# INDA25PlusPlus/rsoderh-raytracing

Hardware: AMD Instinct MI355X
Metric: Mrays/s, house.toml 1920x1080 256spp 8-bounce (higher is better)
Workload: dtype f32; 1 GPU; house.toml 1920x1080 256 spp 8 bounces, synthetic 2048x1024 HDRI env; parallelism=single GPU

## Files before the change

include/rsrt.h:

```cpp
#ifndef RSRT_H
#define RSRT_H

#include <stddef.h>
#include <stdint.h>

#include "rsrt_types.h"

#ifdef __cplusplus
extern "C" {
#endif

typedef enum rsrt_status {
    RSRT_OK = 0,
    RSRT_ERR_INVALID_ARGUMENT = 1,
    RSRT_ERR_NO_DEVICE = 2,
    RSRT_ERR_HIP = 3,
    RSRT_ERR_NOT_READY = 4,
    RSRT_ERR_OUT_OF_MEMORY = 5,
    RSRT_ERR_COMM = 6
} rsrt_status;

typedef struct rsrt_context rsrt_context;

enum {
// ... 92 lines not shown
rsrt_status rsrt_resolve_mean_f16(rsrt_context *ctx, uint32_t sample_total, uint16_t *host_rgba16f, size_t n_halfs);

rsrt_status rsrt_debug_view_f16(rsrt_context *ctx, uint32_t dev_index, uint32_t environment_index, uint32_t sample_count,
                                uint16_t *host_rgba16f_inout, size_t n_halfs);

rsrt_status rsrt_display_srgb8(rsrt_context *ctx, uint32_t sample_total, uint8_t *host_rgba8, size_t n_bytes);

rsrt_status rsrt_render(rsrt_context *ctx, const rsrt_camera *camera, uint32_t width, uint32_t height,
                        uint32_t sample_begin, uint32_t sample_count, uint32_t max_bounces,
                        uint32_t environment_index, uint32_t flags, void *hip_stream);
rsrt_status rsrt_synchronize(rsrt_context *ctx);
rsrt_status rsrt_get_stats(rsrt_context *ctx, rsrt_stats *out);

rsrt_status rsrt_aov_render(rsrt_context *ctx, const rsrt_camera *camera, uint32_t width, uint32_t height, uint32_t sample_begin,
                            uint32_t sample_count, uint32_t flags, void *hip_stream);
rsrt_status rsrt_aov_bind(rsrt_context *ctx, void *device_f32x8, uint32_t width, uint32_t height);
rsrt_status rsrt_aov_clear(rsrt_context *ctx);
rsrt_status rsrt_aov_download(rsrt_context *ctx, float *host_f32x8, size_t n_floats);

enum { RSRT_DENOISE_DEMODULATE = 1u };
typedef struct rsrt_denoise_params {
    uint32_t iterations;
    uint32_t flags;
    float sigma_color;
    float sigma_normal;
    float sigma_depth;
} rsrt_denoise_params;
rsrt_status rsrt_denoise(rsrt_context *ctx, uint32_t sample_total, uint32_t aov_sample_total, const rsrt_denoise_params *params,
                         void *device_out_rgba32f, void *hip_stream);
rsrt_status rsrt_denoised_download(rsrt_context *ctx, float *host_rgba, size_t n_floats);
rsrt_status rsrt_denoised_display_srgb8(rsrt_context *ctx, uint8_t *host_rgba8, size_t n_bytes);

typedef struct rsrt_temporal_params {
    uint32_t max_history;
    float depth_tolerance;
    float normal_tolerance;
} rsrt_temporal_params;
rsrt_status rsrt_temporal_accumulate(rsrt_context *ctx, const rsrt_camera *camera, uint32_t sample_total, uint32_t aov_sample_total,
                                     const rsrt_temporal_params *params, void *hip_stream);
rsrt_status rsrt_temporal_reset(rsrt_context *ctx);
rsrt_status rsrt_temporal_download(rsrt_context *ctx, float *host_rgba, size_t n_floats);
enum { RSRT_DENOISE_TEMPORAL = 2u };

enum { RSRT_TEMPORAL_MOMENTS = 1u };
rsrt_status rsrt_temporal_accumulate_ex(rsrt_context *ctx, const rsrt_camera *camera, uint32_t sample_total, uint32_t aov_sample_total,
                                        const rsrt_temporal_params *params, uint32_t flags, void *hip_stream);
rsrt_status rsrt_temporal_moments_download(rsrt_context *ctx, float *host_f32x4, size_t n_floats);
enum { RSRT_DENOISE_VARIANCE = 4u, RSRT_DENOISE_CLAMP = 8u };

rsrt_status rsrt_guide_render(rsrt_context *ctx, const rsrt_camera *camera, uint32_t width, uint32_t height, uint32_t sample_begin,
                              uint32_t sample_count, uint32_t flags, void *hip_stream);
rsrt_status rsrt_guide_bind(rsrt_context *ctx, void *device_f32x8, uint32_t width, uint32_t height);
rsrt_status rsrt_guide_clear(rsrt_context *ctx);
rsrt_status rsrt_guide_download(rsrt_context *ctx, float *host_f32x8, size_t n_floats);

enum { RSRT_UPSAMPLE_DEMODULATE = 1u, RSRT_UPSAMPLE_DENOISED = 2u, RSRT_UPSAMPLE_TEMPORAL = 4u };
typedef struct rsrt_upsample_params {
    uint32_t flags;
    float sigma_normal;
    float sigma_depth;
} rsrt_upsample_params;
rsrt_status rsrt_upsample(rsrt_context *ctx, uint32_t sample_total, uint32_t aov_sample_total, uint32_t guide_sample_total,
                          const rsrt_upsample_params *params, void *device_out_rgba32f, void *hip_stream);
rsrt_status rsrt_upsampled_download(rsrt_context *ctx, float *host_rgba, size_t n_floats);
rsrt_status rsrt_upsampled_display_srgb8(rsrt_context *ctx, uint8_t *host_rgba8, size_t n_bytes);

typedef struct rsrt_hit {
    uint32_t did_hit;
    float distance;
    float hit_point[3];
    float normal[3];
    uint32_t material_id;
} rsrt_hit;
rsrt_status rsrt_cast_rays(rsrt_context *ctx, uint32_t n_rays, const float *origins_xyz, const float *directions_xyz,
                           uint32_t mode, uint32_t flags, rsrt_hit *out);

rsrt_status rsrt_wide_tree_build(const rsrt_primitive_info *primitives, uint32_t n_primitives, const rsrt_bvh_node *bvh_nodes, uint32_t n_bvh_nodes,
                                 float *wnodes_out, uint32_t *n_wnodes, uint32_t *old_of_new);

rsrt_status rsrt_get_debug_counters(rsrt_context *ctx, uint64_t out[32]);
rsrt_status rsrt_get_region_counters(rsrt_context *ctx, uint64_t out[32]);
rsrt_status rsrt_get_walk_counters(rsrt_context *ctx, uint64_t *out, uint32_t n);

rsrt_status rsrt_selftest_numerics(rsrt_context *ctx, uint64_t out[4]);

const char *rsrt_describe(rsrt_context *ctx);
const char *rsrt_build_id(void);

#ifdef __cplusplus
}
#endif
#endif
```

rsoderh-raytracing_amd/csrc/hip/rsrt_api.hip:

```cpp
#include <hip/hip_fp16.h>
#include <hip/hip_runtime.h>

#include <algorithm>
#include <cstdarg>
#include <cstdio>
#include <cstdlib>
#include <cstring>
#include <string>
#include <vector>

#include "../../../include/rsrt.h"
#include "../../../include/rsrt_tonemap.h"
#include "rt_device.h"

#define RT_BLOCK 256
#define RT_STATS_WORDS 48
#define RT_WAVE 64
#ifndef RT_WALK_POOL
#define RT_WALK_POOL 192u
#endif
#ifndef RT_BIG_POOL
#define RT_BIG_POOL 192u
#endif

// ... 395 lines not shown
    case 2: return reinterpret_cast<const void *>(&rt_cast_rays_kernel<SV, (SV == 2 ? 1 : 2)>);
    case 3: return reinterpret_cast<const void *>(&rt_cast_rays_kernel<SV, 3>);
    case 5: return reinterpret_cast<const void *>(&rt_cast_rays_kernel<SV, 5>);
    case 6: return reinterpret_cast<const void *>(&rt_cast_rays_coop_kernel<SV>);
    default: return reinterpret_cast<const void *>(&rt_cast_rays_kernel<SV, 4>);
    }
}
static const void *probe_function(int sv, int trav)
{
    return sv == 0 ? probe_function_sv<0>(trav) : (sv == 1 ? probe_function_sv<1>(trav) : probe_function_sv<2>(trav));
}

static constexpr uint32_t kLanes = 4;
static constexpr uint64_t kSmallPaths = 4ull << 20;
static constexpr int kPipeBlocks = 1;
static constexpr uint32_t kChunksPerWave = 32;
static constexpr uint32_t kDescendQuorum = 30;
static constexpr uint32_t kStopQuorum = 40;

struct rsrt_context {
    int device = 0;
    hipStream_t stream = nullptr;
    hipEvent_t ev[3] = {nullptr, nullptr, nullptr};
    std::string error;
    std::string description;
    int cus = 0;
    float4 *scene_blob = nullptr;
    DevScene scene{};
    bool scene_ready = false;
    uint32_t hybrid_head_f4 = 0, hybrid_pnode_f4 = 0;
    uint32_t wimg_nodes = 0;
    std::vector<Env> envs;
    uint32_t rank = 0, world = 1, tile_w = 16, tile_h = 16;
    float4 *accum = nullptr;
    float4 *accum_owned = nullptr;
    uint32_t acc_w = 0, acc_h = 0;
    struct Lane {
        hipStream_t stream = nullptr;
        unsigned int *work_counter = nullptr;
        float *sample_buf = nullptr;
        size_t sample_buf_bytes = 0;
        uint32_t *cold_state = nullptr;
        size_t cold_bytes = 0;
        hipEvent_t resolved = nullptr;
        bool resolved_valid = false;
        hipEvent_t traced = nullptr;
        bool traced_valid = false;
        hipEvent_t caller_at = nullptr;
    };
    Lane lanes[kLanes];
    uint32_t next_small_lane = 1;
    unsigned long long *dev_stats = nullptr;
    rsrt_stats stats{};
    struct PassEvents { hipEvent_t begin, traced, end; };
    std::vector<PassEvents> pending_events;
    double cum_trace_ms = 0, cum_resolve_ms = 0, base_trace_ms = 0, base_resolve_ms = 0;
    unsigned long long base_counts[4] = {0, 0, 0, 0};
    uint32_t cum_launches = 0, base_launches = 0;
    std::vector<hipEvent_t> event_pool;
    hipEvent_t last_event = nullptr;
    hipStream_t last_stream = nullptr;
    bool last_valid = false;
    void *comm = nullptr;
    bool comm_owned = false;
    bool comm_dense_mode = false;
    uint32_t comm_rank = 0, comm_world = 1;
    struct ReduceEvents { hipEvent_t begin, end; };
    std::vector<ReduceEvents> pending_reduce;
    double cum_reduce_ms = 0, base_reduce_ms = 0;
    uint32_t cum_reduces = 0;
    void *comm_buf = nullptr;
    size_t comm_buf_bytes = 0;
    void *scratch = nullptr;
    size_t scratch_bytes = 0;
    int blocks_per_cu[21] = {};
    bool small_form = false;
    int max_traversal = 6;
    uint32_t coop_lds_cap = RT_COOP_NCAP, coop_lifo_at = RT_COOP_LIFO_AT, coop_narrow_at = RT_COOP_NARROW_AT;
    uint32_t coop_gcap = RT_COOP_GCAP;
    bool allow_flat = true;
    bool flat_oriented = true;
    bool allow_hybrid = true;
    uint32_t trace_budget = 0;
    uint32_t flat_quorum = 20;
    size_t sample_buffer_budget = 16ull << 30;
    uint32_t probe_repeat = 1;
    int hw_queues = 4;
    bool hw_queue_warned = false;
    unsigned long long debug_words[32] = {0};
    float4 *aov = nullptr;
    float4 *aov_owned = nullptr;
    uint32_t aov_w = 0, aov_h = 0;
    void *dn_scratch = nullptr;
    uint32_t dn_w = 0, dn_h = 0;
    float4 *dn_last = nullptr;
    float4 *tp_buf = nullptr;
    uint32_t tp_w = 0, tp_h = 0, tp_cur = 0, tp_frames = 0;
    float tp_cam[13] = {0};
    float4 *tp_mom = nullptr;
    uint32_t tp_moments = 0;
    float4 *guide = nullptr;
    float4 *guide_owned = nullptr;
    uint32_t guide_w = 0, guide_h = 0;
    void *up_scratch = nullptr;
    uint32_t up_w = 0, up_h = 0;
    float4 *up_out = nullptr;
    uint32_t up_out_w = 0, up_out_h = 0;
    float4 *up_last = nullptr;
    uint32_t up_last_w = 0, up_last_h = 0;
};

namespace {

rsrt_status fail(rsrt_context *ctx, rsrt_status st, const char *fmt, ...)
{
    char buf[1024];
    va_list ap;
    va_start(ap, fmt);
    vsnprintf(buf, sizeof buf, fmt, ap);
    va_end(ap);
    if (ctx) ctx->error = buf;
    else g_create_error = buf;
    return st;
}

#define HIP_TRY(ctx, expr)                                                                                   \
    do {                                                                                                     \
        hipError_t e_ = (expr);                                                                              \
        if (e_ != hipSuccess)                                                                                \
            return fail(ctx, e_ == hipErrorOutOfMemory ? RSRT_ERR_OUT_OF_MEMORY : RSRT_ERR_HIP, "%s failed: %s", #expr, \
                        hipGetErrorString(e_));                                                              \
    } while (0)

struct DeviceGuard {
    explicit DeviceGuard(int dev) { (void)hipSetDevice(dev); }
};

inline float fmaxh(float a, float b) { return a < b ? b : a; }
inline float fminh(float a, float b) { return b < a ? b : a; }
inline float saturateh(float x) { return fminh(fmaxh(x, 0.0f), 1.0f); }
inline float4 f4(float x, float y, float z, float w) { return make_float4(x, y, z, w); }
inline float u2f(uint32_t u) { float f; memcpy(&f, &u, 4); return f; }

void make_sphere_record(const rsrt_sphere &s, float4 *r)
{
    r[0] = f4(s.pos[0], s.pos[1], s.pos[2], u2f(PRIM_SPHERE | (s.material_id << 2)));
    r[1] = f4(s.radius, s.radius * s.radius, 0, 0);
    r[2] = r[3] = f4(0, 0, 0, 0);
}
void make_plane_record(const rsrt_plane &p, float4 *r)
{
    r[0] = f4(p.pos[0], p.pos[1], p.pos[2], u2f(PRIM_PLANE | (p.material_id << 2)));
    r[1] = f4(p.normal[0], p.normal[1], p.normal[2], 0);
    r[2] = f4(p.base_change_matrix[0][0], p.base_change_matrix[1][0], p.base_change_matrix[2][0], 0);
    r[3] = f4(p.base_change_matrix[0][2], p.base_change_matrix[1][2], p.base_change_matrix[2][2], 0);
}
void make_triangle_record(const rsrt_triangle &t, uint32_t index, const rsrt_vec3 *v, float4 *r)
{
    const float *a = v[t.vertex_0].v, *b = v[t.vertex_1].v, *c = v[t.vertex_2].v;
    r[0] = f4(a[0], a[1], a[2], u2f(PRIM_TRIANGLE | (t.material_id << 2)));
    r[1] = f4(b[0] - a[0], b[1] - a[1], b[2] - a[2], u2f(index));
    r[2] = f4(c[0] - a[0], c[1] - a[1], c[2] - a[2], 0);
    r[3] = f4(0, 0, 0, 0);
}
bool same_test(const float4 *a, const float4 *b)
{
    uint32_t ta, tb;
    memcpy(&ta, &a[0].w, 4); memcpy(&tb, &b[0].w, 4);
    if ((ta & 3u) != (tb & 3u) || memcmp(&a[0], &b[0], 12) != 0) return false;
    if ((ta & 3u) == PRIM_TRIANGLE) return memcmp(&a[1], &b[1], 12) == 0 && memcmp(&a[2], &b[2], 12) == 0;
    return memcmp(a + 1, b + 1, 3 * sizeof(float4)) == 0;
}
void make_material_record(const rsrt_material &m, float4 *r)
{
    const float t = saturateh(m.metallic);
    float f0[3], kd[3];
    for (int k = 0; k < 3; k++) f0[k] = (1.0f - t) * 0.04f + t * m.color[k];
    const float maxf0 = fmaxh(f0[0], fmaxh(f0[1], f0[2]));
    for (int k = 0; k < 3; k++) kd[k] = (m.color[k] * (1.0f - t)) * (1.0f - maxf0);
    const float alpha = fmaxh(0.001f, m.roughness * m.roughness);
    const float ps = saturateh(0.2126f * f0[0] + 0.7152f * f0[1] + 0.0722f * f0[2]);
    r[0] = f4(m.color[0], m.color[1], m.color[2], m.metallic);
    r[1] = f4(f0[0], f0[1], f0[2], alpha);
    r[2] = f4(m.emission[0], m.emission[1], m.emission[2], ps);
    r[3] = f4(kd[0], kd[1], kd[2], 1.0f - ps);
}

struct WideNode { uint32_t ch[4]; uint32_t n_ch, n_int, first_child; };
bool build_wide_tree(const rsrt_bvh_node *nodes, uint32_t n_nodes, const rsrt_primitive_info *prims, uint32_t n_prims, std::vector<WideNode> &wide,
                     std::vector<rsrt_primitive_info> &prims_out, std::vector<rsrt_bvh_node> &nodes_out, std::vector<uint32_t> *old_of_new, uint32_t *wide_depth = nullptr)
{
    wide.clear();
    bool ok = n_nodes >= 3 && nodes[0].primitives_len == 0;
    {
        std::vector<uint8_t> covered(n_prims, 0);
        for (uint32_t i = 0; i < n_nodes && ok; i++) {
            const rsrt_bvh_node &nd = nodes[i];
            if (nd.primitives_len > 8) ok = false;
            for (uint32_t k = 0; k < nd.primitives_len && ok; k++) {
                uint8_t &c = covered[nd.primitives_or_second_child_index + k];
                ok = c == 0;
                c = 1;
            }
            if (nd.primitives_len == 0)
                for (uint32_t c : {i + 1u, nd.primitives_or_second_child_index})
                    for (int k = 0; k < 3; k++)
                        ok = ok && nodes[c].bounds_min[k] >= nd.bounds_min[k] && nodes[c].bounds_max[k] <= nd.bounds_max[k];
        }
        for (uint32_t p = 0; p < n_prims; p++) ok = ok && covered[p];
    }
    if (!ok) return false;
    auto area = [&](uint32_t i) {
        const double dx = (double)nodes[i].bounds_max[0] - nodes[i].bounds_min[0], dy = (double)nodes[i].bounds_max[1] - nodes[i].bounds_min[1],
                     dz = (double)nodes[i].bounds_max[2] - nodes[i].bounds_min[2];
        const double a = dx * dy + dy * dz + dz * dx;
        return a == a ? a : 0.0;
    };
    std::vector<uint32_t> queue{0u}, level{0u};
    uint32_t wdepth = 1;
    const bool by_area = true;
    std::vector<std::pair<double, uint32_t>> heap{{area(0), 0u}};
    size_t bfs_next = 0;
    while (by_area ? !heap.empty() : bfs_next < queue.size()) {
        size_t qi;
        if (by_area) {
            std::pop_heap(heap.begin(), heap.end(), [](const std::pair<double, uint32_t> &a, const std::pair<double, uint32_t> &b) { return a.first < b.first || (a.first == b.first && a.second > b.second); });
            qi = heap.back().second;
            heap.pop_back();
        } else {
            qi = bfs_next++;
        }
        const uint32_t r = queue[qi];
        std::vector<uint32_t> ch{r + 1u, nodes[r].primitives_or_second_child_index};
        while (ch.size() < 4) {
            int best = -1;
            for (size_t k = 0; k < ch.size(); k++)
                if (nodes[ch[k]].primitives_len == 0 && (best < 0 || area(ch[k]) > area(ch[best]))) best = (int)k;
            if (best < 0) break;
            const uint32_t c = ch[best];
            ch[best] = c + 1u;
            ch.insert(ch.begin() + best + 1, nodes[c].primitives_or_second_child_index);
        }
        WideNode w{};
        for (uint32_t c : ch) if (nodes[c].primitives_len == 0) w.ch[w.n_ch++] = c;
        w.n_int = w.n_ch;
        for (uint32_t c : ch) if (nodes[c].primitives_len != 0) w.ch[w.n_ch++] = c;
        w.first_child = (uint32_t)queue.size();
        for (uint32_t k = 0; k < w.n_int; k++) {
            const uint32_t idx = (uint32_t)queue.size();
            queue.push_back(w.ch[k]);
            level.push_back(level[qi] + 1u);
            wdepth = std::max(wdepth, level[qi] + 2u);
            if (by_area) {
                heap.push_back({area(w.ch[k]), idx});
// ... 269 lines not shown

rsrt_status pack_environment(rsrt_context *ctx, Env &e)
{
    const size_t n = (size_t)e.width * e.height;
    rsrt_status st = begin_work(ctx, ctx->stream);
    if (st) return st;
    const unsigned nb = (unsigned)((n + 255) / 256);
    hipLaunchKernelGGL(rt_env_pack_texels_kernel, dim3(nb), dim3(256), 0, ctx->stream, e.rgba, e.alias, n);
    hipLaunchKernelGGL(rt_env_pack_alias_kernel, dim3(nb), dim3(256), 0, ctx->stream, e.alias, n);
    HIP_TRY(ctx, hipGetLastError());
    if ((st = end_work(ctx, ctx->stream))) return st;
    HIP_TRY(ctx, hipStreamSynchronize(ctx->stream));
    return RSRT_OK;
}

rsrt_status display_from_n(rsrt_context *ctx, const float4 *sum, size_t n, uint32_t sample_total, uint8_t *host_rgba8, size_t n_bytes)
{
    DeviceGuard g(ctx->device);
    if (!host_rgba8 || n_bytes != n * 4 || sample_total == 0) return fail(ctx, RSRT_ERR_INVALID_ARGUMENT, "display_srgb8: expected %zu bytes and sample_total > 0", n * 4);
    rsrt_status st = ensure_scratch(ctx, n * sizeof(uchar4));
    if (st || (st = begin_work(ctx, ctx->stream))) return st;
    uchar4 *tmp = static_cast<uchar4 *>(ctx->scratch);
    hipLaunchKernelGGL(rt_display_kernel, dim3((unsigned)((n + 255) / 256)), dim3(256), 0, ctx->stream, sum, n, sample_total, tmp);
    HIP_TRY(ctx, hipGetLastError());
    HIP_TRY(ctx, hipMemcpyAsync(host_rgba8, tmp, n * sizeof(uchar4), hipMemcpyDeviceToHost, ctx->stream));
    if ((st = end_work(ctx, ctx->stream))) return st;
    HIP_TRY(ctx, hipStreamSynchronize(ctx->stream));
    return RSRT_OK;
}

rsrt_status display_from(rsrt_context *ctx, const float4 *sum, uint32_t sample_total, uint8_t *host_rgba8, size_t n_bytes)
{
    return display_from_n(ctx, sum, (size_t)ctx->acc_w * ctx->acc_h, sample_total, host_rgba8, n_bytes);
}

}

extern "C" {

rsrt_status rsrt_context_create(int device_index, rsrt_context **out)
{
    if (!out) return fail(nullptr, RSRT_ERR_INVALID_ARGUMENT, "out is NULL");
    *out = nullptr;
    int n = 0;
    hipError_t e = hipGetDeviceCount(&n);
    if (e != hipSuccess || n == 0)
        return fail(nullptr, RSRT_ERR_NO_DEVICE, "no HIP device available (%s); librsrt has no CPU path", hipGetErrorString(e));
    if (device_index < 0 || device_index >= n) return fail(nullptr, RSRT_ERR_INVALID_ARGUMENT, "device_index %d out of range [0,%d)", device_index, n);
    hipDeviceProp_t prop;
    if ((e = hipGetDeviceProperties(&prop, device_index)) != hipSuccess) return fail(nullptr, RSRT_ERR_HIP, "hipGetDeviceProperties: %s", hipGetErrorString(e));
    if (strncmp(prop.gcnArchName, "gfx950", 6) != 0)
        return fail(nullptr, RSRT_ERR_NO_DEVICE, "device %d is %s; librsrt is built for gfx950 (MI355X) only", device_index, prop.gcnArchName);
    rsrt_context *ctx = new rsrt_context();
    ctx->device = device_index;
    ctx->cus = prop.multiProcessorCount;
    DeviceGuard g(device_index);
    if ((e = hipStreamCreateWithFlags(&ctx->stream, hipStreamNonBlocking)) != hipSuccess ||
        (e = hipEventCreateWithFlags(&ctx->last_event, hipEventDisableTiming)) != hipSuccess ||
        (e = [&] { hipError_t r = hipSuccess;
                   for (auto &L : ctx->lanes) {
                       if (r == hipSuccess) r = hipMalloc(&L.work_counter, sizeof(unsigned int));
                       if (r == hipSuccess) r = hipStreamCreateWithFlags(&L.stream, hipStreamNonBlocking);
                       if (r == hipSuccess) r = hipEventCreateWithFlags(&L.resolved, hipEventDisableTiming);
                       if (r == hipSuccess) r = hipEventCreateWithFlags(&L.traced, hipEventDisableTiming);
                       if (r == hipSuccess) r = hipEventCreateWithFlags(&L.caller_at, hipEventDisableTiming);
                   }
                   return r; }()) != hipSuccess ||
        (e = hipMalloc(&ctx->dev_stats, RT_STATS_WORDS * sizeof(unsigned long long))) != hipSuccess ||
        (e = hipMemsetAsync(ctx->dev_stats, 0, RT_STATS_WORDS * sizeof(unsigned long long), ctx->stream)) != hipSuccess ||
        (e = hipStreamSynchronize(ctx->stream)) != hipSuccess) {
        fail(nullptr, RSRT_ERR_HIP, "context setup failed: %s", hipGetErrorString(e));
        delete ctx;
        return RSRT_ERR_HIP;
    }
    for (bool small : {false, true})
        for (int m = 0; m < 21; m++) (void)hipFuncSetAttribute(variant_function(small, m / 7, m % 7), hipFuncAttributeMaxDynamicSharedMemorySize, 160 * 1024);
    if (const char *kv = getenv("RSRT_KERNEL")) ctx->small_form = atoi(kv) == 2;
    if (const char *hy = getenv("RSRT_HYBRID")) ctx->allow_hybrid = atoi(hy) != 0;
    if (const char *ty = getenv("RSRT_TRAVERSAL")) ctx->max_traversal = atoi(ty);
    if (const char *fl = getenv("RSRT_FLAT")) ctx->allow_flat = atoi(fl) != 0;
    if (const char *fo = getenv("RSRT_FLAT_ORIENTED")) ctx->flat_oriented = atoi(fo) != 0;
    if (const char *tb = getenv("RSRT_TRACE_BUDGET")) { int v = atoi(tb); if (v > 0) ctx->trace_budget = (uint32_t)v; }
    if (const char *fq = getenv("RSRT_FLAT_QUORUM")) { int v = atoi(fq); if (v >= 0 && v <= 100) ctx->flat_quorum = (uint32_t)v; }
    if (const char *e2 = getenv("RSRT_SAMPLE_BUFFER_MB")) { long v = atol(e2); if (v > 0) ctx->sample_buffer_budget = (size_t)v << 20; }
    if (const char *pr = getenv("RSRT_PROBE_REPEAT")) { int v = atoi(pr); if (v > 1 && v <= 4096) ctx->probe_repeat = (uint32_t)v; }
    if (const char *cl = getenv("RSRT_COOP_LDS_CAP")) { int v = atoi(cl); if (v >= (int)RT_COOP_MIN_LDS_CAP && v <= (int)RT_COOP_NCAP) ctx->coop_lds_cap = (uint32_t)v; }
    if (const char *cf = getenv("RSRT_COOP_LIFO_AT")) { int v = atoi(cf); if (v >= 0 && v <= (int)RT_COOP_NARROW_AT) ctx->coop_lifo_at = (uint32_t)v; }
    if (const char *cn = getenv("RSRT_COOP_NARROW_AT")) { int v = atoi(cn); if (v >= 0 && v <= (int)RT_COOP_NARROW_AT) ctx->coop_narrow_at = (uint32_t)v; }
    if (const char *cg = getenv("RSRT_COOP_GCAP")) { int v = atoi(cg); if (v >= 64 && v <= (int)RT_COOP_GCAP && v % 64 == 0) ctx->coop_gcap = (uint32_t)v; }
    if (const char *cm = getenv("RSRT_COMM_MODE")) ctx->comm_dense_mode = strcmp(cm, "reduce") == 0;
    if (const char *hq = getenv("GPU_MAX_HW_QUEUES")) { int v = atoi(hq); if (v > 0) ctx->hw_queues = v; }
    for (int m = 0; m < 21; m++) (void)hipFuncSetAttribute(probe_function(m / 7, m % 7), hipFuncAttributeMaxDynamicSharedMemorySize, 160 * 1024);
    char buf[256];
    snprintf(buf, sizeof buf, "librsrt 0.1; %s (%s); %d CUs", prop.name, prop.gcnArchName, ctx->cus);
    ctx->description = buf;
    *out = ctx;
    return RSRT_OK;
}

void rsrt_context_destroy(rsrt_context *ctx)
{
    if (!ctx) return;
    DeviceGuard g(ctx->device);
    (void)sync_all(ctx);
    (void)rsrt_comm_destroy(ctx);
    for (auto &re : ctx->pending_reduce) { (void)hipEventDestroy(re.begin); (void)hipEventDestroy(re.end); }
    if (ctx->last_event) (void)hipEventDestroy(ctx->last_event);
    (void)hipFree(ctx->scratch);
    (void)hipFree(ctx->comm_buf);
    for (auto &pe : ctx->pending_events) { (void)hipEventDestroy(pe.begin); (void)hipEventDestroy(pe.traced); (void)hipEventDestroy(pe.end); }
    for (auto e : ctx->event_pool) (void)hipEventDestroy(e);
    (void)hipFree(ctx->scene_blob);
    for (auto &e : ctx->envs) { (void)hipFree(e.rgba); (void)hipFree(e.alias); }
    (void)hipFree(ctx->accum_owned);
    (void)hipFree(ctx->aov_owned);
    (void)hipFree(ctx->dn_scratch);
    (void)hipFree(ctx->tp_buf);
    (void)hipFree(ctx->tp_mom);
    (void)hipFree(ctx->guide_owned);
    (void)hipFree(ctx->up_scratch);
    (void)hipFree(ctx->up_out);
    for (auto &L : ctx->lanes) {
        (void)hipFree(L.sample_buf);
        (void)hipFree(L.cold_state);
        (void)hipFree(L.work_counter);
        if (L.resolved) (void)hipEventDestroy(L.resolved);
        if (L.traced) (void)hipEventDestroy(L.traced);
        if (L.caller_at) (void)hipEventDestroy(L.caller_at);
        if (L.stream) (void)hipStreamDestroy(L.stream);
    }
    (void)hipFree(ctx->dev_stats);
    (void)hipStreamDestroy(ctx->stream);
    delete ctx;
}

const char *rsrt_last_error(const rsrt_context *ctx) { return ctx ? ctx->error.c_str() : g_create_error.c_str(); }

#ifndef RSRT_BUILD_ID
#define RSRT_BUILD_ID "unknown"
#endif
const char *rsrt_build_id(void) { return RSRT_BUILD_ID; }

const char *rsrt_describe(rsrt_context *ctx) { return ctx ? ctx->description.c_str() : "librsrt 0.1"; }

rsrt_status rsrt_upload_scene(rsrt_context *ctx, const rsrt_material *materials, uint32_t n_materials, const rsrt_sphere *spheres,
                              uint32_t n_spheres, const rsrt_plane *planes, uint32_t n_planes, const rsrt_vec3 *vertices,
                              uint32_t n_vertices, const rsrt_vec3 *normals, uint32_t n_normals, const rsrt_triangle *triangles,
                              uint32_t n_triangles, const rsrt_primitive_info *primitives_in, uint32_t n_primitives,
                              const rsrt_bvh_node *nodes_in, uint32_t n_nodes)
{
    if (!ctx) return RSRT_ERR_INVALID_ARGUMENT;
    DeviceGuard g(ctx->device);
    ctx->tp_frames = 0;
    const rsrt_primitive_info *primitives = primitives_in;
    const rsrt_bvh_node *nodes = nodes_in;
    if (n_nodes == 0 || !nodes) return fail(ctx, RSRT_ERR_INVALID_ARGUMENT, "bvh_nodes is empty");
    if (n_nodes >= RT_END) return fail(ctx, RSRT_ERR_INVALID_ARGUMENT, "bvh_nodes: %u nodes exceed the 25-bit traversal cursor", n_nodes);
    if ((n_materials && !materials) || (n_spheres && !spheres) || (n_planes && !planes) || (n_vertices && !vertices) ||
        (n_normals && !normals) || (n_triangles && !triangles) || (n_primitives && !primitives))
        return fail(ctx, RSRT_ERR_INVALID_ARGUMENT, "a non-empty array has a NULL pointer");
    if (n_materials >= (1u << 30)) return fail(ctx, RSRT_ERR_INVALID_ARGUMENT, "too many materials");
    for (uint32_t i = 0; i < n_spheres; i++)
        if (spheres[i].material_id >= n_materials) return fail(ctx, RSRT_ERR_INVALID_ARGUMENT, "sphere %u: material_id %u out of range", i, spheres[i].material_id);
    for (uint32_t i = 0; i < n_planes; i++)
        if (planes[i].material_id >= n_materials) return fail(ctx, RSRT_ERR_INVALID_ARGUMENT, "plane %u: material_id %u out of range", i, planes[i].material_id);
    for (uint32_t i = 0; i < n_triangles; i++) {
        const rsrt_triangle &t = triangles[i];
        if (t.material_id >= n_materials) return fail(ctx, RSRT_ERR_INVALID_ARGUMENT, "triangle %u: material_id %u out of range", i, t.material_id);
        if (t.vertex_0 >= n_vertices || t.vertex_1 >= n_vertices || t.vertex_2 >= n_vertices)
            return fail(ctx, RSRT_ERR_INVALID_ARGUMENT, "triangle %u: vertex index out of range", i);
        if (t.normal_0 >= n_normals || t.normal_1 >= n_normals || t.normal_2 >= n_normals)
            return fail(ctx, RSRT_ERR_INVALID_ARGUMENT, "triangle %u: normal index out of range", i);
    }
    for (uint32_t i = 0; i < n_primitives; i++) {
        const rsrt_primitive_info &p = primitives[i];
        uint32_t lim = p.primitive_type == 0 ? n_spheres : (p.primitive_type == 1 ? n_planes : (p.primitive_type == 2 ? n_triangles : 0));
        if (p.index >= lim) return fail(ctx, RSRT_ERR_INVALID_ARGUMENT, "primitive %u: type %u index %u out of range", i, p.primitive_type, p.index);
    }
    uint32_t depth = 0;
    {
        std::vector<std::pair<uint32_t, uint32_t>> st;
        std::vector<uint8_t> seen(n_nodes, 0);
        st.push_back({0u, 0u});
        while (!st.empty()) {
            auto [i, d] = st.back();
            st.pop_back();
            if (seen[i]) return fail(ctx, RSRT_ERR_INVALID_ARGUMENT, "bvh node %u reachable twice", i);
            seen[i] = 1;
            depth = std::max(depth, d);
            const rsrt_bvh_node &nd = nodes[i];
            if (nd.primitives_len > 0) {
                if (nd.primitives_len > 0xffffu || (uint64_t)nd.primitives_or_second_child_index + nd.primitives_len > n_primitives)
                    return fail(ctx, RSRT_ERR_INVALID_ARGUMENT, "bvh leaf %u: primitive range out of bounds", i);
            } else {
                uint32_t second = nd.primitives_or_second_child_index;
                if (nd.split_axis > 2 || i + 1 >= n_nodes || second <= i + 1 || second >= n_nodes)
                    return fail(ctx, RSRT_ERR_INVALID_ARGUMENT, "bvh interior node %u: bad child index / axis", i);
                st.push_back({second, d + 1});
                st.push_back({i + 1, d + 1});
            }
        }
        for (uint32_t i = 0; i < n_nodes; i++)
            if (!seen[i]) return fail(ctx, RSRT_ERR_INVALID_ARGUMENT, "bvh node %u is not reachable from the root", i);
    }
    std::vector<WideNode> wide;
    std::vector<rsrt_primitive_info> prims_perm;
    std::vector<rsrt_bvh_node> nodes_perm;
    uint32_t wide_depth = 0;
    const bool wide_ok = build_wide_tree(nodes, n_nodes, primitives, n_primitives, wide, prims_perm, nodes_perm, nullptr, &wide_depth);
    if (wide_ok) {
        primitives = prims_perm.data();
        nodes = nodes_perm.data();
    }
    std::vector<uint32_t> escape(8ull * n_nodes, RT_END);
    for (uint32_t q = 0; q < 8; q++) {
        std::vector<std::pair<uint32_t, uint32_t>> st;
        st.push_back({0u, RT_END});
        while (!st.empty()) {
            auto [i, esc] = st.back();
            st.pop_back();
            escape[(size_t)q * n_nodes + i] = esc;
            const rsrt_bvh_node &nd = nodes[i];
            if (nd.primitives_len == 0) {
                const bool far_first = (q >> nd.split_axis) & 1u;
                const uint32_t first = i + 1, second = nd.primitives_or_second_child_index;
                const uint32_t near_c = far_first ? second : first, far_c = far_first ? first : second;
                st.push_back({near_c, far_c});
                st.push_back({far_c, esc});
            }
        }
    }
    const size_t esc_f4 = (8ull * n_nodes + 3) / 4;
    std::vector<uint32_t> leaf_nodes;
    bool flat_ok = n_primitives <= 64 && n_spheres <= 64 && n_planes <= 64;
    {
        std::vector<uint8_t> covered(n_primitives, 0);
        for (uint32_t i = 0; i < n_nodes && flat_ok; i++)
            for (uint32_t k = 0; k < nodes[i].primitives_len && flat_ok; k++) {
                uint8_t &c = covered[nodes[i].primitives_or_second_child_index + k];
                flat_ok = c == 0;
                c = 1;
            }
    }
    for (uint32_t i = 0; i < n_nodes; i++) {
        const rsrt_bvh_node &nd = nodes[i];
        if (nd.primitives_len != 0) { leaf_nodes.push_back(i); continue; }
        for (uint32_t c : {i + 1u, nd.primitives_or_second_child_index})
            for (int k = 0; k < 3; k++)
                flat_ok = flat_ok && nodes[c].bounds_min[k] >= nd.bounds_min[k] && nodes[c].bounds_max[k] <= nd.bounds_max[k];
    }
    flat_ok = flat_ok && leaf_nodes.size() <= 32;
    std::vector<uint32_t> flat_rank(8 * 16, 0u);
    uint64_t tri_mask = 0, plane_mask = 0;
    if (flat_ok) {
        for (uint32_t p = 0; p < n_primitives; p++) {
            if (primitives[p].primitive_type >= 2) tri_mask |= 1ull << p;
            else if (primitives[p].primitive_type == 1) plane_mask |= 1ull << p;
        }
        for (uint32_t q = 0; q < 8; q++) {
            std::vector<uint32_t> st{0u};
            uint32_t pos = 0;
            while (!st.empty()) {
                const uint32_t i = st.back();
                st.pop_back();
                const rsrt_bvh_node &nd = nodes[i];
                if (nd.primitives_len != 0) {
                    for (uint32_t k = 0; k < nd.primitives_len; k++, pos++) {
                        const uint32_t rec = nd.primitives_or_second_child_index + k;
                        flat_rank[q * 16 + (rec >> 2)] |= pos << (8 * (rec & 3));
                    }
                } else {
                    const bool far_first = (q >> nd.split_axis) & 1u;
                    const uint32_t first = i + 1, second = nd.primitives_or_second_child_index;
                    st.push_back(far_first ? first : second);
                    st.push_back(far_first ? second : first);
                }
            }
        }
    }
    const size_t flat_f4 = flat_ok ? 2 * leaf_nodes.size() : 0, rank_f4 = flat_ok ? 32 : 0;
    const size_t ostride_f4 = 2 * (leaf_nodes.size() | 1);
    const size_t oflat_f4 = flat_ok && ctx->flat_oriented ? 8 * ostride_f4 : 0;
    const size_t base_f4 = 2ull * n_nodes + 4ull * n_primitives + 3ull * n_triangles + 4ull * n_materials + 4ull * n_spheres + 4ull * n_planes + esc_f4 + flat_f4;
    const bool flat_oriented = oflat_f4 != 0 && (base_f4 + oflat_f4) * sizeof(float4) <= kSmallImageBytes;
    std::vector<uint32_t> prim_rank(8ull * n_primitives, 0xffffffffu);
    for (uint32_t q = 0; q < 8; q++) {
        std::vector<uint32_t> st{0u};
        uint32_t pos = 0;
        while (!st.empty()) {
            const uint32_t i = st.back();
            st.pop_back();
            const rsrt_bvh_node &nd = nodes[i];
            if (nd.primitives_len != 0) {
                for (uint32_t k = 0; k < nd.primitives_len; k++, pos++) {
                    uint32_t &rk = prim_rank[(size_t)q * n_primitives + nd.primitives_or_second_child_index + k];
                    rk = std::min(rk, pos);
                }
            } else {
                const bool far_first = (q >> nd.split_axis) & 1u;
                const uint32_t first = i + 1, second = nd.primitives_or_second_child_index;
                st.push_back(far_first ? first : second);
                st.push_back(far_first ? second : first);
            }
        }
    }
    struct PNode { uint32_t old; uint32_t jump_to; };
    std::vector<uint32_t> succ(n_nodes, n_nodes);
    {
        std::vector<std::pair<uint32_t, uint32_t>> st;
        st.push_back({0u, n_nodes});
        while (!st.empty()) {
            auto [i, after] = st.back();
            st.pop_back();
            succ[i] = after;
            const rsrt_bvh_node &nd = nodes[i];
            if (nd.primitives_len == 0) {
                st.push_back({i + 1, nd.primitives_or_second_child_index});
                st.push_back({nd.primitives_or_second_child_index, after});
            }
        }
    }
    const uint32_t kTopMax = kHybridRoomF4 / 2u;
    std::vector<PNode> plist;
    uint32_t top_elems = 0;
    for (uint32_t want = std::min<uint32_t>(n_nodes, kTopMax);; want = want * 7 / 8) {
        std::vector<uint8_t> in_top(n_nodes, 0);
        {
            auto area = [&](uint32_t i) {
                const double dx = (double)nodes[i].bounds_max[0] - nodes[i].bounds_min[0], dy = (double)nodes[i].bounds_max[1] - nodes[i].bounds_min[1],
                             dz = (double)nodes[i].bounds_max[2] - nodes[i].bounds_min[2];
                const double a = dx * dy + dy * dz + dz * dx;
                return a == a ? a : 0.0;
            };
            std::vector<std::pair<double, uint32_t>> heap;
            heap.push_back({area(0), 0u});
            uint32_t taken = 0;
            while (!heap.empty() && taken < want) {
                std::pop_heap(heap.begin(), heap.end());
                const uint32_t i = heap.back().second;
                heap.pop_back();
                in_top[i] = 1;
                taken++;
                if (nodes[i].primitives_len == 0)
                    for (uint32_t c : {i + 1u, nodes[i].primitives_or_second_child_index}) {
                        heap.push_back({area(c), c});
                        std::push_heap(heap.begin(), heap.end());
                    }
            }
        }
        plist.clear();
        for (int pass = 0; pass < 2; pass++) {
            std::vector<uint32_t> order;
            for (uint32_t i = 0; i < n_nodes; i++)
                if ((in_top[i] != 0) == (pass == 0)) order.push_back(i);
            for (size_t k = 0; k < order.size(); k++) {
                const uint32_t i = order[k];
                plist.push_back({i, 0u});
                const uint32_t follows = k + 1 < order.size() ? order[k + 1] : 0xffffffffu;
                if (nodes[i].primitives_len != 0 && succ[i] != follows) plist.push_back({0xffffffffu, succ[i]});
            }
            if (pass == 0) top_elems = (uint32_t)plist.size();
        }
        if (top_elems <= kTopMax || want <= 1) break;
    }
    const uint32_t n_pnodes = (uint32_t)plist.size();
    if (n_pnodes >= RT_END) return fail(ctx, RSRT_ERR_INVALID_ARGUMENT, "bvh_nodes: %u traversal elements exceed the 25-bit cursor", n_pnodes);
    std::vector<uint32_t> new_id(n_nodes + 1, n_pnodes);
    for (uint32_t e = 0; e < n_pnodes; e++)
        if (plist[e].old != 0xffffffffu) new_id[plist[e].old] = e;
    const size_t pnode_f4 = 2ull * n_pnodes, prank_f4 = (8ull * n_primitives + 3) / 4, wnode_f4 = 8ull * wide.size();
    const uint32_t wimg_nodes = wide_ok ? (uint32_t)wide.size() : 0u;
    const size_t n_f4 = base_f4 + (flat_oriented ? oflat_f4 : 0);
    std::vector<float4> img(n_f4 + rank_f4 + pnode_f4 + prank_f4 + wnode_f4);
    float4 *p = img.data();
    float4 *p_nodes = p;
    bool typed_leaves = true;
    for (uint32_t i = 0; i < n_nodes; i++) typed_leaves = typed_leaves && nodes[i].primitives_len <= 8;
    for (uint32_t i = 0; i < n_nodes; i++, p += 2) {
        const rsrt_bvh_node &nd = nodes[i];
        p[0] = f4(nd.bounds_min[0], nd.bounds_min[1], nd.bounds_min[2], u2f(nd.primitives_or_second_child_index));
        uint32_t hi = nd.split_axis;
        if (nd.primitives_len != 0) {
            hi = 0;
            if (typed_leaves)
                for (uint32_t k = 0; k < nd.primitives_len; k++) {
                    const uint32_t ty = primitives[nd.primitives_or_second_child_index + k].primitive_type;
                    if (ty >= 2) hi |= 1u << k;
                    else if (ty == 1) hi |= 1u << (8 + k);
                }
        }
        p[1] = f4(nd.bounds_max[0], nd.bounds_max[1], nd.bounds_max[2], u2f(nd.primitives_len | (hi << 16)));
    }
    float4 *p_esc = p;
    memcpy(p_esc, escape.data(), escape.size() * sizeof(uint32_t));
    p += esc_f4;
    const size_t traversal_head_f4 = (size_t)(p - img.data());
    float4 *p_prims = p;
    for (uint32_t i = 0; i < n_primitives; i++, p += 4) {
        const rsrt_primitive_info &pi = primitives[i];
        if (pi.primitive_type == 0) make_sphere_record(spheres[pi.index], p);
        else if (pi.primitive_type == 1) make_plane_record(planes[pi.index], p);
        else make_triangle_record(triangles[pi.index], pi.index, vertices, p);
    }
    float4 *p_trin = p;
    for (uint32_t i = 0; i < n_triangles; i++, p += 3) {
        const float *a = normals[triangles[i].normal_0].v, *b = normals[triangles[i].normal_1].v, *c = normals[triangles[i].normal_2].v;
        p[0] = f4(a[0], a[1], a[2], b[0]);
        p[1] = f4(b[1], b[2], c[0], c[1]);
        p[2] = f4(c[2], 0, 0, 0);
    }
    float4 *p_mats = p;
    for (uint32_t i = 0; i < n_materials; i++, p += 4) make_material_record(materials[i], p);
    float4 *p_fbs = p;
    for (uint32_t i = 0; i < n_spheres; i++, p += 4) make_sphere_record(spheres[i], p);
    float4 *p_fbp = p;
    for (uint32_t i = 0; i < n_planes; i++, p += 4) make_plane_record(planes[i], p);
    float4 *p_flat = p;
    if (flat_ok) {
        for (uint32_t i : leaf_nodes) {
            const rsrt_bvh_node &nd = nodes[i];
            uint64_t lm = (nd.primitives_len >= 64 ? ~0ull : ((1ull << nd.primitives_len) - 1ull)) << nd.primitives_or_second_child_index;
            for (uint32_t b = 1; b < nd.primitives_len; b++)
                for (uint32_t a = 0; a < b; a++)
                    if (same_test(p_prims + 4 * (nd.primitives_or_second_child_index + a), p_prims + 4 * (nd.primitives_or_second_child_index + b))) {
                        lm &= ~(1ull << (nd.primitives_or_second_child_index + b));
                        break;
                    }
            p[0] = f4(nd.bounds_min[0], nd.bounds_min[1], nd.bounds_min[2], u2f((uint32_t)lm));
            p[1] = f4(nd.bounds_max[0], nd.bounds_max[1], nd.bounds_max[2], u2f((uint32_t)(lm >> 32)));
            p += 2;
        }
        if (flat_oriented) {
            for (uint32_t q = 0; q < 8; q++)
                for (size_t k = 0; k < leaf_nodes.size(); k++) {
                    const float4 lo = p_flat[2 * k], hi = p_flat[2 * k + 1];
                    float4 *c = p + q * ostride_f4 + 2 * k;
                    c[0] = f4(q & 1u ? hi.x : lo.x, q & 2u ? hi.y : lo.y, q & 4u ? hi.z : lo.z, lo.w);
                    c[1] = f4(q & 1u ? lo.x : hi.x, q & 2u ? lo.y : hi.y, q & 4u ? lo.z : hi.z, hi.w);
                }
            p += oflat_f4;
        }
        memcpy(p, flat_rank.data(), flat_rank.size() * sizeof(uint32_t));
    }
    {
        std::vector<uint32_t> twins;
        for (uint32_t i = 0; i < n_nodes; i++) {
            const rsrt_bvh_node &nd = nodes[i];
            for (uint32_t b = 1; b < nd.primitives_len; b++)
                for (uint32_t a = 0; a < b; a++)
                    if (same_test(p_prims + 4 * (nd.primitives_or_second_child_index + a), p_prims + 4 * (nd.primitives_or_second_child_index + b))) {
                        twins.push_back(nd.primitives_or_second_child_index + b);
                        break;
                    }
        }
        for (uint32_t r : twins) p_prims[4 * r + 2].w = u2f(1u);
    }
    float4 *p_pnodes = img.data() + n_f4 + rank_f4;
    for (uint32_t e = 0; e < n_pnodes; e++) {
        if (plist[e].old == 0xffffffffu) {
            const uint32_t to = new_id[plist[e].jump_to];
            p_pnodes[2 * e] = f4(0, 0, 0, u2f(to));
            p_pnodes[2 * e + 1] = f4(0, 0, 0, u2f(to));
            continue;
        }
        const uint32_t i = plist[e].old;
        p_pnodes[2 * e] = p_nodes[2 * i];
        p_pnodes[2 * e + 1] = p_nodes[2 * i + 1];
        if (nodes[i].primitives_len == 0) {
            p_pnodes[2 * e].w = u2f(new_id[i + 1]);
            p_pnodes[2 * e + 1].w = u2f(new_id[succ[i]]);
        } else {
            p_pnodes[2 * e].w = u2f(nodes[i].primitives_or_second_child_index | 0x80000000u);
        }
    }
    if (n_primitives) memcpy(p_pnodes + pnode_f4, prim_rank.data(), prim_rank.size() * sizeof(uint32_t));
    fill_wide_nodes(wide, nodes, primitives, p_pnodes + pnode_f4 + prank_f4);

    { rsrt_status st0 = sync_all(ctx); if (st0) return st0; }
    if (ctx->scene_blob) { (void)hipFree(ctx->scene_blob); ctx->scene_blob = nullptr; }
    ctx->scene_ready = false;
    HIP_TRY(ctx, hipMalloc(&ctx->scene_blob, img.size() * sizeof(float4)));
    HIP_TRY(ctx, hipMemcpy(ctx->scene_blob, img.data(), img.size() * sizeof(float4), hipMemcpyHostToDevice));
    DevScene &sc = ctx->scene;
    sc.nodes = ctx->scene_blob + (p_nodes - img.data());
    sc.prims = ctx->scene_blob + (p_prims - img.data());
    sc.tri_normals = ctx->scene_blob + (p_trin - img.data());
    sc.materials = ctx->scene_blob + (p_mats - img.data());
    sc.fb_spheres = ctx->scene_blob + (p_fbs - img.data());
    sc.fb_planes = ctx->scene_blob + (p_fbp - img.data());
    sc.escape = ctx->scene_blob + (p_esc - img.data());
    sc.flat_leaves = ctx->scene_blob + (p_flat - img.data());
    sc.flat_ostride = flat_oriented ? (uint32_t)ostride_f4 : 0u;
    sc.flat_rank = reinterpret_cast<const uint32_t *>(ctx->scene_blob + n_f4);
    sc.pnodes = ctx->scene_blob + n_f4 + rank_f4;
    sc.n_pnodes = n_pnodes;
    sc.prim_rank = reinterpret_cast<const uint32_t *>(ctx->scene_blob + n_f4 + rank_f4 + pnode_f4);
    sc.wnodes = ctx->scene_blob + n_f4 + rank_f4 + pnode_f4 + prank_f4;
    sc.n_wnodes = (uint32_t)wide.size();
    sc.wide_ok = wide_ok ? 1u : 0u;
    sc.wide_deep = (wide_ok && wide_depth > RT_WSTACK + 1u) ? 1u : 0u;
    sc.coop_ok = (wide_ok && n_primitives < RT_COOP_MAX_RECORDS && wide.size() < RT_COOP_MAX_NODES) ? 1u : 0u;
    sc.lds_wnodes = 0u;
    ctx->wimg_nodes = wimg_nodes;
    sc.flat_ok = flat_ok ? 1u : 0u;
    sc.n_cull = 0; sc.cull_always = 0xffffffffu;
    if (flat_ok) {
        std::vector<uint32_t> leaf_index(n_nodes, 0u);
        for (size_t k = 0; k < leaf_nodes.size(); k++) leaf_index[leaf_nodes[k]] = (uint32_t)k;
        std::vector<std::pair<uint32_t, uint32_t>> st{{0u, 0u}};
        uint32_t always = 0u;
        const uint32_t cull_depth = 2u;
        while (!st.empty()) {
            auto [i, d] = st.back();
            st.pop_back();
            const rsrt_bvh_node &nd = nodes[i];
            if (nd.primitives_len != 0) { always |= 1u << leaf_index[i]; continue; }
            if (d == cull_depth && sc.n_cull < 8) {
                uint32_t m = 0;
                std::vector<uint32_t> sub{i};
                while (!sub.empty()) {
                    const uint32_t j = sub.back();
                    sub.pop_back();
                    if (nodes[j].primitives_len != 0) m |= 1u << leaf_index[j];
                    else { sub.push_back(j + 1); sub.push_back(nodes[j].primitives_or_second_child_index); }
                }
                for (int k = 0; k < 3; k++) { sc.cull_min[sc.n_cull][k] = nd.bounds_min[k]; sc.cull_max[sc.n_cull][k] = nd.bounds_max[k]; }
                sc.cull_mask[sc.n_cull++] = m;
                continue;
            }
            st.push_back({i + 1, d + 1});
            st.push_back({nd.primitives_or_second_child_index, d + 1});
        }
        sc.cull_always = always;
    }
    sc.n_leaves = (uint32_t)leaf_nodes.size();
    sc.tri_mask_lo = (uint32_t)tri_mask; sc.tri_mask_hi = (uint32_t)(tri_mask >> 32);
    sc.plane_mask_lo = (uint32_t)plane_mask; sc.plane_mask_hi = (uint32_t)(plane_mask >> 32);
    sc.n_nodes = n_nodes; sc.n_prims = n_primitives; sc.n_tris = n_triangles; sc.n_materials = n_materials;
    sc.n_spheres = n_spheres; sc.n_planes = n_planes;
    sc.stack_entries = depth + 1;
    sc.typed_leaves = typed_leaves ? 1u : 0u;
    const size_t stack_bytes = (size_t)sc.stack_entries * RT_BLOCK * sizeof(uint32_t);
    if (stack_bytes > 128 * 1024) return fail(ctx, RSRT_ERR_INVALID_ARGUMENT, "bvh depth %u exceeds the supported traversal stack", depth);
    sc.lds_float4s = (n_f4 * sizeof(float4) <= kSmallImageBytes) ? (uint32_t)n_f4 : 0u;
    sc.lds_hybrid = 0;
    sc.lds_src = sc.nodes;
    ctx->hybrid_head_f4 = ctx->hybrid_pnode_f4 = 0;
    if (sc.lds_float4s == 0) {
        if (traversal_head_f4 * sizeof(float4) <= 40 * 1024) ctx->hybrid_head_f4 = (uint32_t)traversal_head_f4;
        ctx->hybrid_pnode_f4 = 2u * top_elems;
    } else {
        ctx->wimg_nodes = 0;
    }
    memset(ctx->blocks_per_cu, 0, sizeof ctx->blocks_per_cu);
    ctx->scene_ready = true;
    return RSRT_OK;
}

rsrt_status rsrt_build_bvh_device(rsrt_context *ctx, const rsrt_sphere *spheres, uint32_t n_spheres, const rsrt_plane_desc *planes, uint32_t n_planes,
                                  const rsrt_vec3 *vertices, uint32_t n_vertices, const rsrt_triangle *triangles, uint32_t n_triangles,
                                  rsrt_primitive_info *primitives_out, rsrt_bvh_node *nodes_out, uint32_t *n_nodes_out, uint32_t *depth_out, double *build_ms_out)
{
    if (!ctx) return RSRT_ERR_INVALID_ARGUMENT;
    DeviceGuard g(ctx->device);
    const uint64_t n64 = (uint64_t)n_spheres + n_planes + n_triangles;
    if (n64 == 0) return fail(ctx, RSRT_ERR_INVALID_ARGUMENT, "build_bvh: empty scene");
    if (n64 > 0x3fffffffull) return fail(ctx, RSRT_ERR_INVALID_ARGUMENT, "build_bvh: too many primitives");
    if (!primitives_out || !nodes_out || (n_spheres && !spheres) || (n_planes && !planes) || (n_triangles && (!triangles || !vertices)))
        return fail(ctx, RSRT_ERR_INVALID_ARGUMENT, "build_bvh: NULL array");
    for (uint32_t i = 0; i < n_triangles; i++)
        if (triangles[i].vertex_0 >= n_vertices || triangles[i].vertex_1 >= n_vertices || triangles[i].vertex_2 >= n_vertices)
            return fail(ctx, RSRT_ERR_INVALID_ARGUMENT, "build_bvh: triangle %u: vertex index out of range", i);
    const uint32_t n = (uint32_t)n64;
    { rsrt_status st0 = sync_all(ctx); if (st0) return st0; }
    size_t off = 0;
    auto take = [&](size_t bytes) { const size_t o = off; off += (bytes + 255) & ~(size_t)255; return o; };
    const size_t o_sph = take((size_t)n_spheres * sizeof(rsrt_sphere)), o_pl = take((size_t)n_planes * sizeof(rsrt_plane_desc)),
                 o_v = take((size_t)n_vertices * sizeof(rsrt_vec3)), o_tri = take((size_t)n_triangles * sizeof(rsrt_triangle));
    size_t o_items[6];
    for (auto &o : o_items) o = take((size_t)n * sizeof(float4));
    const size_t o_nodes = take((size_t)2 * n * sizeof(BvhNodeB)), o_t0 = take((size_t)n * sizeof(BvhTask)), o_t1 = take((size_t)n * sizeof(BvhTask));
    const size_t o_pre = take((size_t)n * 4), o_holes = take((size_t)n * 4), o_backs = take((size_t)n * 4), o_cnt = take(16);
    const size_t o_outn = take((size_t)2 * n * sizeof(rsrt_bvh_node)), o_outp = take((size_t)n * sizeof(rsrt_primitive_info));
    char *blob = nullptr;
    HIP_TRY(ctx, hipMalloc(&blob, off));
    struct Free { char *p; ~Free() { (void)hipFree(p); } } free_blob{blob};
    hipStream_t q = ctx->stream;
    if (n_spheres) HIP_TRY(ctx, hipMemcpyAsync(blob + o_sph, spheres, (size_t)n_spheres * sizeof(rsrt_sphere), hipMemcpyHostToDevice, q));
    if (n_planes) HIP_TRY(ctx, hipMemcpyAsync(blob + o_pl, planes, (size_t)n_planes * sizeof(rsrt_plane_desc), hipMemcpyHostToDevice, q));
    if (n_vertices) HIP_TRY(ctx, hipMemcpyAsync(blob + o_v, vertices, (size_t)n_vertices * sizeof(rsrt_vec3), hipMemcpyHostToDevice, q));
    if (n_triangles) HIP_TRY(ctx, hipMemcpyAsync(blob + o_tri, triangles, (size_t)n_triangles * sizeof(rsrt_triangle), hipMemcpyHostToDevice, q));
    BvhItems A{reinterpret_cast<float4 *>(blob + o_items[0]), reinterpret_cast<float4 *>(blob + o_items[1]), reinterpret_cast<float4 *>(blob + o_items[2])};
    BvhItems B{reinterpret_cast<float4 *>(blob + o_items[3]), reinterpret_cast<float4 *>(blob + o_items[4]), reinterpret_cast<float4 *>(blob + o_items[5])};
    BvhNodeB *bnodes = reinterpret_cast<BvhNodeB *>(blob + o_nodes);
    BvhTask *tasks[2] = {reinterpret_cast<BvhTask *>(blob + o_t0), reinterpret_cast<BvhTask *>(blob + o_t1)};
    uint32_t *counters = reinterpret_cast<uint32_t *>(blob + o_cnt);
    hipEvent_t e0 = get_event(ctx), e1 = get_event(ctx);
    struct Back { rsrt_context *c; hipEvent_t a, b; ~Back() { c->event_pool.push_back(a); c->event_pool.push_back(b); } } back{ctx, e0, e1};
    HIP_TRY(ctx, hipEventRecord(e0, q));
    hipLaunchKernelGGL(rt_bvh_items_kernel, dim3((n + 255) / 256), dim3(256), 0, q, reinterpret_cast<const rsrt_sphere *>(blob + o_sph), n_spheres,
                       reinterpret_cast<const rsrt_plane_desc *>(blob + o_pl), n_planes, reinterpret_cast<const rsrt_vec3 *>(blob + o_v),
                       reinterpret_cast<const rsrt_triangle *>(blob + o_tri), n_triangles, A);
    HIP_TRY(ctx, hipMemcpyAsync(B.bmin, A.bmin, (size_t)n * sizeof(float4), hipMemcpyDeviceToDevice, q));
    HIP_TRY(ctx, hipMemcpyAsync(B.bmax, A.bmax, (size_t)n * sizeof(float4), hipMemcpyDeviceToDevice, q));
    HIP_TRY(ctx, hipMemcpyAsync(B.cen, A.cen, (size_t)n * sizeof(float4), hipMemcpyDeviceToDevice, q));
    const BvhTask root{0u, n, 0u};
    uint32_t cnt[4] = {1u, 0u, 0u, 0u};
    HIP_TRY(ctx, hipMemcpyAsync(tasks[0], &root, sizeof root, hipMemcpyHostToDevice, q));
    HIP_TRY(ctx, hipMemcpyAsync(counters, cnt, sizeof cnt, hipMemcpyHostToDevice, q));
    std::vector<std::pair<uint32_t, uint32_t>> levels;
    uint32_t n_tasks = 1, first = 0, n_build = 1;
    BvhItems *src = &A, *dst = &B;
    for (int lvl = 0; n_tasks > 0; lvl++) {
        if (lvl > 4096) return fail(ctx, RSRT_ERR_INVALID_ARGUMENT, "build_bvh: tree deeper than 4096 levels");
        levels.push_back({first, n_tasks});
        hipLaunchKernelGGL(rt_bvh_level_kernel, dim3(n_tasks), dim3(RT_BVH_BLOCK), 0, q, tasks[lvl & 1], n_tasks, *src, *dst, bnodes, tasks[(lvl + 1) & 1], counters,
                           reinterpret_cast<uint32_t *>(blob + o_pre), reinterpret_cast<uint32_t *>(blob + o_holes), reinterpret_cast<uint32_t *>(blob + o_backs));
        hipLaunchKernelGGL(rt_bvh_copy_leaves_kernel, dim3(n_tasks), dim3(64), 0, q, tasks[lvl & 1], n_tasks, bnodes, *src, *dst);
        HIP_TRY(ctx, hipGetLastError());
        HIP_TRY(ctx, hipMemcpyAsync(cnt, counters, sizeof cnt, hipMemcpyDeviceToHost, q));
        HIP_TRY(ctx, hipStreamSynchronize(q));
        if (cnt[2]) return fail(ctx, RSRT_ERR_INVALID_ARGUMENT, "build_bvh: a split left one side empty (the reference's median fallback, src/bvh.rs:317-326, is not built on the device): use rsrt_build_bvh");
        first = n_build;
        n_tasks = cnt[1];
        n_build = cnt[0];
        cnt[1] = 0;
        HIP_TRY(ctx, hipMemcpyAsync(counters + 1, &cnt[1], 4, hipMemcpyHostToDevice, q));
        std::swap(src, dst);
    }
    for (size_t d = levels.size(); d-- > 0;)
        hipLaunchKernelGGL(rt_bvh_sizes_kernel, dim3((levels[d].second + 255) / 256), dim3(256), 0, q, bnodes, levels[d].first, levels[d].second);
    for (size_t d = 0; d < levels.size(); d++)
        hipLaunchKernelGGL(rt_bvh_positions_kernel, dim3((levels[d].second + 255) / 256), dim3(256), 0, q, bnodes, levels[d].first, levels[d].second);
    hipLaunchKernelGGL(rt_bvh_emit_kernel, dim3((n_build + 255) / 256), dim3(256), 0, q, bnodes, n_build, reinterpret_cast<rsrt_bvh_node *>(blob + o_outn));
    hipLaunchKernelGGL(rt_bvh_prims_kernel, dim3((n + 255) / 256), dim3(256), 0, q, *src, n, reinterpret_cast<rsrt_primitive_info *>(blob + o_outp));
    HIP_TRY(ctx, hipGetLastError());
    HIP_TRY(ctx, hipEventRecord(e1, q));
    HIP_TRY(ctx, hipMemcpyAsync(nodes_out, blob + o_outn, (size_t)n_build * sizeof(rsrt_bvh_node), hipMemcpyDeviceToHost, q));
    HIP_TRY(ctx, hipMemcpyAsync(primitives_out, blob + o_outp, (size_t)n * sizeof(rsrt_primitive_info), hipMemcpyDeviceToHost, q));
    HIP_TRY(ctx, hipStreamSynchronize(q));
    float ms = 0;
    HIP_TRY(ctx, hipEventElapsedTime(&ms, e0, e1));
    if (n_nodes_out) *n_nodes_out = n_build;
    if (depth_out) *depth_out = (uint32_t)levels.size() - 1u;
    if (build_ms_out) *build_ms_out = ms;
    return RSRT_OK;
}

rsrt_status rsrt_wide_tree_build(const rsrt_primitive_info *primitives, uint32_t n_primitives, const rsrt_bvh_node *nodes, uint32_t n_nodes,
                                 float *wnodes_out, uint32_t *n_wnodes, uint32_t *old_of_new)
{
    if (!primitives || !nodes || !n_wnodes || n_nodes == 0) return RSRT_ERR_INVALID_ARGUMENT;
    for (uint32_t i = 0; i < n_nodes; i++) {
        const rsrt_bvh_node &nd = nodes[i];
        if (nd.primitives_len > 0) { if ((uint64_t)nd.primitives_or_second_child_index + nd.primitives_len > n_primitives) return RSRT_ERR_INVALID_ARGUMENT; }
        else if (i + 1 >= n_nodes || nd.primitives_or_second_child_index <= i + 1 || nd.primitives_or_second_child_index >= n_nodes) return RSRT_ERR_INVALID_ARGUMENT;
    }
    std::vector<WideNode> wide;
    std::vector<rsrt_primitive_info> pp;
    std::vector<rsrt_bvh_node> np;
    std::vector<uint32_t> oon;
    if (!build_wide_tree(nodes, n_nodes, primitives, n_primitives, wide, pp, np, &oon)) return RSRT_ERR_INVALID_ARGUMENT;
    const uint32_t cap = *n_wnodes;
    *n_wnodes = (uint32_t)wide.size();
    if (wnodes_out) {
        if (cap < wide.size()) return RSRT_ERR_INVALID_ARGUMENT;
        fill_wide_nodes(wide, np.data(), pp.data(), reinterpret_cast<float4 *>(wnodes_out));
    }
    if (old_of_new) memcpy(old_of_new, oon.data(), oon.size() * sizeof(uint32_t));
    return RSRT_OK;
}

rsrt_status rsrt_upload_environment(rsrt_context *ctx, uint32_t slot, uint32_t width, uint32_t height, const float *rgba,
                                    const rsrt_alias_entry *alias)
{
    if (!ctx) return RSRT_ERR_INVALID_ARGUMENT;
    DeviceGuard g(ctx->device);
    ctx->tp_frames = 0;
    if (!rgba || width == 0 || height == 0) return fail(ctx, RSRT_ERR_INVALID_ARGUMENT, "environment: NULL data or zero size");
    if ((uint64_t)width * height > 0x7fffffffull) return fail(ctx, RSRT_ERR_INVALID_ARGUMENT, "environment too large");
    if (slot > 63) return fail(ctx, RSRT_ERR_INVALID_ARGUMENT, "environment slot %u > 63", slot);
    const size_t n = (size_t)width * height;
    if (alias)
        for (size_t i = 0; i < n; i++)
            if (alias[i].alias_index >= n) return fail(ctx, RSRT_ERR_INVALID_ARGUMENT, "alias entry %zu: alias_index %u out of range", i, alias[i].alias_index);
    if (ctx->envs.size() <= slot) ctx->envs.resize(slot + 1);
    Env &e = ctx->envs[slot];
    { rsrt_status st0 = sync_all(ctx); if (st0) return st0; }
    if (e.rgba) { (void)hipFree(e.rgba); e.rgba = nullptr; }
    if (e.alias) { (void)hipFree(e.alias); e.alias = nullptr; }
    e.width = e.height = 0;
    HIP_TRY(ctx, hipMalloc(&e.rgba, n * sizeof(float4)));
    HIP_TRY(ctx, hipMalloc(&e.alias, n * sizeof(uint4)));
    HIP_TRY(ctx, hipMemcpy(e.rgba, rgba, n * sizeof(float4), hipMemcpyHostToDevice));
    if (alias) {
        HIP_TRY(ctx, hipMemcpy(e.alias, alias, n * sizeof(uint4), hipMemcpyHostToDevice));
        e.width = width;
        e.height = height;
        return pack_environment(ctx, e);
    }
    e.width = width;
    e.height = height;
    const rsrt_status st = rsrt_environment_build_alias(ctx, slot, nullptr, 0, nullptr);
    if (st) { e.width = e.height = 0; }
    return st;
}

rsrt_status rsrt_environment_build_alias(rsrt_context *ctx, uint32_t slot, rsrt_alias_entry *host_out, size_t n_entries, uint32_t *leftover_out)
{
    if (!ctx) return RSRT_ERR_INVALID_ARGUMENT;
    DeviceGuard g(ctx->device);
    if (slot >= ctx->envs.size() || !ctx->envs[slot].rgba || !ctx->envs[slot].alias || ctx->envs[slot].width == 0)
        return fail(ctx, RSRT_ERR_NOT_READY, "environment %u not uploaded", slot);
    Env &e = ctx->envs[slot];
    const size_t n = (size_t)e.width * e.height;
    if (host_out && n_entries != n) return fail(ctx, RSRT_ERR_INVALID_ARGUMENT, "build_alias: expected %zu entries", n);
    const uint32_t nb = (uint32_t)((n + 255) / 256);
    const size_t bytes = n * 4 * 3 + (size_t)nb * 4 + 16;
    rsrt_status st = ensure_scratch(ctx, bytes);
    if (st || (st = begin_work(ctx, ctx->stream))) return st;
    float *p = static_cast<float *>(ctx->scratch);
    uint32_t *small = reinterpret_cast<uint32_t *>(p + n), *large = small + n, *blocks = large + n, *scalars = blocks + nb;
    hipStream_t q = ctx->stream;
    hipLaunchKernelGGL(rt_alias_weights_kernel, dim3(nb), dim3(256), 0, q, e.rgba, e.width, e.height, p);
    hipLaunchKernelGGL(rt_alias_sum_kernel, dim3(1), dim3(64), 0, q, p, n, reinterpret_cast<float *>(scalars));
    hipLaunchKernelGGL(rt_alias_normalise_kernel, dim3(nb), dim3(256), 0, q, p, n, reinterpret_cast<const float *>(scalars), e.alias, blocks);
    hipLaunchKernelGGL(rt_alias_scan_kernel, dim3(1), dim3(1024), 0, q, blocks, nb, scalars + 1);
    hipLaunchKernelGGL(rt_alias_scatter_kernel, dim3(nb), dim3(256), 0, q, p, n, blocks, small, large);
    hipLaunchKernelGGL(rt_alias_vose_kernel, dim3(1), dim3(64), 0, q, p, n, small, scalars + 1, large, e.alias, scalars + 2);
    hipLaunchKernelGGL(rt_alias_pmf_kernel, dim3(nb), dim3(256), 0, q, p, n, e.alias);
    HIP_TRY(ctx, hipGetLastError());
// ... 249 lines not shown
}

rsrt_status rsrt_synchronize(rsrt_context *ctx)
{
    if (!ctx) return RSRT_ERR_INVALID_ARGUMENT;
    DeviceGuard g(ctx->device);
    return sync_all(ctx);
}

rsrt_status rsrt_get_stats(rsrt_context *ctx, rsrt_stats *out)
{
    if (!ctx || !out) return RSRT_ERR_INVALID_ARGUMENT;
    DeviceGuard g(ctx->device);
    rsrt_status st = collect_stats(ctx);
    if (st) return st;
    *out = ctx->stats;
    return RSRT_OK;
}

__global__ void rt_selftest_rcp_kernel(unsigned long long *out)
{
    unsigned long long bad = 0, raw_differs = 0, fast_path = 0;
    const uint64_t stride = (uint64_t)gridDim.x * blockDim.x;
    for (uint64_t i = (uint64_t)blockIdx.x * blockDim.x + threadIdx.x; i < (1ull << 32); i += stride) {
        const float x = as_f((uint32_t)i);
        const float ref = 1.0f / x;
        if (as_u(rt_rcp(x)) != as_u(ref)) {
            bad++;
            atomicMin(&out[3], (unsigned long long)i);
        }
        const uint32_t ex = ((uint32_t)i >> 23) & 0xffu;
        if (ex - 2u < 251u) {
            fast_path++;
            if (as_u(__builtin_amdgcn_rcpf(x)) != as_u(ref)) raw_differs++;
        }
    }
    atomicAdd(&out[0], bad);
    atomicAdd(&out[1], fast_path);
    atomicAdd(&out[2], raw_differs);
}

rsrt_status rsrt_selftest_numerics(rsrt_context *ctx, uint64_t out[4])
{
    if (!ctx || !out) return RSRT_ERR_INVALID_ARGUMENT;
    DeviceGuard g(ctx->device);
    unsigned long long *d = nullptr, h[4] = {0, 0, 0, ~0ull};
    { rsrt_status st0 = sync_all(ctx); if (st0) return st0; }
    HIP_TRY(ctx, hipMalloc(&d, sizeof h));
    hipError_t e = hipMemcpy(d, h, sizeof h, hipMemcpyHostToDevice);
    if (e == hipSuccess) {
        hipLaunchKernelGGL(rt_selftest_rcp_kernel, dim3(ctx->cus * 8), dim3(256), 0, ctx->stream, d);
        e = hipGetLastError();
    }
    if (e == hipSuccess) e = hipStreamSynchronize(ctx->stream);
    if (e == hipSuccess) e = hipMemcpy(h, d, sizeof h, hipMemcpyDeviceToHost);
    (void)hipFree(d);
    if (e != hipSuccess) return fail(ctx, RSRT_ERR_HIP, "selftest: %s", hipGetErrorString(e));
    for (int i = 0; i < 4; i++) out[i] = h[i];
    return RSRT_OK;
}

rsrt_status rsrt_get_debug_counters(rsrt_context *ctx, uint64_t out[32])
{
    if (!ctx || !out) return RSRT_ERR_INVALID_ARGUMENT;
    DeviceGuard g(ctx->device);
    rsrt_status st = collect_stats(ctx);
    if (st) return st;
    for (int i = 0; i < 32; i++) out[i] = ctx->debug_words[i];
    return RSRT_OK;
}

rsrt_status rsrt_get_walk_counters(rsrt_context *ctx, uint64_t *out, uint32_t n)
{
    if (!ctx || (!out && n != 0)) return RSRT_ERR_INVALID_ARGUMENT;
    DeviceGuard g(ctx->device);
    { rsrt_status st0 = sync_all(ctx); if (st0) return st0; }
    unsigned long long c[RT_COOP_NSTATS];
    HIP_TRY(ctx, hipMemcpy(c, ctx->dev_stats + RT_COOP_STATS, sizeof c, hipMemcpyDeviceToHost));
    for (uint32_t i = 0; i < n && i < RT_COOP_NSTATS; i++) out[i] = c[i];
    for (uint32_t i = RT_COOP_NSTATS; i < n; i++) out[i] = 0;
    return RSRT_OK;
}

rsrt_status rsrt_get_region_counters(rsrt_context *ctx, uint64_t out[32])
{
    if (!ctx || !out) return RSRT_ERR_INVALID_ARGUMENT;
    DeviceGuard g(ctx->device);
    for (int i = 0; i < 32; i++) out[i] = 0;
#ifdef RT_INSTRUMENT
    { rsrt_status st0 = sync_all(ctx); if (st0) return st0; }
    unsigned long long h[32], z[32] = {0};
    HIP_TRY(ctx, hipMemcpyFromSymbol(h, HIP_SYMBOL(rt_region_lanes), sizeof h));
    HIP_TRY(ctx, hipMemcpyToSymbol(HIP_SYMBOL(rt_region_lanes), z, sizeof z));
    for (int i = 0; i < 32; i++) out[i] = h[i];
#endif
    return RSRT_OK;
}

rsrt_status rsrt_cast_rays(rsrt_context *ctx, uint32_t n, const float *origins, const float *dirs, uint32_t mode, uint32_t flags,
                           rsrt_hit *out)
{
    if (!ctx) return RSRT_ERR_INVALID_ARGUMENT;
    DeviceGuard g(ctx->device);
    if (!ctx->scene_ready) return fail(ctx, RSRT_ERR_NOT_READY, "no scene uploaded");
    if (n == 0) return RSRT_OK;
    if (!origins || !dirs || !out || mode > 31 || ((mode >> 1) & 7u) > 6u) return fail(ctx, RSRT_ERR_INVALID_ARGUMENT, "cast_rays: bad arguments");
    DevScene sc = ctx->scene;
    const uint32_t sel = (mode >> 1) & 7u;
    const int trav = sel == 0 ? 0 : (sel == 1 ? 4 : (sel == 2 ? 1 : (sel == 3 ? 2 : (sel == 4 ? 3 : (sel == 5 ? 5 : 6)))));
    const size_t coop_lds = trav == 6 ? (size_t)(RT_BLOCK / RT_WAVE) * 4u * pool_wave_lds_dwords(6, 64u) : 0u;
    int sv = 0;
    if (mode & 16u) {
        if (sc.lds_float4s != 0) {
            sv = 1;
        } else {
            const uint32_t all_f4 = 160u * 1024u / (uint32_t)sizeof(float4);
            const uint32_t stack_f4 = trav == 4 ? (uint32_t)(((size_t)sc.stack_entries * RT_BLOCK * sizeof(uint32_t) + 15u) / 16u) : 0u;
            const uint32_t coop_f4 = (uint32_t)((coop_lds + 15u) / 16u);
            if (!hybrid_stage(ctx, sc, trav == 5 ? 4 : (trav == 4 ? 0 : trav), all_f4 > stack_f4 + coop_f4 ? all_f4 - stack_f4 - coop_f4 : 0u))
                return fail(ctx, RSRT_ERR_INVALID_ARGUMENT, "cast_rays: this scene is not staged in LDS by the production kernel");
            sv = 2;
        }
    } else {
        sc.lds_float4s = 0;
    }
    if (trav == 6 && !(sc.wide_ok && sc.coop_ok)) return fail(ctx, RSRT_ERR_INVALID_ARGUMENT, "cast_rays: the cooperative walk needs what the wide walk needs, fewer than 2^21 records and 2^24 wide nodes");
    if (trav == 5 && !sc.wide_ok) return fail(ctx, RSRT_ERR_INVALID_ARGUMENT, "cast_rays: the wide walk needs nested boxes, leaves of at most 8 primitives that share no record, and a wide tree of at most 25 levels");
    if ((trav == 1 || trav == 3) && !sc.typed_leaves) return fail(ctx, RSRT_ERR_INVALID_ARGUMENT, "cast_rays: typed leaf loops need leaves of at most 8 primitives");
    if (trav == 2 && (!sc.flat_ok || sv == 2)) return fail(ctx, RSRT_ERR_INVALID_ARGUMENT, "cast_rays: the flat traversal needs a scene of at most 64 records with nested boxes");
    { rsrt_status st0 = sync_all(ctx); if (st0) return st0; }
    float *d_o = nullptr, *d_d = nullptr;
    rsrt_hit *d_h = nullptr;
    uint32_t *d_g = nullptr;
    const uint32_t n_blocks = (n + RT_BLOCK - 1) / RT_BLOCK;
    hipError_t e = hipMalloc(&d_o, (size_t)n * 12);
    if (e == hipSuccess && trav == 6) e = hipMalloc(&d_g, (size_t)n_blocks * (RT_BLOCK / RT_WAVE) * RT_COOP_GCAP * sizeof(uint32_t));
    if (e == hipSuccess) e = hipMalloc(&d_d, (size_t)n * 12);
    if (e == hipSuccess) e = hipMalloc(&d_h, (size_t)n * sizeof(rsrt_hit));
    if (e == hipSuccess) e = hipMemcpy(d_o, origins, (size_t)n * 12, hipMemcpyHostToDevice);
    if (e == hipSuccess) e = hipMemcpy(d_d, dirs, (size_t)n * 12, hipMemcpyHostToDevice);
    if (e == hipSuccess) {
        const size_t smem = (size_t)sc.lds_float4s * sizeof(float4) + (trav == 4 ? (size_t)sc.stack_entries * RT_BLOCK * sizeof(uint32_t) : 0u) + coop_lds;
        if (smem > 160 * 1024) { (void)hipFree(d_o); (void)hipFree(d_d); (void)hipFree(d_h); (void)hipFree(d_g); return fail(ctx, RSRT_ERR_INVALID_ARGUMENT, "cast_rays: needs %zu bytes of LDS", smem); }
        uint32_t repeat = ctx->probe_repeat;
        void *kargs[] = {&sc, &n, &d_o, &d_d, &mode, &flags, &repeat, &d_h, &d_g, &ctx->coop_lds_cap, &ctx->coop_lifo_at, &ctx->coop_narrow_at, &ctx->coop_gcap,
                         &ctx->dev_stats};
        e = hipLaunchKernel(probe_function(sv, trav), dim3(n_blocks), dim3(RT_BLOCK), kargs, smem, ctx->stream);
    }
    if (e == hipSuccess) e = hipStreamSynchronize(ctx->stream);
    if (e == hipSuccess) e = hipMemcpy(out, d_h, (size_t)n * sizeof(rsrt_hit), hipMemcpyDeviceToHost);
    (void)hipFree(d_o); (void)hipFree(d_d); (void)hipFree(d_h); (void)hipFree(d_g);
    if (e != hipSuccess) return fail(ctx, RSRT_ERR_HIP, "cast_rays: %s", hipGetErrorString(e));
    return RSRT_OK;
}

}

#include "rsrt_comm.h"
#include "rt_denoise.h"
#include "rt_temporal.h"
#include "rt_variance.h"
#include "rt_upsample.h"
```

rsoderh-raytracing_amd/csrc/hip/rt_device.h:

```cpp
#pragma once
#include "rt_math.h"

#ifdef RT_INSTRUMENT
#define RT_DBG_N 32
struct DbgCounters { unsigned long long c[RT_DBG_N]; };
#define DBG_DECL DbgCounters &dbg,
#define DBG_ARG dbg,
#ifdef RT_SHADE_PROFILE
#define DBG_ADD(i, v) do { if ((i) < 10 || (i) > 15) dbg.c[i] += (v); } while (0)
#define DBG_WAVE_TICK(i) do { } while (0)
#else
#define DBG_ADD(i, v) dbg.c[i] += (v)
#define DBG_WAVE_TICK(i) do { if ((threadIdx.x & 63u) == (uint32_t)__builtin_ctzll(__ballot(true))) dbg.c[i] += 1; } while (0)
#endif
#else
#define DBG_DECL
#define DBG_ARG
#define DBG_ADD(i, v) do { } while (0)
#define DBG_WAVE_TICK(i) do { } while (0)
#endif

#define RT_INFINITY 1.70141183460469231732e+38f
#define RT_PI ((float)3.14159)
#define RT_INV_PI ((float)(1.0 / 3.14159))
#define RT_TWO_PI ((float)(2.0 * 3.14159))

enum { PRIM_SPHERE = 0, PRIM_PLANE = 1, PRIM_TRIANGLE = 2 };
enum { SRC_BVH = 0, SRC_FB_SPHERE = 1, SRC_FB_PLANE = 2 };

struct DevScene {
    const float4 *nodes;
    const float4 *prims;
    const float4 *tri_normals;
    const float4 *materials;
    const float4 *fb_spheres;
    const float4 *fb_planes;
    const float4 *escape;
    const float4 *flat_leaves;
    uint32_t n_nodes, n_prims, n_tris, n_materials, n_spheres, n_planes;
    uint32_t stack_entries;
    uint32_t lds_float4s;
    uint32_t lds_hybrid;
    uint32_t typed_leaves;
    uint32_t flat_ok, n_leaves;
    uint32_t tri_mask_lo, tri_mask_hi, plane_mask_lo, plane_mask_hi;
    const uint32_t *flat_rank;
    float cull_min[8][3], cull_max[8][3];
    uint32_t cull_mask[8], cull_always, n_cull;
    const float4 *pnodes;
    uint32_t n_pnodes;
    const uint32_t *prim_rank;
    const float4 *wnodes;
    uint32_t n_wnodes, wide_ok;
    uint32_t wide_deep;
    uint32_t coop_ok;
    uint32_t lds_wnodes;
    uint32_t flat_ostride;
    const float4 *lds_src;
};

struct DevEnv {
    const float4 *rgba;
    const uint4 *alias;
    uint32_t width, height;
    float wf, hf;
    float dphi_dtheta;
    uint32_t width_shift;
};

template <bool LDS>
struct SceneView;

extern __shared__ float4 rt_smem[];

template <>
struct SceneView<true> {
    uint32_t o_nodes, o_prims, o_esc, o_trin, o_mats, o_fbs, o_fbp, o_flat;
    const float4 *pnodes;
    const float4 *wnodes;
    RT_DEV void pnode_pair(uint32_t e, float4 &n0, float4 &n1) const { n0 = pnodes[2u * e]; n1 = pnodes[2u * e + 1u]; }
    RT_DEV void wnode(uint32_t i, float4 (&n)[8]) const
    {
#pragma unroll
        for (int k = 0; k < 8; k++) n[k] = wnodes[8u * i + k];
    }
    RT_DEV float4 node(uint32_t i) const { return rt_smem[o_nodes + i]; }
    RT_DEV float4 flat(uint32_t i) const { return rt_smem[o_flat + i]; }
    RT_DEV float4 prim(uint32_t i) const { return rt_smem[o_prims + i]; }
    template <int N>
    RT_DEV void prim_rec(uint32_t rec, float4 (&r)[N]) const
    {
#pragma unroll
        for (int k = 0; k < N; k++) r[k] = rt_smem[o_prims + 4u * rec + (uint32_t)k];
    }
    RT_DEV float4 trin(uint32_t i) const { return rt_smem[o_trin + i]; }
    RT_DEV float4 mat(uint32_t i) const { return rt_smem[o_mats + i]; }
    RT_DEV float4 rec(uint32_t src, uint32_t i) const
    {
        return rt_smem[o_prims + (src == SRC_FB_SPHERE ? o_fbs - o_prims : 0u) + (src == SRC_FB_PLANE ? o_fbp - o_prims : 0u) + i];
    }
    RT_DEV uint32_t esc(uint32_t i) const { return reinterpret_cast<const uint32_t *>(rt_smem + o_esc)[i]; }
};
template <>
struct SceneView<false> {
    const float4 *nodes, *prims, *tri_normals, *materials, *fb_spheres, *fb_planes, *escape, *flat_leaves, *pnodes, *wnodes;
    RT_DEV void pnode_pair(uint32_t e, float4 &n0, float4 &n1) const { n0 = pnodes[2u * e]; n1 = pnodes[2u * e + 1u]; }
    RT_DEV void wnode(uint32_t i, float4 (&n)[8]) const
    {
#pragma unroll
        for (int k = 0; k < 8; k++) n[k] = wnodes[8u * i + k];
    }
    RT_DEV float4 node(uint32_t i) const { return nodes[i]; }
    RT_DEV float4 flat(uint32_t i) const { return flat_leaves[i]; }
    RT_DEV float4 prim(uint32_t i) const { return prims[i]; }
    template <int N>
    RT_DEV void prim_rec(uint32_t rec, float4 (&r)[N]) const
    {
#pragma unroll
        for (int k = 0; k < N; k++) r[k] = prims[4u * rec + (uint32_t)k];
    }
    RT_DEV float4 trin(uint32_t i) const { return tri_normals[i]; }
    RT_DEV float4 mat(uint32_t i) const { return materials[i]; }
    RT_DEV float4 rec(uint32_t src, uint32_t i) const
    {
        const ptrdiff_t ds = fb_spheres - prims, dp = fb_planes - prims;
        return prims[(src == SRC_FB_SPHERE ? ds : 0) + (src == SRC_FB_PLANE ? dp : 0) + (ptrdiff_t)i];
    }
    RT_DEV uint32_t esc(uint32_t i) const { return reinterpret_cast<const uint32_t *>(escape)[i]; }
};

struct SceneViewHybrid {
    uint32_t o_nodes, o_esc;
    const float4 *prims, *tri_normals, *materials, *fb_spheres, *fb_planes;
// ... 797 lines not shown
            const float4 n0 = S.node(2u * cur), n1 = S.node(2u * cur + 1u);
            const uint32_t esc = S.esc(ebase + cur);
            float t_0;
            bool inside = slab_test(n0, n1, o, inv, t_0);
            inside = inside & !(prune & (t_0 > h.t));
            const uint32_t idx = as_u(n0.w), la = as_u(n1.w);
            const uint32_t len = la & 0xffffu, hi = la >> 16;
            const bool descend = inside & (len == 0u);
            const uint32_t near_child = ((octant >> (hi & 3u)) & 1u) ? idx : cur + 1u;
            if (inside & (len != 0u)) {
#pragma unroll
                for (int j = 0; j < RT_LEAFQ; j++) qi[j] = (nq == (uint32_t)j) ? idx : qi[j];
                const uint32_t sh = 8u * nq;
                all_m |= ((1u << len) - 1u) << sh;
                tri_m |= (hi & 0xffu) << sh;
                pl_m |= (hi >> 8) << sh;
                steps += len;
                nq++;
            }
            cur = descend ? near_child : esc;
        }
        uint32_t sp_m = all_m & ~(tri_m | pl_m);
        uint32_t best_p = 0xffffffffu;
        while (tri_m != 0u) {
            DBG_WAVE_TICK(12);
            DBG_ADD(13, 1);
            const uint32_t p = take_lowest(tri_m);
            uint32_t base = qi[0];
#pragma unroll
            for (int j = 1; j < RT_LEAFQ; j++) base = ((p >> 3) == (uint32_t)j) ? qi[j] : base;
            const uint32_t rec = base + (p & 7u);
            const float4 r0 = S.prim(4u * rec), r1 = S.prim(4u * rec + 1u), r2 = S.prim(4u * rec + 2u);
            float u, v;
            const float t = triangle_t(o, d, v3(r0.x, r0.y, r0.z), v3(r1.x, r1.y, r1.z), v3(r2.x, r2.y, r2.z), u, v);
            const bool better = (t >= 0.0f) & (t < h.t);
            h.t = better ? t : h.t;
            h.ref = better ? rec : h.ref;
            best_p = better ? p : best_p;
            if (better & anyhit) { cur = RT_END; tri_m = pl_m = sp_m = 0u; }
        }
        while (pl_m != 0u) {
            DBG_WAVE_TICK(15);
            DBG_ADD(13, 1);
            const uint32_t p = take_lowest(pl_m);
            uint32_t base = qi[0];
#pragma unroll
            for (int j = 1; j < RT_LEAFQ; j++) base = ((p >> 3) == (uint32_t)j) ? qi[j] : base;
            const uint32_t rec = base + (p & 7u);
            const float4 r0 = S.prim(4u * rec), r1 = S.prim(4u * rec + 1u), r2 = S.prim(4u * rec + 2u), r3 = S.prim(4u * rec + 3u);
            const float t = plane_t(o, d, v3(r0.x, r0.y, r0.z), v3(r1.x, r1.y, r1.z), v3(r2.x, r2.y, r2.z), v3(r3.x, r3.y, r3.z));
            const bool better = (t >= 0.0f) & ((t < h.t) | ((t == h.t) & (p < best_p) & (best_p != 0xffffffffu)));
            h.t = better ? t : h.t;
            h.ref = better ? rec : h.ref;
            best_p = better ? p : best_p;
            if (better & anyhit) { cur = RT_END; pl_m = sp_m = 0u; }
        }
        while (sp_m != 0u) {
            DBG_WAVE_TICK(28);
            DBG_ADD(13, 1);
            const uint32_t p = take_lowest(sp_m);
            uint32_t base = qi[0];
#pragma unroll
            for (int j = 1; j < RT_LEAFQ; j++) base = ((p >> 3) == (uint32_t)j) ? qi[j] : base;
            const uint32_t rec = base + (p & 7u);
            const float4 r0 = S.prim(4u * rec), r1 = S.prim(4u * rec + 1u);
            const float t = sphere_t(o, d, v3(r0.x, r0.y, r0.z), r1.y);
            const bool better = (t >= 0.0f) & ((t < h.t) | ((t == h.t) & (p < best_p) & (best_p != 0xffffffffu)));
            h.t = better ? t : h.t;
            h.ref = better ? rec : h.ref;
            best_p = better ? p : best_p;
            if (better & anyhit) { cur = RT_END; sp_m = 0u; }
        }
    }
    work += steps;
}

RT_DEV uint32_t flat_rank_of(const DevScene &sc, uint32_t octant, uint32_t rec)
{
    return (sc.flat_rank[octant * 16u + (rec >> 2)] >> (8u * (rec & 3u))) & 0xffu;
}

template <class View>
RT_DEV void trace_flat(DBG_DECL const View &S, const DevScene &sc, V3 o, V3 d, V3 inv, bool anyhit, uint32_t quorum, uint32_t &cur, unsigned long long &rem, Hit &h,
                       bool coherent = false)
{
    RT_MARK(4);
    const bool resumed = cur != 0u;
    uint32_t all_lo = 0u, all_hi = 0u;
    const uint32_t n_leaves = __ballot(!resumed) != 0ull ? sc.n_leaves : 0u;
    uint32_t active = 0xffffffffu;
    if (coherent && n_leaves != 0u) {
        active = sc.cull_always;
        for (uint32_t g = 0; g < sc.n_cull; g++) {
            const float ax = (sc.cull_min[g][0] - o.x) * inv.x, bx = (sc.cull_max[g][0] - o.x) * inv.x;
            const float ay = (sc.cull_min[g][1] - o.y) * inv.y, by = (sc.cull_max[g][1] - o.y) * inv.y;
            const float az = (sc.cull_min[g][2] - o.z) * inv.z, bz = (sc.cull_max[g][2] - o.z) * inv.z;
            const float t_0 = __builtin_fmaxf(__builtin_fmaxf(__builtin_fmaxf(__builtin_fminf(ax, bx), __builtin_fminf(ay, by)), __builtin_fminf(az, bz)), 0.0f);
            const float t_1 = __builtin_fminf(__builtin_fminf(__builtin_fminf(__builtin_fmaxf(ax, bx), __builtin_fmaxf(ay, by)), __builtin_fmaxf(az, bz)), RT_INFINITY);
            if (__ballot(!resumed & !(t_0 > t_1)) != 0ull) active |= sc.cull_mask[g];
        }
    }
    if (sc.flat_ostride != 0u) {
        const uint32_t octant = (inv.x < 0.0f ? 1u : 0u) | (inv.y < 0.0f ? 2u : 0u) | (inv.z < 0.0f ? 4u : 0u);
        const uint32_t table = 2u * sc.n_leaves + octant * sc.flat_ostride;
#pragma unroll 4
        for (uint32_t L = 0; L < n_leaves; L++) {
            if (!((active >> L) & 1u)) continue;
            RT_MARK(5);
            DBG_WAVE_TICK(10);
            DBG_ADD(11, 1);
            const float4 n0 = S.flat(table + 2u * L), n1 = S.flat(table + 2u * L + 1u);
            const float ax = (n0.x - o.x) * inv.x, bx = (n1.x - o.x) * inv.x;
            const float ay = (n0.y - o.y) * inv.y, by = (n1.y - o.y) * inv.y;
            const float az = (n0.z - o.z) * inv.z, bz = (n1.z - o.z) * inv.z;
            const float t_0 = __builtin_fmaxf(__builtin_fmaxf(__builtin_fmaxf(ax, ay), az), 0.0f);
            const float t_1 = __builtin_fminf(__builtin_fminf(__builtin_fminf(bx, by), bz), RT_INFINITY);
            const uint32_t keep = t_0 > t_1 ? 0u : 0xffffffffu;
            all_lo |= as_u(n0.w) & keep;
            all_hi |= as_u(n1.w) & keep;
        }
    } else {
#pragma unroll 4
        for (uint32_t L = 0; L < n_leaves; L++) {
            if (!((active >> L) & 1u)) continue;
            RT_MARK(5);
            DBG_WAVE_TICK(10);
            DBG_ADD(11, 1);
            const float4 n0 = S.flat(2u * L), n1 = S.flat(2u * L + 1u);
            const float ax = (n0.x - o.x) * inv.x, bx = (n1.x - o.x) * inv.x;
            const float ay = (n0.y - o.y) * inv.y, by = (n1.y - o.y) * inv.y;
            const float az = (n0.z - o.z) * inv.z, bz = (n1.z - o.z) * inv.z;
            const float t_0 = __builtin_fmaxf(__builtin_fmaxf(__builtin_fmaxf(__builtin_fminf(ax, bx), __builtin_fminf(ay, by)), __builtin_fminf(az, bz)), 0.0f);
            const float t_1 = __builtin_fminf(__builtin_fminf(__builtin_fminf(__builtin_fmaxf(ax, bx), __builtin_fmaxf(ay, by)), __builtin_fmaxf(az, bz)), RT_INFINITY);
            const bool miss = t_0 > t_1;
            all_lo |= miss ? 0u : as_u(n0.w);
            all_hi |= miss ? 0u : as_u(n1.w);
        }
    }
    RT_MARK(6);
    const unsigned long long all_m = resumed ? rem : (((unsigned long long)all_hi << 32) | all_lo);
    const unsigned long long tri_all = ((unsigned long long)sc.tri_mask_hi << 32) | sc.tri_mask_lo;
    const unsigned long long pl_all = ((unsigned long long)sc.plane_mask_hi << 32) | sc.plane_mask_lo;
    unsigned long long tri_m = all_m & tri_all, pl_m = all_m & pl_all, sp_m = all_m & ~(tri_all | pl_all);
    const uint32_t octant = (inv.x < 0.0f ? 1u : 0u) | (inv.y < 0.0f ? 2u : 0u) | (inv.z < 0.0f ? 4u : 0u);
#define RT_FLAT_ACCEPT(t, rec)                                                                                         \
    bool better = ((t) >= 0.0f) & ((t) < h.t);                                                                         \
    if (((t) == h.t) & (h.t < RT_INFINITY)) better = flat_rank_of(sc, octant, (rec)) < flat_rank_of(sc, octant, h.ref); \
    h.t = better ? (t) : h.t;                                                                                          \
    h.ref = better ? (rec) : h.ref;
    const uint32_t tri_started = (uint32_t)__popcll(__ballot(tri_m != 0ull));
    while (tri_m != 0ull) {
        RT_MARK(7);
        DBG_WAVE_TICK(12);
        DBG_ADD(13, 1); DBG_ADD(25, 1);
        const uint32_t rec_a = (uint32_t)__builtin_ctzll(tri_m);
        tri_m &= tri_m - 1ull;
        const bool two = tri_m != 0ull;
        const uint32_t rec_b = two ? (uint32_t)__builtin_ctzll(tri_m) : rec_a;
        tri_m &= tri_m - 1ull;
        const float4 a0 = S.prim(4u * rec_a), a1 = S.prim(4u * rec_a + 1u), a2 = S.prim(4u * rec_a + 2u);
        const float4 b0 = S.prim(4u * rec_b), b1 = S.prim(4u * rec_b + 1u), b2 = S.prim(4u * rec_b + 2u);
        float u, v;
        const float ta = triangle_t(o, d, v3(a0.x, a0.y, a0.z), v3(a1.x, a1.y, a1.z), v3(a2.x, a2.y, a2.z), u, v);
        const float tb = triangle_t(o, d, v3(b0.x, b0.y, b0.z), v3(b1.x, b1.y, b1.z), v3(b2.x, b2.y, b2.z), u, v);
        bool stop;
        {
            const float t = ta;
            RT_FLAT_ACCEPT(t, rec_a)
            stop = better & anyhit;
        }
        if (two & !stop) {
            DBG_ADD(13, 1);
            const float t = tb;
            RT_FLAT_ACCEPT(t, rec_b)
            stop = better & anyhit;
        }
        if (stop) tri_m = pl_m = sp_m = 0ull;
        if ((uint32_t)__popcll(__ballot(tri_m != 0ull)) * 100u < tri_started * quorum) break;
    }
    RT_MARK(8);
    const unsigned long long tri_left = tri_m;
    while (pl_m != 0ull) {
        RT_MARK(9);
        DBG_WAVE_TICK(15);
        DBG_ADD(13, 1); DBG_ADD(29, 1);
        const uint32_t rec = (uint32_t)__builtin_ctzll(pl_m);
        pl_m &= pl_m - 1ull;
        const float4 r0 = S.prim(4u * rec), r1 = S.prim(4u * rec + 1u), r2 = S.prim(4u * rec + 2u), r3 = S.prim(4u * rec + 3u);
        const float t = plane_t(o, d, v3(r0.x, r0.y, r0.z), v3(r1.x, r1.y, r1.z), v3(r2.x, r2.y, r2.z), v3(r3.x, r3.y, r3.z));
        RT_FLAT_ACCEPT(t, rec)
        if (better & anyhit) pl_m = sp_m = 0ull;
    }
    RT_MARK(8);
    while (sp_m != 0ull) {
        RT_MARK(10);
        DBG_WAVE_TICK(28);
        DBG_ADD(13, 1); DBG_ADD(30, 1);
        const uint32_t rec = (uint32_t)__builtin_ctzll(sp_m);
        sp_m &= sp_m - 1ull;
        const float4 r0 = S.prim(4u * rec), r1 = S.prim(4u * rec + 1u);
        const float t = sphere_t(o, d, v3(r0.x, r0.y, r0.z), r1.y);
        RT_FLAT_ACCEPT(t, rec)
        if (better & anyhit) sp_m = 0ull;
    }
#undef RT_FLAT_ACCEPT
    RT_MARK(13);
    rem = (anyhit & (h.t < RT_INFINITY)) ? 0ull : tri_left;
    cur = rem != 0ull ? 1u : RT_END;
}

#define RT_REF_UNKNOWN 0xffffffffu
RT_DEV uint32_t prim_rank_of(const DevScene &sc, uint32_t octant, uint32_t rec) { return sc.prim_rank[(size_t)octant * sc.n_prims + rec]; }

template <class View>
RT_DEV void trace_preorder(DBG_DECL const View &S, const DevScene &sc, V3 o, V3 d, bool prune, bool anyhit, uint32_t budget, uint32_t quorum, uint32_t &cur,
                           Hit &h, const uint32_t *ref_mem, uint32_t &work)
{
    static_assert(RT_LEAFQ >= 2 && RT_LEAFQ <= 4, "one byte of each 32-bit mask per held leaf; the leaf-loop vote rewinds to a second or later leaf");
    const V3 inv = rt_rcp3(d);
    const uint32_t octant = (inv.x < 0.0f ? 1u : 0u) | (inv.y < 0.0f ? 2u : 0u) | (inv.z < 0.0f ? 4u : 0u);
    const uint32_t n_elems = sc.n_pnodes;
    uint32_t steps = 0;
    while (cur != RT_END && steps < budget) {
        DBG_WAVE_TICK(14);
        uint32_t qi[RT_LEAFQ], qe[RT_LEAFQ];
        uint32_t nq = 0, all_m = 0, tri_m = 0, pl_m = 0;
#pragma unroll
        for (int j = 0; j < RT_LEAFQ; j++) qi[j] = qe[j] = 0u;
        const uint32_t started = (uint32_t)__popcll(__ballot(true));
        while (cur != RT_END && nq < RT_LEAFQ) {
            DBG_WAVE_TICK(10);
            DBG_ADD(11, 1);
            steps++;
            float4 n0, n1;
            S.pnode_pair(cur, n0, n1);
            float t_0;
            bool inside = slab_test(n0, n1, o, inv, t_0);
            inside = inside & !(prune & (t_0 > h.t));
            const uint32_t w0 = as_u(n0.w), w1 = as_u(n1.w);
            const bool leaf = (w0 >> 31) != 0u;
            if (inside & leaf) {
                const uint32_t idx = w0 & 0x7fffffffu, len = w1 & 0xffffu, hi = w1 >> 16;
#pragma unroll
                for (int j = 0; j < RT_LEAFQ; j++) {
                    qi[j] = (nq == (uint32_t)j) ? idx : qi[j];
                    qe[j] = (nq == (uint32_t)j) ? cur : qe[j];
                }
                const uint32_t sh = 8u * nq;
                all_m |= ((1u << len) - 1u) << sh;
                tri_m |= (hi & 0xffu) << sh;
                pl_m |= (hi >> 8) << sh;
                steps += len;
                nq++;
            }
            const uint32_t next = leaf ? cur + 1u : (inside ? w0 : w1);
            cur = next >= n_elems ? RT_END : next;
            if ((uint32_t)__popcll(__ballot((cur != RT_END) & (nq < RT_LEAFQ))) * 100u < started * quorum) break;
        }
        uint32_t sp_m = all_m & ~(tri_m | pl_m);
#define RT_PRE_ACCEPT(t, rec)                                                                                   \
        bool better = ((t) >= 0.0f) & ((t) < h.t);                                                                  \
        if (((t) == h.t) & (h.t < RT_INFINITY)) {                                                                   \
            if (h.ref == RT_REF_UNKNOWN) h.ref = *ref_mem;                                                          \
            better = prim_rank_of(sc, octant, (rec)) < prim_rank_of(sc, octant, h.ref);                            \
        }                                                                                                           \
        h.t = better ? (t) : h.t;                                                                                   \
        h.ref = better ? (rec) : h.ref;
        const uint32_t tri_started = (uint32_t)__popcll(__ballot(tri_m != 0u));
        while (tri_m != 0u) {
            DBG_WAVE_TICK(12);
            DBG_ADD(13, 1);
            const uint32_t pa = take_lowest(tri_m);
            const bool two = tri_m != 0u;
            const uint32_t pb = two ? take_lowest(tri_m) : pa;
            uint32_t base_a = qi[0], base_b = qi[0];
#pragma unroll
            for (int j = 1; j < RT_LEAFQ; j++) {
                base_a = ((pa >> 3) == (uint32_t)j) ? qi[j] : base_a;
                base_b = ((pb >> 3) == (uint32_t)j) ? qi[j] : base_b;
            }
            const uint32_t rec_a = base_a + (pa & 7u), rec_b = base_b + (pb & 7u);
            const float4 a0 = S.prim(4u * rec_a), a1 = S.prim(4u * rec_a + 1u), a2 = S.prim(4u * rec_a + 2u);
            const float4 b0 = S.prim(4u * rec_b), b1 = S.prim(4u * rec_b + 1u), b2 = S.prim(4u * rec_b + 2u);
            float u, v;
            bool stop = false;
            {
                const float t = triangle_t(o, d, v3(a0.x, a0.y, a0.z), v3(a1.x, a1.y, a1.z), v3(a2.x, a2.y, a2.z), u, v);
                RT_PRE_ACCEPT(t, rec_a)
// ... 198 lines not shown
        if (im != 0u) {
            if ((w.grp & 15u) != 0u) wstack_push<DEEP>(w, w.grp, r.wmem, r.wstride);
            w.grp = ((wa & 0x3ffffffu) << 4) | im;
        } else if ((w.grp & 15u) == 0u) {
            w.grp = wstack_pop<DEEP>(w, r.wmem, r.wstride);
        }
        if ((w.grp & 15u) != 0u) {
            w.cur = (w.grp >> 4) + (uint32_t)__builtin_ctz(w.grp);
            w.grp &= w.grp - 1u;
        } else {
            w.cur = RT_END;
        }
        if (stop) { w.cur = RT_END; r.tri_m = 0ull; r.ovf_tri = 0u; }
        if ((uint32_t)__popcll(__ballot(r.looking())) * 100u < n_started * quorum) break;
    }
}

template <class View>
RT_DEV void wide_tris(DBG_DECL const View &S, const DevScene &sc, WideRay &r, Hit &h, uint32_t quorum, bool all)
{
    const V3 o = r.o, d = r.d;
    const uint32_t tri_started = (uint32_t)__popcll(__ballot(r.tri_m != 0ull));
    while (r.tri_m != 0ull) {
        DBG_WAVE_TICK(12);
        DBG_ADD(13, 1);
        const uint32_t rec_a = r.win_base + (uint32_t)__builtin_ctzll(r.tri_m);
        r.tri_m &= r.tri_m - 1ull;
        const bool two = r.tri_m != 0ull;
        const uint32_t rec_b = two ? r.win_base + (uint32_t)__builtin_ctzll(r.tri_m) : rec_a;
        r.tri_m &= r.tri_m - 1ull;
        float4 ra[3], rb[3];
        S.template prim_rec<3>(rec_a, ra);
        S.template prim_rec<3>(rec_b, rb);
        float u, v;
        bool stop = false;
        {
            const float t = triangle_t(o, d, v3(ra[0].x, ra[0].y, ra[0].z), v3(ra[1].x, ra[1].y, ra[1].z), v3(ra[2].x, ra[2].y, ra[2].z), u, v);
            RT_WIDE_ACCEPT(t, rec_a)
            stop = better & r.anyhit;
        }
        if (two & !stop) {
            DBG_ADD(13, 1);
            const float t = triangle_t(o, d, v3(rb[0].x, rb[0].y, rb[0].z), v3(rb[1].x, rb[1].y, rb[1].z), v3(rb[2].x, rb[2].y, rb[2].z), u, v);
            RT_WIDE_ACCEPT(t, rec_b)
            stop = better & r.anyhit;
        }
        if (stop) { r.w.cur = RT_END; r.tri_m = 0ull; r.ovf_tri = 0u; }
        if (!all && (uint32_t)__popcll(__ballot(r.tri_m != 0ull)) * 100u < tri_started * quorum) break;
    }
    if (r.ovf_tri != 0u && r.tri_m == 0ull) { r.win_base = r.ovf_base; r.tri_m = r.ovf_tri; r.ovf_tri = 0u; }
}
#undef RT_WIDE_TEST_OTHER
#undef RT_WIDE_ACCEPT

template <bool DEEP, class View>
RT_DEV void trace_wide(DBG_DECL const View &S, const DevScene &sc, V3 o, V3 d, V3 inv, bool anyhit, uint32_t budget, uint32_t quorum, uint32_t stop_quorum,
                       WalkState &w, Hit &h, const uint32_t *ref_mem, uint32_t *wmem, uint32_t wstride, uint32_t &work)
{
    WideRay r;
    r.start(o, d, inv, anyhit, ref_mem, wmem, wstride);
    r.w = w;
    uint32_t steps = 0, rounds = 0;
    const uint32_t started = (uint32_t)__popcll(__ballot(r.w.cur != RT_END));
    bool stopping = false;
    for (;;) {
        DBG_WAVE_TICK(14);
        if (!stopping) wide_nodes<DEEP>(DBG_ARG S, sc, r, h, quorum, (uint32_t)__popcll(__ballot(true)), steps);
        wide_tris(DBG_ARG S, sc, r, h, quorum, stopping);
        if (stopping) {
            if (r.tri_m == 0ull) break;
            continue;
        }
        rounds++;
        stopping = rounds >= budget || (uint32_t)__popcll(__ballot((r.w.cur != RT_END) | (r.tri_m != 0ull))) * 100u < started * stop_quorum;
        if (r.tri_m == 0ull && (stopping || r.w.cur == RT_END)) break;
    }
    w = r.w;
    work += steps;
}

template <int TRAV, class View>
RT_DEV void trace_dispatch(DBG_DECL const View &S, const DevScene &sc, V3 o, V3 d, bool prune, bool anyhit, uint32_t budget, uint32_t quorum, uint32_t &cur,
                           Hit &h, const uint32_t *ref_mem, uint32_t &work, unsigned long long &flat_rem, uint32_t *wmem = nullptr, uint32_t wstride = 0,
                           uint32_t stop_quorum = 0, bool coherent = false)
{
    if (TRAV == 4 || TRAV == 5) {
        constexpr bool DEEP = TRAV == 5;
        const V3 inv = rt_rcp3(d);
        const float finite = ((inv.x + inv.y) + inv.z) * 0.0f + ((o.x + o.y) + o.z) * 0.0f;
        if (finite == 0.0f) {
            WalkState w;
            w.fresh();
            if (cur != 0u) wstate_load<DEEP>(w, wmem, wstride);
            trace_wide<DEEP>(DBG_ARG S, sc, o, d, inv, anyhit, budget, quorum, stop_quorum, w, h, ref_mem, wmem, wstride, work);
            if (w.cur == RT_END) {
                cur = RT_END;
            } else {
                wstate_store<DEEP>(w, wmem, wstride);
                cur = 1u;
            }
        } else {
            trace_preorder(DBG_ARG S, sc, o, d, prune, anyhit, 0xffffffffu, 0u, cur, h, ref_mem, work);
        }
    } else if (TRAV == 2) {
        const V3 inv = rt_rcp3(d);
        const float finite = ((inv.x + inv.y) + inv.z) * 0.0f + ((o.x + o.y) + o.z) * 0.0f;
        if (finite == 0.0f) {
            trace_flat(DBG_ARG S, sc, o, d, inv, anyhit, quorum, cur, flat_rem, h, coherent);
        } else {
            RT_MARK_COLD();
            trace_threaded(DBG_ARG S, sc.n_nodes, o, d, prune, anyhit, 0xffffffffu, cur, h, work);
        }
    } else if (TRAV == 3) {
        trace_preorder(DBG_ARG S, sc, o, d, prune, anyhit, budget, quorum, cur, h, ref_mem, work);
    } else if (TRAV == 1) {
        trace_threaded_typed(DBG_ARG S, sc.n_nodes, o, d, prune, anyhit, budget, cur, h, work);
    } else {
        trace_threaded(DBG_ARG S, sc.n_nodes, o, d, prune, anyhit, budget, cur, h, work);
    }
}
```

rsoderh-raytracing_amd/csrc/hip/rt_wavepool.h:

```cpp
#pragma once
#include "rt_device.h"
#include "rt_coop.h"

enum HotField { H_OX, H_OY, H_OZ, H_EX, H_EY, H_EZ, H_SX, H_SY, H_SZ, H_T, H_CT, H_COUNT };
enum CtBits : uint32_t {
    F_SHADOW = 8u,
    F_EXT = 16u,
    F_NEE = 32u,
    F_OCCLUDED = 64u,
    CT_FLAGS = 120u,
    CT_SHIFT = 7u
};
enum ColdField {
    C_TX, C_TY, C_TZ, C_LX, C_LY, C_LZ, C_NEEX, C_NEEY, C_NEEZ, C_LASTPDF, C_OUT,
    C_RNG,
    C_BOUNCE,
    C_REF,
    C_COUNT,
    C_REM_LO = C_RNG, C_REM_HI = C_BOUNCE,
    C_COUNT_FLAT = C_REF
};
#define RT_FLAT_BOUNCE_SHIFT 8u
#define RT_FLAT_BOUNCE_BITS 0xffff00u
#define RT_FLAT_RESUMED (1u << 24)
#define RT_FLAT_MAX_BOUNCES 0xffffu
#define C_WIDE_STATE ((uint32_t)C_COUNT)
#define C_COUNT_WIDE ((uint32_t)C_COUNT + 2u + RT_WSTACK)
#define C_COUNT_WIDE_DEEP ((uint32_t)C_COUNT + RT_WSTATE_WORDS)
__host__ __device__ constexpr uint32_t pool_cold_columns(int trav)
{
    return trav == 2 ? (uint32_t)C_COUNT_FLAT : (trav == 4 ? C_COUNT_WIDE : (trav == 5 ? C_COUNT_WIDE_DEEP : (trav == 6 ? (uint32_t)C_REF : (uint32_t)C_COUNT)));
}
enum PoolTag { TAG_FREE = 0, TAG_TRACE = 1, TAG_MISS = 2, TAG_SHADE = 3, TAG_FINISH = 4, TAG_IDLE = 6 };
enum PoolStage { ST_GEN = 0, ST_TRACE = 1, ST_MISS = 2, ST_SHADE = 3, ST_FINISH = 4, ST_COUNT = 5 };

__host__ __device__ constexpr uint32_t pool_hot_columns(int trav) { return trav == 6 ? 12u : (uint32_t)H_COUNT; }
__host__ __device__ constexpr uint32_t pool_list_dwords(int trav) { return trav == 6 ? RT_COOP_LCAP : 64u; }
__host__ __device__ constexpr uint32_t pool_wave_lds_dwords(int trav, uint32_t pool) { return pool_hot_columns(trav) * pool + pool_list_dwords(trav) + (trav == 6 ? RT_COOP_NCAP + RT_COOP_MAP : 0u); }
__host__ __device__ constexpr uint32_t pool_wave_cold_dwords(int trav, uint32_t pool) { return pool_cold_columns(trav) * pool + (trav == 6 ? RT_COOP_GCAP : 0u); }
template <uint32_t POOL, int TRAV>
struct PoolLayout {
    static constexpr uint32_t kSlotsPerLane = (POOL + 63u) / 64u;
    static constexpr uint32_t kHotDwords = pool_hot_columns(TRAV) * POOL;
    static constexpr uint32_t kListDwords = pool_list_dwords(TRAV);
    static constexpr uint32_t kWaveLdsDwords = pool_wave_lds_dwords(TRAV, POOL);
    static constexpr uint32_t kColdColumns = pool_cold_columns(TRAV);
    static constexpr uint32_t kWaveColdDwords = pool_wave_cold_dwords(TRAV, POOL);
    static constexpr uint32_t kCtColumn = pool_hot_columns(TRAV) - 1u;
};

RT_DEV uint32_t stage_of_tag(uint32_t tag) { return tag; }

#define RT_WAVE_HANDOVER()                                        \
    do {                                                          \
        __builtin_amdgcn_fence(__ATOMIC_RELEASE, "wavefront");    \
        __builtin_amdgcn_wave_barrier();                          \
        __builtin_amdgcn_fence(__ATOMIC_ACQUIRE, "wavefront");    \
    } while (0)

typedef float rt_f3v __attribute__((ext_vector_type(3)));
typedef rt_f3v rt_f3v_a4 __attribute__((aligned(4)));
RT_DEV void store_sample(float *dst, V3 L) { __builtin_nontemporal_store(rt_f3v{L.x, L.y, L.z}, reinterpret_cast<rt_f3v_a4 *>(dst)); }

#ifndef RT_POOL_WAVES_PER_SIMD
#define RT_POOL_WAVES_PER_SIMD 4
#endif
template <int SV> struct PoolView;
template <> struct PoolView<0> { typedef SceneView<false> type; static __device__ __forceinline__ type make(const DevScene &sc) { return make_view<false>(sc); } };
template <> struct PoolView<1> { typedef SceneView<true> type; static __device__ __forceinline__ type make(const DevScene &sc) { return make_view<true>(sc); } };
template <> struct PoolView<2> { typedef SceneViewHybrid type; static __device__ __forceinline__ type make(const DevScene &sc) { return make_view_hybrid(sc); } };

template <int SV, uint32_t BLOCK, uint32_t POOL, int TRAV>
__global__ __launch_bounds__(BLOCK, RT_POOL_WAVES_PER_SIMD) void rt_render_pool_kernel(RenderParams P)
{
    typedef PoolLayout<POOL, TRAV> L;
    constexpr bool kCoop = TRAV == 6;
    constexpr bool kBounceInCt = TRAV == 2;
    constexpr bool kRngHot = TRAV == 2;
    constexpr uint32_t kTCell = kRngHot ? (uint32_t)H_SX : (uint32_t)H_T;
    constexpr bool kFlatVote = kRngHot && kBounceInCt;
    constexpr bool kPackedMiss = TRAV == 2 || TRAV == 6;
    constexpr bool kGenTrace = TRAV >= 2 && !kCoop;
    const DevScene &sc = P.scene;
    if (SV != 0) stage_scene_lds(sc);
    const typename PoolView<SV>::type S = PoolView<SV>::make(sc);
    const uint32_t lane0 = threadIdx.x & (RT_WAVE - 1);
    constexpr bool kScalarWave = SV == 2 || TRAV == 6;
    const uint32_t wave = kScalarWave ? (uint32_t)__builtin_amdgcn_readfirstlane((int)(threadIdx.x / RT_WAVE)) : threadIdx.x / RT_WAVE;
    uint32_t *const lds32 = reinterpret_cast<uint32_t *>(rt_smem + sc.lds_float4s);
    uint32_t *const W = lds32 + wave * L::kWaveLdsDwords;
    uint32_t *const WCT = W + L::kCtColumn * POOL;
    uint32_t *const list = W + L::kHotDwords;
    uint32_t *const G = P.cold_state + (size_t)(blockIdx.x * (BLOCK / RT_WAVE) + wave) * L::kWaveColdDwords;
    const bool prune = (P.flags & RSRT_FLAG_PRUNE) != 0;
    const bool anyhit_shadow = !(P.flags & RSRT_FLAG_REFERENCE_TRAVERSAL);
    const uint32_t tile_px = P.tile_w * P.tile_h;

#define HOT(f, slot) W[(f) * POOL + (slot)]
#define HOTF(f, slot) as_f(HOT(f, slot))
#define SETHU(f, slot, val) W[(f) * POOL + (slot)] = (val)
#define SETH(f, slot, val) SETHU(f, slot, as_u(val))
#define CT_OF(slot) WCT[(slot)]
#define TAG_OF(slot) (WCT[(slot)] & 7u)
#define SET_TAG(slot, tag) WCT[(slot)] = (uint32_t)(tag)
#define SET_CT(slot, payload, flags, tag) WCT[(slot)] = ((payload) << CT_SHIFT) | (flags) | (uint32_t)(tag)
#define BEST_REF(slot) W[9u * POOL + 2u * (slot)]
#define BEST_T(slot) W[9u * POOL + 2u * (slot) + 1u]
#define COLD(f, slot) G[(f) * POOL + (slot)]
#define COLDF(f, slot) as_f(G[(f) * POOL + (slot)])
#define SETC(f, slot, val) G[(f) * POOL + (slot)] = as_u(val)

    for (uint32_t k = 0; k < L::kSlotsPerLane; k++)
        if (lane0 + 64u * k < POOL) SET_TAG(lane0 + 64u * k, TAG_FREE);
    RT_WAVE_HANDOVER();

    uint32_t chunk_next = 0, chunk_left = 0, chunk_tile_slot0 = 0, chunk_tx0 = 0, chunk_ty0 = 0, chunk_s0 = 0, chunk_p0 = 0;
    bool exhausted = false;
    unsigned long long n_paths = 0, n_ext = 0, n_shadow = 0;
    uint32_t n_work = 0;
#ifdef RT_INSTRUMENT
    DbgCounters dbg;
    for (int i = 0; i < RT_DBG_N; i++) dbg.c[i] = 0;
#endif

#ifdef RT_INSTRUMENT
    unsigned long long t_prev = __builtin_amdgcn_s_memtime();
#define DBG_STAMP(i) do { unsigned long long t_now = __builtin_amdgcn_s_memtime(); if (lane0 == 0) dbg.c[i] += t_now - t_prev; t_prev = t_now; } while (0)
#else
#define DBG_STAMP(i) do { } while (0)
#endif
#if defined(RT_INSTRUMENT) && defined(RT_SHADE_PROFILE)
#define SHADE_STAMP(i) DBG_STAMP(i)
#else
#define SHADE_STAMP(i) do { } while (0)
#endif
    auto ray_end = [&](const uint32_t slot, const uint32_t ct, const Hit &h, const uint32_t cur, const float t_in, const unsigned long long flat_rem) __attribute__((always_inline)) {
        const bool shadow = (ct & F_SHADOW) != 0u;
        const uint32_t bounce_bits = kBounceInCt ? ((ct >> CT_SHIFT) & RT_FLAT_BOUNCE_BITS) : 0u;
        const bool found = TRAV >= 3 ? (h.ref != RT_REF_UNKNOWN) : (h.t < t_in);
        const bool done = cur == RT_END || (kFlatVote && shadow && h.t < RT_INFINITY);
        if (!done && kFlatVote) {
            COLD(C_REM_LO, slot) = (uint32_t)flat_rem;
            COLD(C_REM_HI, slot) = (uint32_t)(flat_rem >> 32);
            if (!shadow) SETH(kTCell, slot, h.t);
            SET_CT(slot, RT_FLAT_RESUMED | bounce_bits | (shadow ? 0u : h.ref), ct & CT_FLAGS, TAG_TRACE);
        } else if (!done) {
            if (!kRngHot) SETH(H_T, slot, h.t);
            if (TRAV != 2 && !shadow && found) COLD(C_REF, slot) = h.ref;
            SET_CT(slot, cur, ct & CT_FLAGS, TAG_TRACE);
        } else if (shadow) {
            n_shadow++;
            if (!kRngHot) SETH(H_T, slot, RT_INFINITY);
            const uint32_t fl = (ct & (F_EXT | F_NEE)) | (h.t < RT_INFINITY ? (uint32_t)F_OCCLUDED : 0u);
            SET_CT(slot, bounce_bits, fl, (ct & F_EXT) ? TAG_TRACE : TAG_FINISH);
        } else {
            n_ext++;
            SETH(kTCell, slot, h.t);
            if (TRAV != 2 && found) COLD(C_REF, slot) = h.ref;
            SET_CT(slot, (TRAV == 2 ? h.ref : 0u) | bounce_bits, ct & (F_NEE | F_OCCLUDED), h.did_hit() ? TAG_SHADE : TAG_MISS);
        }
    };
    auto trace_slot = [&](const uint32_t slot, const uint32_t ct, const V3 o, const V3 d, const bool coherent) __attribute__((always_inline)) {
        const bool shadow = (ct & F_SHADOW) != 0u;
        Hit h;
        uint32_t cur = kBounceInCt ? (kFlatVote ? (ct >> (CT_SHIFT + 24u)) : 0u) : (ct >> CT_SHIFT);
        h.src = SRC_BVH;
        h.t = kRngHot ? RT_INFINITY : HOTF(H_T, slot); h.u = h.v = 0.0f;
        unsigned long long flat_rem = 0ull;
        if (kFlatVote && cur != 0u) {
            flat_rem = ((unsigned long long)COLD(C_REM_HI, slot) << 32) | COLD(C_REM_LO, slot);
            if (!shadow) h.t = HOTF(kTCell, slot);
        }
        h.ref = (TRAV >= 3 && !shadow) ? RT_REF_UNKNOWN : ((kFlatVote && cur != 0u) ? ((ct >> CT_SHIFT) & 63u) : 0u);
        const float t_in = h.t;
        trace_dispatch<TRAV>(DBG_ARG S, sc, o, d, prune, shadow && anyhit_shadow, P.trace_budget, TRAV == 2 ? (kFlatVote ? P.flat_quorum : 0u) : P.descend_quorum,
                             cur, h, &COLD(C_REF, slot), n_work, flat_rem, TRAV >= 4 ? &G[C_WIDE_STATE * POOL + slot] : nullptr, POOL, P.stop_quorum, coherent);
        ray_end(slot, ct, h, cur, t_in, flat_rem);
    };
    for (;;) {
        uint32_t lane = lane0;
        if (kCoop) asm volatile("" : "+v"(lane));
        RT_MARK(0);
        DBG_STAMP(21);
        uint32_t tags[L::kSlotsPerLane];
        uint32_t count[ST_COUNT] = {};
        for (uint32_t k = 0; k < L::kSlotsPerLane; k++) {
            tags[k] = (lane + 64u * k < POOL) ? TAG_OF(lane + 64u * k) : (uint32_t)TAG_IDLE;
            const uint32_t st = stage_of_tag(tags[k]);
            for (uint32_t s = 0; s < ST_COUNT; s++) count[s] += (uint32_t)__popcll(__ballot(st == s));
        }
        if (exhausted) count[ST_GEN] = 0;
        uint32_t best = ST_COUNT, best_n = 0;
        for (uint32_t s = 0; s < ST_COUNT; s++)
            if (count[s] >= best_n && count[s] > 0) { best = s; best_n = count[s]; }
        if (best == ST_COUNT) break;
        uint32_t base = 0;
        for (uint32_t k = 0; k < L::kSlotsPerLane; k++) {
            const bool mine = stage_of_tag(tags[k]) == best;
            const unsigned long long m = __ballot(mine);
            const uint32_t pos = base + (uint32_t)__popcll(m & ((1ull << lane) - 1ull));
            if (mine && pos < L::kListDwords) list[pos] = lane + 64u * k;
            base += (uint32_t)__popcll(m);
        }
        RT_WAVE_HANDOVER();
        const uint32_t n_run = min(best_n, 64u);
        const bool on = lane < n_run;
        const uint32_t slot = on ? list[lane] : 0u;
        const uint32_t dbg_stage = best;
        (void)dbg_stage;
        if (lane == 0) { DBG_ADD(dbg_stage, 1); DBG_ADD(5 + dbg_stage, (kCoop && best == ST_TRACE) ? best_n : n_run); }
        DBG_STAMP(22);
        RT_MARK(1);

        if (best == ST_GEN) {
            RT_MARK(2);
            uint32_t given = 0;
            bool started = false;
            V3 cam_o = v3(0.0f, 0.0f, 0.0f), cam_d = v3(0.0f, 0.0f, 0.0f);
            while (given < n_run && !exhausted) {
                if (chunk_left == 0u) {
                    uint32_t c = 0;
                    if (lane == 0) c = atomicAdd(P.work_counter, 1u);
                    c = __builtin_amdgcn_readfirstlane((int)c);
                    if (c >= P.n_chunks) { exhausted = true; break; }
                    const uint32_t q = c % P.n_subtiles, cb = c / P.n_subtiles;
                    const uint32_t j = cb / P.n_sblocks, b = cb % P.n_sblocks;
                    uint32_t ttx, tty;
                    if (!owned_tile(j, P.rank, P.world, P.skew, P.tiles_x, P.tiles_per_row, ttx, tty)) continue;
                    chunk_tx0 = ttx * P.tile_w;
                    chunk_ty0 = tty * P.tile_h;
                    chunk_tile_slot0 = j * tile_px;
                    chunk_s0 = b * P.samples_per_chunk;
                    chunk_p0 = q * P.chunk_px;
                    chunk_next = 0;
                    chunk_left = min(P.samples_per_chunk, P.sample_count - chunk_s0) * P.chunk_px;
                }
                const uint32_t take = min(n_run - given, chunk_left);
                if (on && lane >= given && lane < given + take) {
                    const uint32_t item = chunk_next + (lane - given);
                    const uint32_t ks = item / P.chunk_px, p = chunk_p0 + item % P.chunk_px;
                    const uint32_t px = chunk_tx0 + p % P.tile_w, py = chunk_ty0 + p / P.tile_w;
                    if (px < P.width && py < P.height) {
                        const uint32_t srel = chunk_s0 + ks;
                        PathState ps;
                        start_path(P, px, py, P.sample_begin + srel, ps);
                        SETH(H_OX, slot, ps.o.x); SETH(H_OY, slot, ps.o.y); SETH(H_OZ, slot, ps.o.z);
                        SETH(H_EX, slot, ps.d.x); SETH(H_EY, slot, ps.d.y); SETH(H_EZ, slot, ps.d.z);
                        if (kRngHot) SETHU(H_T, slot, ps.rng);
                        else if (!kCoop) SETH(H_T, slot, RT_INFINITY);
                        SETC(C_TX, slot, 1.0f); SETC(C_TY, slot, 1.0f); SETC(C_TZ, slot, 1.0f);
                        SETC(C_LX, slot, 0.0f); SETC(C_LY, slot, 0.0f); SETC(C_LZ, slot, 0.0f);
                        SETC(C_LASTPDF, slot, 1.0f);
                        if (!kRngHot) COLD(C_RNG, slot) = ps.rng;
                        if (!kBounceInCt) COLD(C_BOUNCE, slot) = 0u;
                        COLD(C_OUT, slot) = srel * P.n_slots + chunk_tile_slot0 + p;
                        if (kGenTrace) { started = true; cam_o = ps.o; cam_d = ps.d; }
                        else SET_CT(slot, 0u, F_EXT, TAG_TRACE);
                        n_paths++;
                    }
                }
                given += take;
                chunk_next += take;
                chunk_left -= take;
            }
            RT_MARK(3);
            if (kGenTrace && started) trace_slot(slot, (uint32_t)F_EXT | (uint32_t)TAG_TRACE, cam_o, cam_d, true);
            RT_MARK(14);
            if (exhausted) {
                for (uint32_t k = 0; k < L::kSlotsPerLane; k++)
                    if (lane + 64u * k < POOL && TAG_OF(lane + 64u * k) == TAG_FREE) SET_TAG(lane + 64u * k, TAG_IDLE);
            }
        } else if (kCoop && best == ST_TRACE) {
            if constexpr (kCoop) {
                CoopStacks cs;
                cs.ns = list + L::kListDwords; cs.ls = list; cs.gs = G + L::kColdColumns * POOL;
                cs.map = reinterpret_cast<uint16_t *>(cs.ns + RT_COOP_NCAP);
                cs.ns_h = cs.ns_n = cs.ls_n = cs.gs_n = 0u;
                cs.lds_cap = P.coop_lds_cap; cs.lifo_at = P.coop_lifo_at; cs.narrow_at = P.coop_narrow_at; cs.gcap = P.coop_gcap;
                CoopNoCount coop_cc;
                for (uint32_t i0 = 0; i0 < best_n; i0 += 64u) {
                    const bool valid = i0 + lane < best_n;
                    const uint32_t s = list[valid ? i0 + lane : 0u];
                    coop_push_rays<POOL>(W, cs, coop_cc, valid, s, CT_OF(s), (uint32_t)F_EXT, (uint32_t)F_SHADOW);
                }
                coop_trace<POOL>(DBG_ARG S, W, cs, coop_cc, anyhit_shadow, lane, n_work);
                RT_WAVE_HANDOVER();
                uint32_t my_slot[L::kSlotsPerLane];
                bool mine[L::kSlotsPerLane];
                for (uint32_t k = 0; k < L::kSlotsPerLane; k++) { my_slot[k] = lane + 64u * k; mine[k] = tags[k] == (uint32_t)TAG_TRACE; }
                if (cs.overflowed()) {
                    if (lane == 0u) atomicAdd(&P.stats[RT_COOP_STATS + 6u], 1ull);
                    for (uint32_t k = 0; k < L::kSlotsPerLane; k++)
                        if (mine[k]) coop_abandon<POOL>(W, my_slot[k], (uint32_t)F_EXT, (uint32_t)F_SHADOW);
                }
                coop_slow_rays<POOL, L::kSlotsPerLane>(DBG_ARG S, sc, W, mine, my_slot, anyhit_shadow, n_work);
                for (uint32_t k = 0; k < L::kSlotsPerLane; k++) {
                    if (!mine[k]) continue;
                    const uint32_t s = my_slot[k], ct = CT_OF(s);
                    const uint32_t fl = ct & (uint32_t)(F_NEE | F_OCCLUDED);
                    if (ct & F_SHADOW) n_shadow++;
                    if (ct & F_EXT) {
                        n_ext++;
                        SET_CT(s, 0u, fl, as_f(BEST_T(s)) < RT_INFINITY ? TAG_SHADE : TAG_MISS);
                    } else {
                        SET_CT(s, 0u, fl, TAG_FINISH);
                    }
                }
            }
        } else if (best == ST_TRACE) {
            RT_MARK(12);
            if (on) {
                const uint32_t ct = CT_OF(slot);
                const uint32_t dcol = (ct & F_SHADOW) ? (uint32_t)H_SX : (uint32_t)H_EX;
                const V3 o = v3(HOTF(H_OX, slot), HOTF(H_OY, slot), HOTF(H_OZ, slot));
                const V3 d = v3(HOTF(dcol, slot), HOTF(dcol + 1u, slot), HOTF(dcol + 2u, slot));
                trace_slot(slot, ct, o, d, false);
            }
        } else if (best == ST_MISS) {
            RT_MARK2(0);
            if (on) {
                const uint32_t ct = CT_OF(slot);
                const V3 o = v3(HOTF(H_OX, slot), HOTF(H_OY, slot), HOTF(H_OZ, slot));
                const V3 d = v3(HOTF(H_EX, slot), HOTF(H_EY, slot), HOTF(H_EZ, slot));
                float env_u, env_v;
                direction_to_equirectangular_uv(d, env_u, env_v);
                const EnvBilinearFetch sky_fetch = kPackedMiss ? sample_env_bilinear_begin_pmf(P.env, env_u, env_v) : sample_env_bilinear_begin(P.env, env_u, env_v);
                float sky_pmf = 0.0f;
                if (!kPackedMiss) sky_pmf = environment_direction_pmf(P.env, env_u, env_v);
                const float last_pdf = COLDF(C_LASTPDF, slot);
                const V3 T = v3(COLDF(C_TX, slot), COLDF(C_TY, slot), COLDF(C_TZ, slot));
                V3 Lr = v3(COLDF(C_LX, slot), COLDF(C_LY, slot), COLDF(C_LZ, slot));
                const V3 nee_prev = v3(COLDF(C_NEEX, slot), COLDF(C_NEEY, slot), COLDF(C_NEEZ, slot));
                const uint32_t out_slot = COLD(C_OUT, slot);
                Hit h;
                h.t = RT_INFINITY; h.ref = 0; h.src = SRC_BVH; h.u = h.v = 0.0f;
                for (uint32_t i = 0; i < sc.n_spheres; i++) {
                    RT_MARK2(1);
                    float u, v;
                    float t = test_record(S, i, SRC_FB_SPHERE, o, d, u, v);
                    if (t >= 0.0f && t < h.t) { h.t = t; h.ref = i; h.src = SRC_FB_SPHERE; }
                }
                for (uint32_t i = 0; i < sc.n_planes; i++) {
                    RT_MARK2(2);
                    float u, v;
                    float t = test_record(S, i, SRC_FB_PLANE, o, d, u, v);
                    if (t >= 0.0f && t < h.t) { h.t = t; h.ref = i; h.src = SRC_FB_PLANE; }
                }
                RT_MARK2(3);
                if (h.did_hit()) {
                    if (kCoop) BEST_T(slot) = as_u(h.t); else SETH(kTCell, slot, h.t);
                    if (kCoop) {
                        BEST_REF(slot) = h.ref | (h.src << 30);
                        SET_CT(slot, 0u, ct & (F_NEE | F_OCCLUDED), TAG_SHADE);
                    } else if (TRAV == 2) {
                        SET_CT(slot, h.ref | (h.src << 6) | (kBounceInCt ? ((ct >> CT_SHIFT) & RT_FLAT_BOUNCE_BITS) : 0u), ct & (F_NEE | F_OCCLUDED), TAG_SHADE);
                    } else {
                        COLD(C_REF, slot) = h.ref | (h.src << 30);
                        SET_CT(slot, 0u, ct & (F_NEE | F_OCCLUDED), TAG_SHADE);
                    }
                } else {
                    const V3 sky = sample_env_bilinear_finish(sky_fetch);
                    if (kPackedMiss) sky_pmf = env_bilinear_pmf(P.env, sky_fetch, env_u, env_v);
                    const float pdf = sky_pmf / environment_pixel_solid_angle(env_v, P.env);
                    const float w = power_heuristic(last_pdf, pdf);
                    if ((ct & (F_NEE | F_OCCLUDED)) == F_NEE) Lr = Lr + nee_prev;
                    Lr = Lr + T * sky * w;
                    store_sample(P.sample_buf + (size_t)out_slot * 3u, Lr);
                    SET_TAG(slot, TAG_FREE);
                }
            }
        } else if (best == ST_SHADE) {
            RT_MARK2(4);
            if (on) {
                const uint32_t ct = CT_OF(slot);
                const V3 o = v3(HOTF(H_OX, slot), HOTF(H_OY, slot), HOTF(H_OZ, slot));
                const V3 d = v3(HOTF(H_EX, slot), HOTF(H_EY, slot), HOTF(H_EZ, slot));
                Hit h;
                h.t = kCoop ? as_f(BEST_T(slot)) : HOTF(kTCell, slot);
                if (TRAV == 2) {
                    const uint32_t hr = (ct >> CT_SHIFT) & 0xffu;
                    h.ref = hr & 63u; h.src = hr >> 6;
                } else {
                    const uint32_t hr = kCoop ? BEST_REF(slot) : COLD(C_REF, slot);
                    h.ref = hr & 0x3fffffffu; h.src = hr >> 30;
                }
                DBG_ADD(27, (as_u(hit_record(S, h, 0).w) & 3u) == PRIM_TRIANGLE ? 1 : 0); DBG_ADD(31, (as_u(hit_record(S, h, 0).w) & 3u) == PRIM_SPHERE ? 1 : 0);
                uint32_t rng, bounce;
                V3 T, Lr;
                Surface surf;
                BsdfMaterial mat;
                EnvironmentSample es;
                if constexpr (kRngHot) {
                    rng = HOT(H_T, slot);
                    const EnvironmentPick pick = sample_environment_begin(P.env, rng);
                    T = v3(COLDF(C_TX, slot), COLDF(C_TY, slot), COLDF(C_TZ, slot));
                    Lr = v3(COLDF(C_LX, slot), COLDF(C_LY, slot), COLDF(C_LZ, slot));
                    const V3 nee_prev = v3(COLDF(C_NEEX, slot), COLDF(C_NEEY, slot), COLDF(C_NEEZ, slot));
                    bounce = (kBounceInCt ? (ct >> (CT_SHIFT + RT_FLAT_BOUNCE_SHIFT)) : COLD(C_BOUNCE, slot)) + 1u;
                    SHADE_STAMP(10);
                    hit_barycentrics(S, h, o, d);
                    surf = resolve_hit(S, h, o, d);
                    mat = load_material(S, surf.material_id);
                    SHADE_STAMP(11);
                    es = sample_environment_finish<true>(P.env, rng, pick);
                    SHADE_STAMP(12);
                    if ((ct & (F_NEE | F_OCCLUDED)) == F_NEE) Lr = Lr + nee_prev;
                    Lr = Lr + T * mat.emission;
                } else {
                    hit_barycentrics(S, h, o, d);
                    rng = COLD(C_RNG, slot);
                    T = v3(COLDF(C_TX, slot), COLDF(C_TY, slot), COLDF(C_TZ, slot));
                    Lr = v3(COLDF(C_LX, slot), COLDF(C_LY, slot), COLDF(C_LZ, slot));
                    bounce = (kBounceInCt ? (ct >> (CT_SHIFT + RT_FLAT_BOUNCE_SHIFT)) : COLD(C_BOUNCE, slot)) + 1u;
                    if ((ct & (F_NEE | F_OCCLUDED)) == F_NEE) Lr = Lr + v3(COLDF(C_NEEX, slot), COLDF(C_NEEY, slot), COLDF(C_NEEZ, slot));
                    surf = resolve_hit(S, h, o, d);
                    mat = load_material(S, surf.material_id);
                    Lr = Lr + T * mat.emission;
                    es = sample_environment(P.env, rng);
                }
                const float cos_nee = fmax_(0.0f, dot(surf.normal, es.direction));
                const bool want_shadow = cos_nee > 0.0f && es.pdf > 0.0f;
                const Frame frame = make_frame(surf.normal);
                const V3 wo = to_frame_local(frame, -d);
                V3 nee = v3(0.0f, 0.0f, 0.0f);
                if (want_shadow) {
                    RT_MARK2(5);
                    DBG_WAVE_TICK(23); DBG_ADD(24, 1);
                    const V3 wi = to_frame_local(frame, es.direction);
                    V3 scattering;
                    float pdf_bsdf;
                    bsdf_eval_pdf_local(wo, wi, mat, scattering, pdf_bsdf);
                    const float w = power_heuristic(es.pdf, pdf_bsdf);
                    nee = T * w * es.radiance * scattering * cos_nee / es.pdf;
                }
                RT_MARK2(6);
                SHADE_STAMP(13);
                const BsdfSample bs = bsdf_sample_in_frame(d, surf.normal, frame, wo, mat, rng);
                RT_MARK2(15);
                SHADE_STAMP(14);
                bool finished = false, nee_counts = want_shadow;
                if (bs.dir.x == 0.0f && bs.dir.y == 0.0f && bs.dir.z == 0.0f) {
                    Lr = bs.scattering;
                    nee_counts = false;
                    finished = true;
                } else if (bs.pdf <= 0.0f) {
                    finished = true;
                } else {
                    const float c = fmax_(0.0f, dot(surf.normal, bs.dir));
                    T = T * (bs.scattering * (c / bs.pdf));
                    if (length(T) < 0.001f) finished = true;
                }
                if (bounce >= P.max_bounces) finished = true;
                if (finished && !want_shadow) {
                    store_sample(P.sample_buf + (size_t)COLD(C_OUT, slot) * 3u, Lr);
                    SET_TAG(slot, TAG_FREE);
                } else {
                    SETC(C_LX, slot, Lr.x); SETC(C_LY, slot, Lr.y); SETC(C_LZ, slot, Lr.z);
                    if (nee_counts) { SETC(C_NEEX, slot, nee.x); SETC(C_NEEY, slot, nee.y); SETC(C_NEEZ, slot, nee.z); }
                    if (!finished) {
                        SETC(C_LASTPDF, slot, bs.pdf);
                        SETC(C_TX, slot, T.x); SETC(C_TY, slot, T.y); SETC(C_TZ, slot, T.z);
                        if (kRngHot) SETHU(H_T, slot, rng); else COLD(C_RNG, slot) = rng;
                        if (!kBounceInCt) COLD(C_BOUNCE, slot) = bounce;
                        SETH(H_EX, slot, bs.dir.x); SETH(H_EY, slot, bs.dir.y); SETH(H_EZ, slot, bs.dir.z);
                    }
                    if (want_shadow) { SETH(H_SX, slot, es.direction.x); SETH(H_SY, slot, es.direction.y); SETH(H_SZ, slot, es.direction.z); }
                    SETH(H_OX, slot, surf.point.x); SETH(H_OY, slot, surf.point.y); SETH(H_OZ, slot, surf.point.z);
                    if (!kRngHot && !kCoop) SETH(H_T, slot, RT_INFINITY);
                    SET_CT(slot, kBounceInCt ? (bounce << RT_FLAT_BOUNCE_SHIFT) : 0u,
                           (want_shadow ? (uint32_t)F_SHADOW : 0u) | (finished ? 0u : (uint32_t)F_EXT) | (nee_counts ? (uint32_t)F_NEE : 0u), TAG_TRACE);
                }
            }
        } else {
            RT_MARK2(7);
            if (on) {
                const uint32_t ct = CT_OF(slot);
                V3 Lr = v3(COLDF(C_LX, slot), COLDF(C_LY, slot), COLDF(C_LZ, slot));
                if ((ct & (F_NEE | F_OCCLUDED)) == F_NEE) Lr = Lr + v3(COLDF(C_NEEX, slot), COLDF(C_NEEY, slot), COLDF(C_NEEZ, slot));
                store_sample(P.sample_buf + (size_t)COLD(C_OUT, slot) * 3u, Lr);
                SET_TAG(slot, TAG_FREE);
            }
        }
        RT_MARK(15);
        RT_WAVE_HANDOVER();
        DBG_STAMP(16 + dbg_stage);
    }
#undef HOT
#undef HOTF
#undef SETHU
#undef SETH
#undef CT_OF
#undef TAG_OF
#undef SET_TAG
#undef SET_CT
#undef COLD
#undef BEST_REF
#undef BEST_T
#undef COLDF
#undef SETC

    RT_MARK(11);
    unsigned long long n_work64 = n_work;
    for (int off = 32; off > 0; off >>= 1) {
        n_paths += __shfl_down(n_paths, off);
        n_ext += __shfl_down(n_ext, off);
        n_shadow += __shfl_down(n_shadow, off);
        if (TRAV != 2) n_work64 += __shfl_down(n_work64, off);
    }
    if (lane0 == 0) {
        atomicAdd(&P.stats[0], n_paths);
        atomicAdd(&P.stats[1], n_ext);
        atomicAdd(&P.stats[2], n_shadow);
        if (TRAV != 2) atomicAdd(&P.stats[3], n_work64);
    }
#ifdef RT_INSTRUMENT
    for (int i = 0; i < RT_DBG_N; i++) {
        unsigned long long v = dbg.c[i];
        for (int off = 32; off > 0; off >>= 1) v += __shfl_down(v, off);
        if (lane0 == 0 && v) atomicAdd(&P.stats[4 + i], v);
    }
#endif
}
```

rsoderh-raytracing_amd/state.py:

```python
import ctypes as C

import numpy as np

from . import _build, types as T

FLAG_REFERENCE_TRAVERSAL = 1
WALK_COUNTERS = ("node_trips", "leaf_trips", "spills", "refills", "lifo_trips", "narrow_trips", "overflows", "peak")
FLAG_PRUNE = 2

_SYMBOLS = ["rsrt_context_create", "rsrt_context_destroy", "rsrt_last_error", "rsrt_upload_scene",
            "rsrt_upload_environment", "rsrt_set_partition", "rsrt_accumulator_resize", "rsrt_accumulator_bind",
            "rsrt_accumulator_clear", "rsrt_accumulator_download", "rsrt_resolve_mean_f16", "rsrt_debug_view_f16", "rsrt_render",
            "rsrt_synchronize", "rsrt_get_stats", "rsrt_cast_rays", "rsrt_describe", "rsrt_get_debug_counters", "rsrt_get_region_counters", "rsrt_get_walk_counters", "rsrt_display_srgb8",
            "rsrt_selftest_numerics", "rsrt_build_id", "rsrt_wide_tree_build", "rsrt_build_bvh_device",
            "rsrt_partition_owner", "rsrt_partition_mask", "rsrt_partition_tiles", "rsrt_comm_available", "rsrt_comm_unique_id", "rsrt_comm_init", "rsrt_comm_reduce", "rsrt_comm_set_mode", "rsrt_comm_destroy",
            "rsrt_multi_create", "rsrt_multi_destroy", "rsrt_multi_last_error", "rsrt_multi_size", "rsrt_multi_context",
            "rsrt_multi_upload_scene", "rsrt_multi_upload_environment", "rsrt_multi_resize", "rsrt_multi_clear", "rsrt_multi_render",
            "rsrt_multi_synchronize", "rsrt_multi_download", "rsrt_multi_display_srgb8", "rsrt_multi_get_stats", "rsrt_multi_uses_rccl",
            "rsrt_aov_render", "rsrt_aov_bind", "rsrt_aov_clear", "rsrt_aov_download", "rsrt_denoise", "rsrt_denoised_download",
            "rsrt_denoised_display_srgb8", "rsrt_temporal_accumulate", "rsrt_temporal_reset", "rsrt_temporal_download",
            "rsrt_temporal_accumulate_ex", "rsrt_temporal_moments_download",
            "rsrt_guide_render", "rsrt_guide_bind", "rsrt_guide_clear", "rsrt_guide_download", "rsrt_upsample", "rsrt_upsampled_download",
            "rsrt_upsampled_display_srgb8"]


class RsrtError(RuntimeError):
    def __init__(self, msg, status=None):
        super().__init__(msg)
        self.status = status


DENOISE_DEMODULATE = 1
DENOISE_DEFAULTS = {"iterations": 5, "sigma_color": 2.0, "sigma_normal": 0.5, "sigma_depth": 0.3, "demodulate": True}
AOV_FLOATS = 8


DENOISE_TEMPORAL = 2
TEMPORAL_DEFAULTS = {"max_history": 32, "depth_tolerance": 0.05, "normal_tolerance": 0.9}
TEMPORAL_MOMENTS = 1
DENOISE_VARIANCE = 4
DENOISE_CLAMP = 8
VARIANCE_SIGMA_L = 4.0


UPSAMPLE_DEMODULATE = 1
UPSAMPLE_DENOISED = 2
UPSAMPLE_TEMPORAL = 4
UPSAMPLE_DEFAULTS = {"sigma_normal": 0.5, "sigma_depth": 0.3, "demodulate": True}


class UpsampleParams(C.Structure):
    _fields_ = [("flags", C.c_uint32), ("sigma_normal", C.c_float), ("sigma_depth", C.c_float)]


class TemporalParams(C.Structure):
    _fields_ = [("max_history", C.c_uint32), ("depth_tolerance", C.c_float), ("normal_tolerance", C.c_float)]


class DenoiseParams(C.Structure):
    _fields_ = [("iterations", C.c_uint32), ("flags", C.c_uint32), ("sigma_color", C.c_float), ("sigma_normal", C.c_float),
                ("sigma_depth", C.c_float)]


def build_id():
    return lib().rsrt_build_id().decode()


class Stats(C.Structure):
    _fields_ = [("paths", C.c_uint64), ("ext_rays", C.c_uint64), ("shadow_rays", C.c_uint64), ("kernel_ms", C.c_double),
                ("total_paths", C.c_uint64), ("total_ext_rays", C.c_uint64), ("total_shadow_rays", C.c_uint64),
                ("total_kernel_ms", C.c_double), ("launches", C.c_uint32), ("_pad", C.c_uint32),
                ("trace_kernel_ms", C.c_double), ("resolve_kernel_ms", C.c_double), ("reduce_ms", C.c_double), ("traversal_steps", C.c_uint64)]

    def as_dict(self):
        return {n: getattr(self, n) for n, _ in self._fields_ if n != "_pad"}


_lib = None


def lib():
    global _lib
    if _lib is None:
        try:
            import os
            path = os.environ.get("RSRT_LIB") or _build.build_hip(instrument=os.environ.get("RSRT_INSTRUMENT") == "1")
            L = C.CDLL(path)
        except Exception as e:
            raise RsrtError("librsrt.so (the HIP integrator) is not available: %s" % e) from e
        for s in _SYMBOLS:
            getattr(L, s)
        L.rsrt_last_error.restype = C.c_char_p
        L.rsrt_last_error.argtypes = [C.c_void_p]
        L.rsrt_describe.restype = C.c_char_p
        L.rsrt_describe.argtypes = [C.c_void_p]
        L.rsrt_build_id.restype = C.c_char_p
        L.rsrt_build_id.argtypes = []
        L.rsrt_context_create.argtypes = [C.c_int, C.POINTER(C.c_void_p)]
        L.rsrt_context_destroy.argtypes = [C.c_void_p]
        L.rsrt_upload_scene.argtypes = [C.c_void_p] + [C.c_void_p, C.c_uint32] * 8
        L.rsrt_upload_environment.argtypes = [C.c_void_p, C.c_uint32, C.c_uint32, C.c_uint32, C.c_void_p, C.c_void_p]
        L.rsrt_set_partition.argtypes = [C.c_void_p, C.c_uint32, C.c_uint32, C.c_uint32, C.c_uint32]
        L.rsrt_accumulator_resize.argtypes = [C.c_void_p, C.c_uint32, C.c_uint32]
        L.rsrt_accumulator_bind.argtypes = [C.c_void_p, C.c_void_p, C.c_uint32, C.c_uint32]
        L.rsrt_accumulator_clear.argtypes = [C.c_void_p]
        L.rsrt_accumulator_download.argtypes = [C.c_void_p, C.c_void_p, C.c_size_t]
        L.rsrt_resolve_mean_f16.argtypes = [C.c_void_p, C.c_uint32, C.c_void_p, C.c_size_t]
        L.rsrt_debug_view_f16.argtypes = [C.c_void_p, C.c_uint32, C.c_uint32, C.c_uint32, C.c_void_p, C.c_size_t]
        L.rsrt_display_srgb8.argtypes = [C.c_void_p, C.c_uint32, C.c_void_p, C.c_size_t]
        L.rsrt_render.argtypes = [C.c_void_p, C.c_void_p] + [C.c_uint32] * 7 + [C.c_void_p]
        L.rsrt_synchronize.argtypes = [C.c_void_p]
        L.rsrt_get_stats.argtypes = [C.c_void_p, C.c_void_p]
        L.rsrt_get_debug_counters.argtypes = [C.c_void_p, C.c_void_p]
        L.rsrt_get_region_counters.argtypes = [C.c_void_p, C.c_void_p]
        L.rsrt_get_walk_counters.argtypes = [C.c_void_p, C.c_void_p, C.c_uint32]
        L.rsrt_selftest_numerics.argtypes = [C.c_void_p, C.c_void_p]
        L.rsrt_cast_rays.argtypes = [C.c_void_p, C.c_uint32, C.c_void_p, C.c_void_p, C.c_uint32, C.c_uint32, C.c_void_p]
        L.rsrt_partition_owner.restype = C.c_uint32
        L.rsrt_partition_owner.argtypes = [C.c_uint32] * 7
        L.rsrt_partition_mask.argtypes = [C.c_uint32] * 6 + [C.c_void_p, C.c_void_p]
        L.rsrt_partition_tiles.argtypes = [C.c_uint32] * 6 + [C.c_void_p, C.c_void_p]
        L.rsrt_comm_available.restype = C.c_int
        L.rsrt_comm_available.argtypes = []
        L.rsrt_comm_unique_id.argtypes = [C.c_void_p]
        L.rsrt_comm_init.argtypes = [C.c_void_p, C.c_uint32, C.c_uint32, C.c_void_p]
        L.rsrt_comm_reduce.argtypes = [C.c_void_p, C.c_uint32, C.c_void_p, C.c_void_p]
        L.rsrt_comm_destroy.argtypes = [C.c_void_p]
        L.rsrt_comm_set_mode.argtypes = [C.c_void_p, C.c_uint32]
        L.rsrt_multi_create.argtypes = [C.c_void_p, C.c_uint32, C.POINTER(C.c_void_p)]
        L.rsrt_multi_destroy.argtypes = [C.c_void_p]
        L.rsrt_multi_last_error.restype = C.c_char_p
        L.rsrt_multi_last_error.argtypes = [C.c_void_p]
        L.rsrt_multi_size.restype = C.c_uint32
        L.rsrt_multi_size.argtypes = [C.c_void_p]
        L.rsrt_multi_context.restype = C.c_void_p
        L.rsrt_multi_context.argtypes = [C.c_void_p, C.c_uint32]
        L.rsrt_multi_upload_scene.argtypes = [C.c_void_p] + [C.c_void_p, C.c_uint32] * 8
        L.rsrt_multi_upload_environment.argtypes = [C.c_void_p, C.c_uint32, C.c_uint32, C.c_uint32, C.c_void_p, C.c_void_p]
        L.rsrt_multi_resize.argtypes = [C.c_void_p, C.c_uint32, C.c_uint32]
        L.rsrt_multi_clear.argtypes = [C.c_void_p]
        L.rsrt_multi_render.argtypes = [C.c_void_p, C.c_void_p] + [C.c_uint32] * 7
        L.rsrt_multi_synchronize.argtypes = [C.c_void_p]
        L.rsrt_multi_download.argtypes = [C.c_void_p, C.c_void_p, C.c_size_t]
        L.rsrt_multi_display_srgb8.argtypes = [C.c_void_p, C.c_uint32, C.c_void_p, C.c_size_t]
        L.rsrt_multi_get_stats.argtypes = [C.c_void_p, C.c_void_p]
        L.rsrt_multi_uses_rccl.argtypes = [C.c_void_p]
        L.rsrt_aov_render.argtypes = [C.c_void_p, C.c_void_p] + [C.c_uint32] * 5 + [C.c_void_p]
        L.rsrt_aov_bind.argtypes = [C.c_void_p, C.c_void_p, C.c_uint32, C.c_uint32]
        L.rsrt_aov_clear.argtypes = [C.c_void_p]
        L.rsrt_aov_download.argtypes = [C.c_void_p, C.c_void_p, C.c_size_t]
        L.rsrt_denoise.argtypes = [C.c_void_p, C.c_uint32, C.c_uint32, C.c_void_p, C.c_void_p, C.c_void_p]
        L.rsrt_denoised_download.argtypes = [C.c_void_p, C.c_void_p, C.c_size_t]
        L.rsrt_denoised_display_srgb8.argtypes = [C.c_void_p, C.c_void_p, C.c_size_t]
        L.rsrt_temporal_accumulate.argtypes = [C.c_void_p, C.c_void_p, C.c_uint32, C.c_uint32, C.c_void_p, C.c_void_p]
        L.rsrt_temporal_reset.argtypes = [C.c_void_p]
        L.rsrt_temporal_download.argtypes = [C.c_void_p, C.c_void_p, C.c_size_t]
        L.rsrt_temporal_accumulate_ex.argtypes = [C.c_void_p, C.c_void_p, C.c_uint32, C.c_uint32, C.c_void_p, C.c_uint32, C.c_void_p]
        L.rsrt_temporal_moments_download.argtypes = [C.c_void_p, C.c_void_p, C.c_size_t]
        L.rsrt_guide_render.argtypes = [C.c_void_p, C.c_void_p] + [C.c_uint32] * 5 + [C.c_void_p]
        L.rsrt_guide_bind.argtypes = [C.c_void_p, C.c_void_p, C.c_uint32, C.c_uint32]
        L.rsrt_guide_clear.argtypes = [C.c_void_p]
        L.rsrt_guide_download.argtypes = [C.c_void_p, C.c_void_p, C.c_size_t]
        L.rsrt_upsample.argtypes = [C.c_void_p, C.c_uint32, C.c_uint32, C.c_uint32, C.c_void_p, C.c_void_p, C.c_void_p]
        L.rsrt_upsampled_download.argtypes = [C.c_void_p, C.c_void_p, C.c_size_t]
        L.rsrt_upsampled_display_srgb8.argtypes = [C.c_void_p, C.c_void_p, C.c_size_t]
        _lib = L
    return _lib


def _p(a):
    return a.ctypes.data_as(C.c_void_p) if a is not None and a.size else None


class State:
    def __init__(self, device=0):
        self._L = lib()
        self._ctx = C.c_void_p()
        rc = self._L.rsrt_context_create(device, C.byref(self._ctx))
        if rc != 0:
            raise RsrtError("rsrt_context_create: %s" % self._L.rsrt_last_error(None).decode())
        self.width = self.height = 0
        self.sample_count = 0
        self.max_bounces = 10
        self.environment_index = 0
        self.camera = None
        self._last_hash = None
        self.flags = 0
        self.aov_sample_count = 0
        self._has_aov = False
        self.temporal_sample_count = 0
        self._temporal_key = None
        self.guide_sample_count = 0
        self.guide_width = self.guide_height = 0
        self._guide_bound = False

    @classmethod
    def new(cls, scene, environments, width, height, device=0, camera=None):
        st = cls(device)
# ... 222 lines not shown
            self.denoise(download=False)
        return self.upsample("denoised" if denoise else "mean")

    def render_temporal(self, n=1, max_history=None, depth_tolerance=None, normal_tolerance=None, stream=None, moments=False):
        key = (self.environment_index, self.max_bounces, self.flags, self.width, self.height, bool(moments))
        if key != self._temporal_key:
            self.temporal_reset()
            self._temporal_key = key
        self.clear()
        if self._has_aov:
            self.clear_aov()
        k = self.temporal_sample_count
        self.render_range(k, n, stream=stream)
        self.render_aov(k, n, stream=stream)
        d = TEMPORAL_DEFAULTS
        p = TemporalParams(d["max_history"] if max_history is None else max_history,
                           d["depth_tolerance"] if depth_tolerance is None else depth_tolerance,
                           d["normal_tolerance"] if normal_tolerance is None else normal_tolerance)
        self._check(self._L.rsrt_temporal_accumulate_ex(self._ctx, _p(self.camera), n, n, C.byref(p), TEMPORAL_MOMENTS if moments else 0,
                                                        C.c_void_p(stream) if stream else None), "rsrt_temporal_accumulate_ex")
        self.temporal_sample_count = k + n
        self.sample_count = n
        self._last_hash = None

    def temporal_reset(self):
        self._check(self._L.rsrt_temporal_reset(self._ctx), "rsrt_temporal_reset")
        self.temporal_sample_count = 0

    def download_temporal(self):
        out = np.empty((self.height, self.width, 4), np.float32)
        self._check(self._L.rsrt_temporal_download(self._ctx, _p(out), out.size), "rsrt_temporal_download")
        return out

    def download_temporal_moments(self):
        out = np.empty((self.height, self.width, 4), np.float32)
        self._check(self._L.rsrt_temporal_moments_download(self._ctx, _p(out), out.size), "rsrt_temporal_moments_download")
        return out

    def download(self):
        out = np.empty((self.height, self.width, 4), np.float32)
        self._check(self._L.rsrt_accumulator_download(self._ctx, _p(out), out.size), "rsrt_accumulator_download")
        return out

    def download_mean_f16(self, sample_total=None):
        out = np.empty((self.height, self.width, 4), np.float16)
        n = sample_total if sample_total is not None else self.sample_count
        self._check(self._L.rsrt_resolve_mean_f16(self._ctx, n, _p(out), out.size), "rsrt_resolve_mean_f16")
        return out

    def debug_view(self, dev_index, out_texture=None, sample_count=None, environment_index=None):
        out = np.zeros((self.height, self.width, 4), np.float16) if out_texture is None else np.ascontiguousarray(out_texture, np.float16).copy()
        assert out.shape == (self.height, self.width, 4)
        n = self.sample_count if sample_count is None else sample_count
        e = self.environment_index if environment_index is None else environment_index
        self._check(self._L.rsrt_debug_view_f16(self._ctx, dev_index, e, n, _p(out), out.size), "rsrt_debug_view_f16")
        return out

    def display_srgb8(self, sample_total=None):
        out = np.empty((self.height, self.width, 4), np.uint8)
        n = sample_total if sample_total is not None else self.sample_count
        self._check(self._L.rsrt_display_srgb8(self._ctx, n, _p(out), out.size), "rsrt_display_srgb8")
        return out

    def stats(self):
        s = Stats()
        self._check(self._L.rsrt_get_stats(self._ctx, C.byref(s)), "rsrt_get_stats")
        return s.as_dict()

    def debug_counters(self):
        out = np.zeros(32, np.uint64)
        self._check(self._L.rsrt_get_debug_counters(self._ctx, _p(out)), "rsrt_get_debug_counters")
        return out

    def region_counters(self):
        out = np.zeros(32, np.uint64)
        self._check(self._L.rsrt_get_region_counters(self._ctx, _p(out)), "rsrt_get_region_counters")
        return out

    def walk_counters(self):
        out = np.zeros(len(WALK_COUNTERS), np.uint64)
        self._check(self._L.rsrt_get_walk_counters(self._ctx, _p(out), len(out)), "rsrt_get_walk_counters")
        return {k: int(v) for k, v in zip(WALK_COUNTERS, out)}

    def selftest_numerics(self):
        out = np.zeros(4, np.uint64)
        self._check(self._L.rsrt_selftest_numerics(self._ctx, _p(out)), "rsrt_selftest_numerics")
        return {"mismatches": int(out[0]), "short_path_inputs": int(out[1]), "bare_rcp_wrong": int(out[2]), "first_bad": int(out[3])}

    def build_bvh_device(self, spheres, plane_descs, vertices, triangles):
        sph, pls = np.ascontiguousarray(spheres).view(T.SPHERE).reshape(-1), np.ascontiguousarray(plane_descs).view(T.PLANE_DESC).reshape(-1)
        ver, tri = np.ascontiguousarray(vertices).view(T.VEC3).reshape(-1), np.ascontiguousarray(triangles).view(T.TRIANGLE).reshape(-1)
        n = len(sph) + len(pls) + len(tri)
        prims, nodes = np.zeros(max(n, 1), T.PRIMITIVE_INFO), np.zeros(max(2 * n, 1), T.BVH_NODE)
        n_nodes, depth, ms = C.c_uint32(0), C.c_uint32(0), C.c_double(0.0)
        self._check(self._L.rsrt_build_bvh_device(self._ctx, _p(sph), len(sph), _p(pls), len(pls), _p(ver), len(ver), _p(tri), len(tri), _p(prims), _p(nodes),
                                                  C.byref(n_nodes), C.byref(depth), C.byref(ms)), "rsrt_build_bvh_device")
        return prims[:n], nodes[:n_nodes.value].copy(), depth.value, ms.value

    def cast_rays(self, origins, directions, mode=0, flags=0):
        o = np.ascontiguousarray(origins, np.float32).reshape(-1, 3)
        d = np.ascontiguousarray(directions, np.float32).reshape(-1, 3)
        assert o.shape == d.shape
        out = np.zeros(len(o), T.HIT)
        self._check(self._L.rsrt_cast_rays(self._ctx, len(o), _p(o), _p(d), mode, flags, _p(out)), "rsrt_cast_rays")
        return out


class MultiState:

    def __init__(self, scene, environments, width, height, devices=(0,), camera=None):
        self._L = lib()
        self._m = C.c_void_p()
        devs = (C.c_int * len(devices))(*devices)
        rc = self._L.rsrt_multi_create(devs, len(devices), C.byref(self._m))
        if rc != 0:
            raise RsrtError("rsrt_multi_create failed (%d): %s" % (rc, self._L.rsrt_multi_last_error(None).decode()))
        a = [scene.materials, scene.spheres, scene.planes, scene.vertices, scene.normals, scene.triangles, scene.primitives, scene.bvh_nodes]
        args = []
        for arr in a:
            arr = np.ascontiguousarray(arr)
            args += [_p(arr), len(arr)]
        self._check(self._L.rsrt_multi_upload_scene(self._m, *args), "rsrt_multi_upload_scene")
        for i, env in enumerate(environments if isinstance(environments, (list, tuple)) else [environments]):
            rgba, alias = np.ascontiguousarray(env.rgba, dtype=np.float32), np.ascontiguousarray(env.alias)
            self._check(self._L.rsrt_multi_upload_environment(self._m, i, env.width, env.height, _p(rgba), _p(alias)), "rsrt_multi_upload_environment")
        self._check(self._L.rsrt_multi_resize(self._m, width, height), "rsrt_multi_resize")
        self.width, self.height = width, height
        self.camera = np.array(camera if camera is not None else scene.camera_uniform()).view(T.CAMERA).reshape(1).copy()
        self.max_bounces, self.environment_index, self.flags, self.sample_count = 10, 0, 0, 0

    def _check(self, rc, what):
        if rc != 0:
            raise RsrtError("%s failed (%d): %s" % (what, rc, self._L.rsrt_multi_last_error(self._m).decode()))

    def close(self):
        if self._m:
            self._L.rsrt_multi_destroy(self._m)
            self._m = C.c_void_p()

    def __del__(self):
        try:
            self.close()
        except Exception:
            pass

    def size(self):
        return self._L.rsrt_multi_size(self._m)

    def uses_rccl(self):
        return bool(self._L.rsrt_multi_uses_rccl(self._m))

    def clear(self):
        self._check(self._L.rsrt_multi_clear(self._m), "rsrt_multi_clear")
        self.sample_count = 0

    def render_samples(self, n):
        self._check(self._L.rsrt_multi_render(self._m, _p(self.camera), self.width, self.height, self.sample_count, n, self.max_bounces,
                                              self.environment_index, self.flags), "rsrt_multi_render")
        self.sample_count += n

    def download(self):
        out = np.empty((self.height, self.width, 4), np.float32)
        self._check(self._L.rsrt_multi_download(self._m, _p(out), out.size), "rsrt_multi_download")
        return out

    def display_srgb8(self):
# ... 9 lines not shown
```

Measured before the change: 21730 Mrays/s.

## Fuse fallback sphere/plane tests into flat traversal to skip shadow fallback loop

```diff
diff --git a/include/rsrt.h b/include/rsrt.h
--- a/include/rsrt.h
+++ b/include/rsrt.h
@@ -198,6 +198,11 @@
 rsrt_status rsrt_get_region_counters(rsrt_context *ctx, uint64_t out[32]);
 rsrt_status rsrt_get_walk_counters(rsrt_context *ctx, uint64_t *out, uint32_t n);
 
+rsrt_status rsrt_get_fallback_info(rsrt_context *ctx, uint64_t out[4]);
+rsrt_status rsrt_fallback_table_build(const rsrt_sphere *spheres, uint32_t n_spheres, const rsrt_plane *planes, uint32_t n_planes,
+                                      const rsrt_primitive_info *primitives, uint32_t n_primitives, const rsrt_bvh_node *bvh_nodes, uint32_t n_bvh_nodes,
+                                      uint32_t *sphere_words, uint32_t *plane_words, uint32_t info[4]);
+
 rsrt_status rsrt_selftest_numerics(rsrt_context *ctx, uint64_t out[4]);
 
 const char *rsrt_describe(rsrt_context *ctx);
diff --git a/rsoderh-raytracing_amd/csrc/hip/rsrt_api.hip b/rsoderh-raytracing_amd/csrc/hip/rsrt_api.hip
--- a/rsoderh-raytracing_amd/csrc/hip/rsrt_api.hip
+++ b/rsoderh-raytracing_amd/csrc/hip/rsrt_api.hip
@@ -501,6 +501,8 @@
     bool flat_oriented = true;
     bool allow_hybrid = true;
     uint32_t trace_budget = 0;
+    uint32_t fb_mode = 1;
+    uint32_t fb_distinct = 0, fb_twins = 0;
     uint32_t flat_quorum = 20;
     size_t sample_buffer_budget = 16ull << 30;
     uint32_t probe_repeat = 1;
@@ -589,6 +591,89 @@
     if ((ta & 3u) != (tb & 3u) || memcmp(&a[0], &b[0], 12) != 0) return false;
     if ((ta & 3u) == PRIM_TRIANGLE) return memcmp(&a[1], &b[1], 12) == 0 && memcmp(&a[2], &b[2], 12) == 0;
     return memcmp(a + 1, b + 1, 3 * sizeof(float4)) == 0;
+}
+bool flat_scene_ok(const rsrt_bvh_node *nodes, uint32_t n_nodes, uint32_t n_primitives, uint32_t n_spheres, uint32_t n_planes, std::vector<uint32_t> &leaf_nodes)
+{
+    bool flat_ok = n_primitives <= 64 && n_spheres <= 64 && n_planes <= 64;
+    {
+        std::vector<uint8_t> covered(n_primitives, 0);
+        for (uint32_t i = 0; i < n_nodes && flat_ok; i++)
+            for (uint32_t k = 0; k < nodes[i].primitives_len && flat_ok; k++) {
+                uint8_t &c = covered[nodes[i].primitives_or_second_child_index + k];
+                flat_ok = c == 0;
+                c = 1;
+            }
+    }
+    leaf_nodes.clear();
+    for (uint32_t i = 0; i < n_nodes; i++) {
+        const rsrt_bvh_node &nd = nodes[i];
+        if (nd.primitives_len != 0) { leaf_nodes.push_back(i); continue; }
+        for (uint32_t c : {i + 1u, nd.primitives_or_second_child_index})
+            for (int k = 0; k < 3; k++)
+                flat_ok = flat_ok && nodes[c].bounds_min[k] >= nd.bounds_min[k] && nodes[c].bounds_max[k] <= nd.bounds_max[k];
+    }
+    return flat_ok && leaf_nodes.size() <= 32;
+}
+uint64_t flat_leaf_mask(const rsrt_bvh_node &nd, const float4 *p_prims)
+{
+    uint64_t lm = (nd.primitives_len >= 64 ? ~0ull : ((1ull << nd.primitives_len) - 1ull)) << nd.primitives_or_second_child_index;
+    for (uint32_t b = 1; b < nd.primitives_len; b++)
+        for (uint32_t a = 0; a < b; a++)
+            if (same_test(p_prims + 4 * (nd.primitives_or_second_child_index + a), p_prims + 4 * (nd.primitives_or_second_child_index + b))) {
+                lm &= ~(1ull << (nd.primitives_or_second_child_index + b));
+                break;
+            }
+    return lm;
+}
+struct FallbackTable {
+    std::vector<uint32_t> sphere_word, plane_word;
+    uint32_t distinct = 0, twins = 0, unmatched = 0;
+    bool one_to_one = true;
+    uint32_t packed() const;
+};
+uint32_t FallbackTable::packed() const
+{
+    static_assert(RT_FB_FUSED_MAX * 6u + 8u <= 32u, "the records of the fused loops share one word with their counts");
+    uint32_t np = 0, ns = 0, list = 0, k = 0;
+    for (uint32_t w : plane_word) np += !(w & RT_FB_TWIN);
+    for (uint32_t w : sphere_word) ns += !(w & RT_FB_TWIN);
+    for (const std::vector<uint32_t> *words : {&plane_word, &sphere_word})
+        for (uint32_t w : *words)
+            if (!(w & RT_FB_TWIN) && k < RT_FB_FUSED_MAX) list |= (w & 63u) << (6 * k++);
+    return (np << 2) | (ns << 5) | (list << 8);
+}
+FallbackTable build_fallback_table(const float4 *fbs, uint32_t n_spheres, const float4 *fbp, uint32_t n_planes, const float4 *prims, uint32_t n_prims, uint64_t tested)
+{
+    FallbackTable ft;
+    ft.sphere_word.assign(n_spheres, RT_FB_NONE);
+    ft.plane_word.assign(n_planes, RT_FB_NONE);
+    auto mark_twins = [&](const float4 *arr, std::vector<uint32_t> &word) {
+        for (size_t i = 0; i < word.size(); i++) {
+            bool twin = false;
+            for (size_t j = 0; j < i && !twin; j++) twin = same_test(arr + 4 * j, arr + 4 * i);
+            if (twin) { word[i] |= RT_FB_TWIN; ft.twins++; } else ft.distinct++;
+        }
+    };
+    mark_twins(fbs, ft.sphere_word);
+    mark_twins(fbp, ft.plane_word);
+    for (uint32_t r = 0; r < n_prims && r < 64; r++) {
+        uint32_t tag;
+        memcpy(&tag, &prims[4 * r].w, 4);
+        if (!((tested >> r) & 1ull) || (tag & 3u) == PRIM_TRIANGLE) continue;
+        const float4 *arr = (tag & 3u) == PRIM_SPHERE ? fbs : fbp;
+        std::vector<uint32_t> &word = (tag & 3u) == PRIM_SPHERE ? ft.sphere_word : ft.plane_word;
+        size_t i = 0;
+        while (i < word.size() && ((word[i] & RT_FB_TWIN) || !same_test(arr + 4 * i, prims + 4 * r))) i++;
+        if (i == word.size() || (word[i] & 0xffu) != RT_FB_NONE) { ft.one_to_one = false; continue; }
+        word[i] = r;
+    }
+    for (const std::vector<uint32_t> *words : {&ft.plane_word, &ft.sphere_word})
+        for (uint32_t w : *words) ft.unmatched += !(w & RT_FB_TWIN) && (w & 0xffu) == RT_FB_NONE;
+    return ft;
+}
+bool fallback_fused_ok(const FallbackTable &ft)
+{
+    return ft.one_to_one && ft.unmatched == 0u && ft.distinct >= 1u && ft.distinct <= RT_FB_FUSED_MAX;
 }
 void make_material_record(const rsrt_material &m, float4 *r)
 {
@@ -1024,6 +1109,7 @@
     if (const char *fo = getenv("RSRT_FLAT_ORIENTED")) ctx->flat_oriented = atoi(fo) != 0;
     if (const char *tb = getenv("RSRT_TRACE_BUDGET")) { int v = atoi(tb); if (v > 0) ctx->trace_budget = (uint32_t)v; }
     if (const char *fq = getenv("RSRT_FLAT_QUORUM")) { int v = atoi(fq); if (v >= 0 && v <= 100) ctx->flat_quorum = (uint32_t)v; }
+    if (const char *ff = getenv("RSRT_FB_FUSED")) { int v = atoi(ff); if (v >= 0 && v <= 2) ctx->fb_mode = (uint32_t)v; }
     if (const char *e2 = getenv("RSRT_SAMPLE_BUFFER_MB")) { long v = atol(e2); if (v > 0) ctx->sample_buffer_budget = (size_t)v << 20; }
     if (const char *pr = getenv("RSRT_PROBE_REPEAT")) { int v = atoi(pr); if (v > 1 && v <= 4096) ctx->probe_repeat = (uint32_t)v; }
     if (const char *cl = getenv("RSRT_COOP_LDS_CAP")) { int v = atoi(cl); if (v >= (int)RT_COOP_MIN_LDS_CAP && v <= (int)RT_COOP_NCAP) ctx->coop_lds_cap = (uint32_t)v; }
@@ -1174,24 +1260,7 @@
     }
     const size_t esc_f4 = (8ull * n_nodes + 3) / 4;
     std::vector<uint32_t> leaf_nodes;
-    bool flat_ok = n_primitives <= 64 && n_spheres <= 64 && n_planes <= 64;
-    {
-        std::vector<uint8_t> covered(n_primitives, 0);
-        for (uint32_t i = 0; i < n_nodes && flat_ok; i++)
-            for (uint32_t k = 0; k < nodes[i].primitives_len && flat_ok; k++) {
-                uint8_t &c = covered[nodes[i].primitives_or_second_child_index + k];
-                flat_ok = c == 0;
-                c = 1;
-            }
-    }
-    for (uint32_t i = 0; i < n_nodes; i++) {
-        const rsrt_bvh_node &nd = nodes[i];
-        if (nd.primitives_len != 0) { leaf_nodes.push_back(i); continue; }
-        for (uint32_t c : {i + 1u, nd.primitives_or_second_child_index})
-            for (int k = 0; k < 3; k++)
-                flat_ok = flat_ok && nodes[c].bounds_min[k] >= nd.bounds_min[k] && nodes[c].bounds_max[k] <= nd.bounds_max[k];
-    }
-    flat_ok = flat_ok && leaf_nodes.size() <= 32;
+    const bool flat_ok = flat_scene_ok(nodes, n_nodes, n_primitives, n_spheres, n_planes, leaf_nodes);
     std::vector<uint32_t> flat_rank(8 * 16, 0u);
     uint64_t tri_mask = 0, plane_mask = 0;
     if (flat_ok) {
@@ -1358,16 +1427,12 @@
     float4 *p_fbp = p;
     for (uint32_t i = 0; i < n_planes; i++, p += 4) make_plane_record(planes[i], p);
     float4 *p_flat = p;
+    uint64_t flat_tested = 0;
     if (flat_ok) {
         for (uint32_t i : leaf_nodes) {
             const rsrt_bvh_node &nd = nodes[i];
-            uint64_t lm = (nd.primitives_len >= 64 ? ~0ull : ((1ull << nd.primitives_len) - 1ull)) << nd.primitives_or_second_child_index;
-            for (uint32_t b = 1; b < nd.primitives_len; b++)
-                for (uint32_t a = 0; a < b; a++)
-                    if (same_test(p_prims + 4 * (nd.primitives_or_second_child_index + a), p_prims + 4 * (nd.primitives_or_second_child_index + b))) {
-                        lm &= ~(1ull << (nd.primitives_or_second_child_index + b));
-                        break;
-                    }
+            const uint64_t lm = flat_leaf_mask(nd, p_prims);
+            flat_tested |= lm;
             p[0] = f4(nd.bounds_min[0], nd.bounds_min[1], nd.bounds_min[2], u2f((uint32_t)lm));
             p[1] = f4(nd.bounds_max[0], nd.bounds_max[1], nd.bounds_max[2], u2f((uint32_t)(lm >> 32)));
             p += 2;
@@ -1383,6 +1448,12 @@
             p += oflat_f4;
         }
         memcpy(p, flat_rank.data(), flat_rank.size() * sizeof(uint32_t));
+    }
+    uint32_t fb_fused = 0, fb_distinct = 0, fb_twins = 0;
+    if (flat_ok && ctx->fb_mode != 0u) {
+        const FallbackTable ft = build_fallback_table(p_fbs, n_spheres, p_fbp, n_planes, p_prims, n_primitives, flat_tested);
+        if (fallback_fused_ok(ft)) fb_fused = ctx->fb_mode | ft.packed();
+        fb_distinct = ft.distinct; fb_twins = ft.twins;
     }
     {
         std::vector<uint32_t> twins;
@@ -1445,6 +1516,8 @@
     sc.lds_wnodes = 0u;
     ctx->wimg_nodes = wimg_nodes;
     sc.flat_ok = flat_ok ? 1u : 0u;
+    sc.fb_fused = fb_fused;
+    ctx->fb_distinct = fb_distinct; ctx->fb_twins = fb_twins;
     sc.n_cull = 0; sc.cull_always = 0xffffffffu;
     if (flat_ok) {
         std::vector<uint32_t> leaf_index(n_nodes, 0u);
@@ -1589,6 +1662,53 @@
     return RSRT_OK;
 }
 
+rsrt_status rsrt_fallback_table_build(const rsrt_sphere *spheres, uint32_t n_spheres, const rsrt_plane *planes, uint32_t n_planes,
+                                      const rsrt_primitive_info *primitives, uint32_t n_primitives, const rsrt_bvh_node *nodes, uint32_t n_nodes,
+                                      uint32_t *sphere_words, uint32_t *plane_words, uint32_t info[4])
+{
+    if (!nodes || !info || n_nodes == 0 || (n_primitives && !primitives) || (n_spheres && (!spheres || !sphere_words)) || (n_planes && (!planes || !plane_words)))
+        return RSRT_ERR_INVALID_ARGUMENT;
+    for (uint32_t i = 0; i < n_nodes; i++) {
+        const rsrt_bvh_node &nd = nodes[i];
+        if (nd.primitives_len > 0) { if ((uint64_t)nd.primitives_or_second_child_index + nd.primitives_len > n_primitives) return RSRT_ERR_INVALID_ARGUMENT; }
+        else if (i + 1 >= n_nodes || nd.primitives_or_second_child_index <= i + 1 || nd.primitives_or_second_child_index >= n_nodes) return RSRT_ERR_INVALID_ARGUMENT;
+    }
+    for (uint32_t i = 0; i < n_primitives; i++) {
+        const rsrt_primitive_info &p = primitives[i];
+        if ((p.primitive_type == 0 && p.index >= n_spheres) || (p.primitive_type == 1 && p.index >= n_planes)) return RSRT_ERR_INVALID_ARGUMENT;
+    }
+    std::vector<WideNode> wide;
+    std::vector<rsrt_primitive_info> pp;
+    std::vector<rsrt_bvh_node> nn;
+    std::vector<uint32_t> old_of_new;
+    const bool wide_ok = build_wide_tree(nodes, n_nodes, primitives, n_primitives, wide, pp, nn, &old_of_new);
+    if (wide_ok) { primitives = pp.data(); nodes = nn.data(); }
+    std::vector<uint32_t> leaf_nodes;
+    const bool flat_ok = flat_scene_ok(nodes, n_nodes, n_primitives, n_spheres, n_planes, leaf_nodes);
+    info[0] = flat_ok ? 1u : 0u; info[1] = info[2] = info[3] = 0u;
+    for (uint32_t i = 0; i < n_spheres; i++) sphere_words[i] = 0u;
+    for (uint32_t i = 0; i < n_planes; i++) plane_words[i] = 0u;
+    if (!flat_ok) return RSRT_OK;
+    std::vector<float4> rec(4ull * (n_primitives + n_spheres + n_planes), f4(0, 0, 0, 0));
+    float4 *p_prims = rec.data(), *p_fbs = p_prims + 4ull * n_primitives, *p_fbp = p_fbs + 4ull * n_spheres;
+    for (uint32_t i = 0; i < n_primitives; i++) {
+        const rsrt_primitive_info &pi = primitives[i];
+        if (pi.primitive_type == 0) make_sphere_record(spheres[pi.index], p_prims + 4 * i);
+        else if (pi.primitive_type == 1) make_plane_record(planes[pi.index], p_prims + 4 * i);
+        else p_prims[4 * i] = f4(0, 0, 0, u2f(PRIM_TRIANGLE));
+    }
+    for (uint32_t i = 0; i < n_spheres; i++) make_sphere_record(spheres[i], p_fbs + 4 * i);
+    for (uint32_t i = 0; i < n_planes; i++) make_plane_record(planes[i], p_fbp + 4 * i);
+    uint64_t tested = 0;
+    for (uint32_t i : leaf_nodes) tested |= flat_leaf_mask(nodes[i], p_prims);
+    const FallbackTable ft = build_fallback_table(p_fbs, n_spheres, p_fbp, n_planes, p_prims, n_primitives, tested);
+    auto given = [&](uint32_t w) { return (w & RT_FB_TWIN) || (w & 0xffu) == RT_FB_NONE || !wide_ok ? w : old_of_new[w]; };
+    for (uint32_t i = 0; i < n_spheres; i++) sphere_words[i] = given(ft.sphere_word[i]);
+    for (uint32_t i = 0; i < n_planes; i++) plane_words[i] = given(ft.plane_word[i]);
+    info[1] = fallback_fused_ok(ft) ? 1u : 0u; info[2] = ft.distinct; info[3] = ft.twins;
+    return RSRT_OK;
+}
+
 rsrt_status rsrt_wide_tree_build(const rsrt_primitive_info *primitives, uint32_t n_primitives, const rsrt_bvh_node *nodes, uint32_t n_nodes,
                                  float *wnodes_out, uint32_t *n_wnodes, uint32_t *old_of_new)
 {
@@ -2004,6 +2124,20 @@
     return RSRT_OK;
 }
 
+rsrt_status rsrt_get_fallback_info(rsrt_context *ctx, uint64_t out[4])
+{
+    if (!ctx || !out) return RSRT_ERR_INVALID_ARGUMENT;
+    DeviceGuard g(ctx->device);
+    { rsrt_status st0 = sync_all(ctx); if (st0) return st0; }
+    unsigned long long c = 0;
+    HIP_TRY(ctx, hipMemcpy(&c, ctx->dev_stats + RT_FB_STAT, sizeof c, hipMemcpyDeviceToHost));
+    out[0] = ctx->scene_ready ? (ctx->scene.fb_fused & 3u) : 0u;
+    out[1] = ctx->fb_distinct;
+    out[2] = ctx->fb_twins;
+    out[3] = c;
+    return RSRT_OK;
+}
+
 rsrt_status rsrt_get_region_counters(rsrt_context *ctx, uint64_t out[32])
 {
     if (!ctx || !out) return RSRT_ERR_INVALID_ARGUMENT;
diff --git a/rsoderh-raytracing_amd/csrc/hip/rt_device.h b/rsoderh-raytracing_amd/csrc/hip/rt_device.h
--- a/rsoderh-raytracing_amd/csrc/hip/rt_device.h
+++ b/rsoderh-raytracing_amd/csrc/hip/rt_device.h
@@ -27,6 +27,13 @@
 
 enum { PRIM_SPHERE = 0, PRIM_PLANE = 1, PRIM_TRIANGLE = 2 };
 enum { SRC_BVH = 0, SRC_FB_SPHERE = 1, SRC_FB_PLANE = 2 };
+#define RT_FB_NONE 0xffu
+#define RT_FB_TWIN 0x100u
+#define RT_FB_FUSED_MAX 4u
+enum { FB_UNKNOWN = 0, FB_NO_HIT = 1, FB_NO_HIT_CHECK = 2, FB_SOME_HIT = 3 };
+#define RT_FB_CT_SHADOW 8u
+#define RT_FB_CT_SHIFT 13u
+#define RT_FB_STAT 36u
 
 struct DevScene {
     const float4 *nodes;
@@ -49,6 +56,7 @@
     uint32_t cull_mask[8], cull_always, n_cull;
     const float4 *pnodes;
     uint32_t n_pnodes;
+    uint32_t fb_fused;
     const uint32_t *prim_rank;
     const float4 *wnodes;
     uint32_t n_wnodes, wide_ok;
@@ -1012,7 +1020,7 @@
 
 template <class View>
 RT_DEV void trace_flat(DBG_DECL const View &S, const DevScene &sc, V3 o, V3 d, V3 inv, bool anyhit, uint32_t quorum, uint32_t &cur, unsigned long long &rem, Hit &h,
-                       bool coherent = false)
+                       uint32_t &fb, bool coherent = false)
 {
     RT_MARK(4);
     const bool resumed = cur != 0u;
@@ -1110,6 +1118,39 @@
     }
     RT_MARK(8);
     const unsigned long long tri_left = tri_m;
+    uint32_t fb_known = (fb >> RT_FB_CT_SHIFT) & 3u;
+    if (sc.fb_fused != 0u) {
+        float fb_t = RT_INFINITY;
+        if (__ballot(((pl_m | sp_m) != 0ull) | (((fb & RT_FB_CT_SHADOW) == 0u) & (fb_known == (uint32_t)FB_UNKNOWN))) != 0ull) {
+            uint32_t list = sc.fb_fused >> 8;
+            for (uint32_t k = (sc.fb_fused >> 2) & 7u; k != 0u; k--, list >>= 6) {
+                RT_MARK(9);
+                DBG_WAVE_TICK(15);
+                DBG_ADD(13, 1); DBG_ADD(29, 1);
+                const uint32_t rec = list & 63u;
+                const float4 r0 = S.prim(4u * rec), r1 = S.prim(4u * rec + 1u), r2 = S.prim(4u * rec + 2u), r3 = S.prim(4u * rec + 3u);
+                const float tp = plane_t(o, d, v3(r0.x, r0.y, r0.z), v3(r1.x, r1.y, r1.z), v3(r2.x, r2.y, r2.z), v3(r3.x, r3.y, r3.z));
+                fb_t = __builtin_fminf(fb_t, tp >= 0.0f ? tp : RT_INFINITY);
+                const float t = ((pl_m >> rec) & 1ull) != 0ull ? tp : RT_NO_HIT;
+                RT_FLAT_ACCEPT(t, rec)
+                if (better & anyhit) pl_m = sp_m = 0ull;
+            }
+            RT_MARK(8);
+            for (uint32_t k = (sc.fb_fused >> 5) & 7u; k != 0u; k--, list >>= 6) {
+                RT_MARK(10);
+                DBG_WAVE_TICK(28);
+                DBG_ADD(13, 1); DBG_ADD(30, 1);
+                const uint32_t rec = list & 63u;
+                const float4 r0 = S.prim(4u * rec), r1 = S.prim(4u * rec + 1u);
+                const float ts = sphere_t(o, d, v3(r0.x, r0.y, r0.z), r1.y);
+                fb_t = __builtin_fminf(fb_t, ts >= 0.0f ? ts : RT_INFINITY);
+                const float t = ((sp_m >> rec) & 1ull) != 0ull ? ts : RT_NO_HIT;
+                RT_FLAT_ACCEPT(t, rec)
+                if (better & anyhit) sp_m = 0ull;
+            }
+            fb_known = fb_t < RT_INFINITY ? (uint32_t)FB_SOME_HIT : (sc.fb_fused & 3u);
+        }
+    } else {
     while (pl_m != 0ull) {
         RT_MARK(9);
         DBG_WAVE_TICK(15);
@@ -1133,7 +1174,9 @@
         RT_FLAT_ACCEPT(t, rec)
         if (better & anyhit) sp_m = 0ull;
     }
+    }
 #undef RT_FLAT_ACCEPT
+    fb = fb_known;
     RT_MARK(13);
     rem = (anyhit & (h.t < RT_INFINITY)) ? 0ull : tri_left;
     cur = rem != 0ull ? 1u : RT_END;
@@ -1498,7 +1541,7 @@
 template <int TRAV, class View>
 RT_DEV void trace_dispatch(DBG_DECL const View &S, const DevScene &sc, V3 o, V3 d, bool prune, bool anyhit, uint32_t budget, uint32_t quorum, uint32_t &cur,
                            Hit &h, const uint32_t *ref_mem, uint32_t &work, unsigned long long &flat_rem, uint32_t *wmem = nullptr, uint32_t wstride = 0,
-                           uint32_t stop_quorum = 0, bool coherent = false)
+                           uint32_t stop_quorum = 0, bool coherent = false, uint32_t *fb = nullptr)
 {
     if (TRAV == 4 || TRAV == 5) {
         constexpr bool DEEP = TRAV == 5;
@@ -1522,10 +1565,13 @@
         const V3 inv = rt_rcp3(d);
         const float finite = ((inv.x + inv.y) + inv.z) * 0.0f + ((o.x + o.y) + o.z) * 0.0f;
         if (finite == 0.0f) {
-            trace_flat(DBG_ARG S, sc, o, d, inv, anyhit, quorum, cur, flat_rem, h, coherent);
+            uint32_t fb_state = fb ? *fb : (uint32_t)RT_FB_CT_SHADOW;
+            trace_flat(DBG_ARG S, sc, o, d, inv, anyhit, quorum, cur, flat_rem, h, fb_state, coherent);
+            if (fb) *fb = fb_state;
         } else {
             RT_MARK_COLD();
             trace_threaded(DBG_ARG S, sc.n_nodes, o, d, prune, anyhit, 0xffffffffu, cur, h, work);
+            if (fb) *fb = (uint32_t)FB_UNKNOWN;
         }
     } else if (TRAV == 3) {
         trace_preorder(DBG_ARG S, sc, o, d, prune, anyhit, budget, quorum, cur, h, ref_mem, work);
diff --git a/rsoderh-raytracing_amd/csrc/hip/rt_wavepool.h b/rsoderh-raytracing_amd/csrc/hip/rt_wavepool.h
--- a/rsoderh-raytracing_amd/csrc/hip/rt_wavepool.h
+++ b/rsoderh-raytracing_amd/csrc/hip/rt_wavepool.h
@@ -21,6 +21,7 @@
     C_COUNT_FLAT = C_REF
 };
 #define RT_FLAT_BOUNCE_SHIFT 8u
+#define RT_FLAT_FB_SHIFT 6u
 #define RT_FLAT_BOUNCE_BITS 0xffff00u
 #define RT_FLAT_RESUMED (1u << 24)
 #define RT_FLAT_MAX_BOUNCES 0xffffu
@@ -134,7 +135,7 @@
 #else
 #define SHADE_STAMP(i) do { } while (0)
 #endif
-    auto ray_end = [&](const uint32_t slot, const uint32_t ct, const Hit &h, const uint32_t cur, const float t_in, const unsigned long long flat_rem) __attribute__((always_inline)) {
+    auto ray_end = [&](const uint32_t slot, const uint32_t ct, const Hit &h, const uint32_t cur, const float t_in, const unsigned long long flat_rem, const uint32_t fb) __attribute__((always_inline)) {
         const bool shadow = (ct & F_SHADOW) != 0u;
         const uint32_t bounce_bits = kBounceInCt ? ((ct >> CT_SHIFT) & RT_FLAT_BOUNCE_BITS) : 0u;
         const bool found = TRAV >= 3 ? (h.ref != RT_REF_UNKNOWN) : (h.t < t_in);
@@ -143,7 +144,7 @@
             COLD(C_REM_LO, slot) = (uint32_t)flat_rem;
             COLD(C_REM_HI, slot) = (uint32_t)(flat_rem >> 32);
             if (!shadow) SETH(kTCell, slot, h.t);
-            SET_CT(slot, RT_FLAT_RESUMED | bounce_bits | (shadow ? 0u : h.ref), ct & CT_FLAGS, TAG_TRACE);
+            SET_CT(slot, RT_FLAT_RESUMED | bounce_bits | (shadow ? 0u : (h.ref | (fb << RT_FLAT_FB_SHIFT))), ct & CT_FLAGS, TAG_TRACE);
         } else if (!done) {
             if (!kRngHot) SETH(H_T, slot, h.t);
             if (TRAV != 2 && !shadow && found) COLD(C_REF, slot) = h.ref;
@@ -157,7 +158,7 @@
             n_ext++;
             SETH(kTCell, slot, h.t);
             if (TRAV != 2 && found) COLD(C_REF, slot) = h.ref;
-            SET_CT(slot, (TRAV == 2 ? h.ref : 0u) | bounce_bits, ct & (F_NEE | F_OCCLUDED), h.did_hit() ? TAG_SHADE : TAG_MISS);
+            SET_CT(slot, (TRAV == 2 ? (h.did_hit() ? h.ref : (fb << RT_FLAT_FB_SHIFT)) : 0u) | bounce_bits, ct & (F_NEE | F_OCCLUDED), h.did_hit() ? TAG_SHADE : TAG_MISS);
         }
     };
     auto trace_slot = [&](const uint32_t slot, const uint32_t ct, const V3 o, const V3 d, const bool coherent) __attribute__((always_inline)) {
@@ -173,9 +174,11 @@
         }
         h.ref = (TRAV >= 3 && !shadow) ? RT_REF_UNKNOWN : ((kFlatVote && cur != 0u) ? ((ct >> CT_SHIFT) & 63u) : 0u);
         const float t_in = h.t;
+        static_assert(CT_SHIFT + RT_FLAT_FB_SHIFT == RT_FB_CT_SHIFT && (uint32_t)F_SHADOW == RT_FB_CT_SHADOW, "trace_flat reads the verdict bits and the shadow flag from the tag word");
+        uint32_t fb = ct;
         trace_dispatch<TRAV>(DBG_ARG S, sc, o, d, prune, shadow && anyhit_shadow, P.trace_budget, TRAV == 2 ? (kFlatVote ? P.flat_quorum : 0u) : P.descend_quorum,
-                             cur, h, &COLD(C_REF, slot), n_work, flat_rem, TRAV >= 4 ? &G[C_WIDE_STATE * POOL + slot] : nullptr, POOL, P.stop_quorum, coherent);
-        ray_end(slot, ct, h, cur, t_in, flat_rem);
+                             cur, h, &COLD(C_REF, slot), n_work, flat_rem, TRAV >= 4 ? &G[C_WIDE_STATE * POOL + slot] : nullptr, POOL, P.stop_quorum, coherent, TRAV == 2 ? &fb : nullptr);
+        ray_end(slot, ct, h, cur, t_in, flat_rem, fb);
     };
     for (;;) {
         uint32_t lane = lane0;
@@ -334,17 +337,21 @@
                 const uint32_t out_slot = COLD(C_OUT, slot);
                 Hit h;
                 h.t = RT_INFINITY; h.ref = 0; h.src = SRC_BVH; h.u = h.v = 0.0f;
-                for (uint32_t i = 0; i < sc.n_spheres; i++) {
-                    RT_MARK2(1);
-                    float u, v;
-                    float t = test_record(S, i, SRC_FB_SPHERE, o, d, u, v);
-                    if (t >= 0.0f && t < h.t) { h.t = t; h.ref = i; h.src = SRC_FB_SPHERE; }
-                }
-                for (uint32_t i = 0; i < sc.n_planes; i++) {
-                    RT_MARK2(2);
-                    float u, v;
-                    float t = test_record(S, i, SRC_FB_PLANE, o, d, u, v);
-                    if (t >= 0.0f && t < h.t) { h.t = t; h.ref = i; h.src = SRC_FB_PLANE; }
+                const uint32_t fb = TRAV == 2 ? ((ct >> (CT_SHIFT + RT_FLAT_FB_SHIFT)) & 3u) : (uint32_t)FB_UNKNOWN;
+                if (fb != (uint32_t)FB_NO_HIT) {
+                    for (uint32_t i = 0; i < sc.n_spheres; i++) {
+                        RT_MARK2(1);
+                        float u, v;
+                        float t = test_record(S, i, SRC_FB_SPHERE, o, d, u, v);
+                        if (t >= 0.0f && t < h.t) { h.t = t; h.ref = i; h.src = SRC_FB_SPHERE; }
+                    }
+                    for (uint32_t i = 0; i < sc.n_planes; i++) {
+                        RT_MARK2(2);
+                        float u, v;
+                        float t = test_record(S, i, SRC_FB_PLANE, o, d, u, v);
+                        if (t >= 0.0f && t < h.t) { h.t = t; h.ref = i; h.src = SRC_FB_PLANE; }
+                    }
+                    if (TRAV == 2) n_shadow += (unsigned long long)(((fb == (uint32_t)FB_NO_HIT_CHECK) & h.did_hit()) | ((fb == (uint32_t)FB_SOME_HIT) & !h.did_hit())) << 32;
                 }
                 RT_MARK2(3);
                 if (h.did_hit()) {
@@ -510,7 +517,12 @@
     if (lane0 == 0) {
         atomicAdd(&P.stats[0], n_paths);
         atomicAdd(&P.stats[1], n_ext);
-        atomicAdd(&P.stats[2], n_shadow);
+        if (TRAV == 2) {
+            atomicAdd(&P.stats[2], n_shadow & 0xffffffffull);
+            if ((n_shadow >> 32) != 0ull) atomicAdd(&P.stats[RT_FB_STAT], n_shadow >> 32);
+        } else {
+            atomicAdd(&P.stats[2], n_shadow);
+        }
         if (TRAV != 2) atomicAdd(&P.stats[3], n_work64);
     }
 #ifdef RT_INSTRUMENT
diff --git a/rsoderh-raytracing_amd/state.py b/rsoderh-raytracing_amd/state.py
--- a/rsoderh-raytracing_amd/state.py
+++ b/rsoderh-raytracing_amd/state.py
@@ -11,7 +11,7 @@
 _SYMBOLS = ["rsrt_context_create", "rsrt_context_destroy", "rsrt_last_error", "rsrt_upload_scene",
             "rsrt_upload_environment", "rsrt_set_partition", "rsrt_accumulator_resize", "rsrt_accumulator_bind",
             "rsrt_accumulator_clear", "rsrt_accumulator_download", "rsrt_resolve_mean_f16", "rsrt_debug_view_f16", "rsrt_render",
-            "rsrt_synchronize", "rsrt_get_stats", "rsrt_cast_rays", "rsrt_describe", "rsrt_get_debug_counters", "rsrt_get_region_counters", "rsrt_get_walk_counters", "rsrt_display_srgb8",
+            "rsrt_synchronize", "rsrt_get_stats", "rsrt_cast_rays", "rsrt_describe", "rsrt_get_debug_counters", "rsrt_get_region_counters", "rsrt_get_walk_counters", "rsrt_get_fallback_info", "rsrt_fallback_table_build", "rsrt_display_srgb8",
             "rsrt_selftest_numerics", "rsrt_build_id", "rsrt_wide_tree_build", "rsrt_build_bvh_device",
             "rsrt_partition_owner", "rsrt_partition_mask", "rsrt_partition_tiles", "rsrt_comm_available", "rsrt_comm_unique_id", "rsrt_comm_init", "rsrt_comm_reduce", "rsrt_comm_set_mode", "rsrt_comm_destroy",
             "rsrt_multi_create", "rsrt_multi_destroy", "rsrt_multi_last_error", "rsrt_multi_size", "rsrt_multi_context",
@@ -64,6 +64,21 @@
 
 def build_id():
     return lib().rsrt_build_id().decode()
+
+
+def fallback_table(scene):
+    arrs = [np.ascontiguousarray(scene.spheres), np.ascontiguousarray(scene.planes), np.ascontiguousarray(scene.primitives), np.ascontiguousarray(scene.bvh_nodes)]
+    for arr, dt in zip(arrs, (T.SPHERE, T.PLANE, T.PRIMITIVE_INFO, T.BVH_NODE)):
+        assert arr.dtype.itemsize == dt.itemsize, (arr.dtype, dt)
+    sw, pw, info = np.zeros(max(len(arrs[0]), 1), np.uint32), np.zeros(max(len(arrs[1]), 1), np.uint32), np.zeros(4, np.uint32)
+    args = []
+    for arr in arrs:
+        args += [_p(arr) if len(arr) else None, len(arr)]
+    rc = lib().rsrt_fallback_table_build(*args, _p(sw), _p(pw), _p(info))
+    if rc != 0:
+        raise RsrtError("rsrt_fallback_table_build: bad arguments", rc)
+    return {"sphere_words": sw[:len(arrs[0])].copy(), "plane_words": pw[:len(arrs[1])].copy(), "flat": int(info[0]), "fused": int(info[1]),
+            "distinct": int(info[2]), "twins": int(info[3])}
 
 
 class Stats(C.Structure):
@@ -114,6 +129,8 @@
         L.rsrt_get_debug_counters.argtypes = [C.c_void_p, C.c_void_p]
         L.rsrt_get_region_counters.argtypes = [C.c_void_p, C.c_void_p]
         L.rsrt_get_walk_counters.argtypes = [C.c_void_p, C.c_void_p, C.c_uint32]
+        L.rsrt_get_fallback_info.argtypes = [C.c_void_p, C.c_void_p]
+        L.rsrt_fallback_table_build.argtypes = [C.c_void_p, C.c_uint32] * 4 + [C.c_void_p] * 3
         L.rsrt_selftest_numerics.argtypes = [C.c_void_p, C.c_void_p]
         L.rsrt_cast_rays.argtypes = [C.c_void_p, C.c_uint32, C.c_void_p, C.c_void_p, C.c_uint32, C.c_uint32, C.c_void_p]
         L.rsrt_partition_owner.restype = C.c_uint32
@@ -502,6 +519,11 @@
         self._check(self._L.rsrt_get_walk_counters(self._ctx, _p(out), len(out)), "rsrt_get_walk_counters")
         return {k: int(v) for k, v in zip(WALK_COUNTERS, out)}
 
+    def fallback_info(self):
+        out = np.zeros(4, np.uint64)
+        self._check(self._L.rsrt_get_fallback_info(self._ctx, _p(out)), "rsrt_get_fallback_info")
+        return {k: int(v) for k, v in zip(("fused", "distinct", "twins", "mismatches"), out)}
+
     def selftest_numerics(self):
         out = np.zeros(4, np.uint64)
         self._check(self._L.rsrt_selftest_numerics(self._ctx, _p(out)), "rsrt_selftest_numerics")
```

After: 21300 Mrays/s. 2.0% lower.
